# XieResearchGroup/Physics-aware-Multiplex-GNN

Hardware: AMD Instinct MI355X
Metric: molecules/sec (QM9 dim=128 n_layer=6) at 1/2/4/8 GPU; scatter-add HBM GB/s vs peak (higher is better)
Workload: dtype f32; 1 GPU; QM9-schema synthetic radius-graph batches, PAMNet dim=128 n_layer=6, 128 molecules/GPU (BASELINE configs[1]), full training step fwd+bwd+allreduce+clip+Adam+EMA; global_batch=128, parallelism=dp1 (molecule-sharded, RCCL all-reduce of flat grad), nodes_per_batch=2286, global_edges=32888, local_edges=4316, triplets=6662, pairs=10978

## Files before the change

include/pamnet_hip.h:

```cpp
#ifndef PAMNET_HIP_H
#define PAMNET_HIP_H

#include <stdint.h>

#ifdef __cplusplus
extern "C" {
#endif

#define PAMNET_OK 0
#define PAMNET_EINVAL (-1)
#define PAMNET_ENULL (-2)
#define PAMNET_WEIGHT_IMAGES 2
#define PAMNET_CHAIN_PIECES 16

typedef void* pamnet_stream_t;

#define PAMNET_ABI_VERSION 18
int pamnet_abi_version(void);

int pamnet_segment_sum_f32(float* out, const float* init, const float* A, const int32_t* ia, const float* B,
                           const int32_t* ib, const int32_t* perm, const int32_t* ptr, int64_t rows, int64_t d,
                           pamnet_stream_t stream);

int pamnet_gather_mul_f32(float* out, const float* A, const int32_t* ia, const float* B, const int32_t* ib,
                          int64_t m, int64_t d, pamnet_stream_t stream);

int pamnet_segment_sum_multi_f32(int64_t njobs, float* const* out, const float* const* A, const int32_t* const* perm,
                                 const int32_t* const* ptr, int64_t rows, int64_t d, pamnet_stream_t stream);
int pamnet_gather_mul2_f32(float* out1, float* out2, const float* A, const int32_t* ia, const float* B1,
                           const float* B2, int64_t m, int64_t d, pamnet_stream_t stream);

int pamnet_exclusive_scan_i32(const int32_t* in, int32_t* out, int64_t n, int32_t* tmp, pamnet_stream_t stream);
int pamnet_exclusive_scan_pair_i32(const int32_t* in_a, int32_t* out_a, const int32_t* in_b, int32_t* out_b, int64_t n,
                                   int32_t* tmp, pamnet_stream_t stream);

int pamnet_validate_inputs_i32(const int32_t* node_graph, int64_t n, int64_t n_graphs, const float* types,
                               int64_t type_stride, int64_t n_types, const int32_t* src, const int32_t* dst,
                               int64_t n_edges, int32_t* flag, pamnet_stream_t stream);
int pamnet_csr_from_keys_i32(const int32_t* keys, int64_t m, int64_t rows, int32_t* ptr, int32_t* perm,
                             int32_t* cursor, int32_t* perm_tmp, int32_t* tmp, pamnet_stream_t stream);
int pamnet_csr_from_keys_z_i32(const int32_t* keys, int64_t m, int64_t rows, int32_t* ptr, int32_t* perm,
                               int32_t* cursor, int32_t* perm_tmp, int32_t* tmp, pamnet_stream_t stream);

int pamnet_expand_rows_i32(const int32_t* ptr, int64_t rows, int32_t* row_of, int64_t cap, pamnet_stream_t stream);

int pamnet_csr_filter_count_i32(const int32_t* ptr_in, const int32_t* nbr, const float* dist, int64_t rows, float cut,
                                int32_t* count, pamnet_stream_t stream);
int pamnet_csr_filter_fill_i32(const int32_t* ptr_in, const int32_t* nbr, const float* dist, int64_t rows, float cut,
                               const int32_t* ptr_out, int32_t* nbr_out, float* dist_out, int64_t cap,
                               pamnet_stream_t stream);

int pamnet_radius_count_i32(const float* pos, const int32_t* node_graph, const int32_t* gptr, int64_t n,
                            int64_t n_graphs, float r, int64_t max_neighbors, int32_t* count, int32_t* cap_flag,
                            pamnet_stream_t stream);
int pamnet_radius_fill_i32(const float* pos, const int32_t* node_graph, const int32_t* gptr, int64_t n,
                           int64_t n_graphs, float r, int64_t max_neighbors, const int32_t* ptr, int32_t* nbr, float* dist,
                           int32_t* row_of , int64_t cap,
                           pamnet_stream_t stream);

int pamnet_knn_i32(const float* pos, const int32_t* node_graph, const int32_t* gptr, int64_t n, int32_t k,
                   float cutoff, int32_t* nbr, float* dist, pamnet_stream_t stream);
int pamnet_knn_cut_i32(const float* pos, const int32_t* node_graph, const int32_t* gptr, int64_t n, int32_t k, float cut_a,
                       float cut_b, int32_t* nbr, float* dist, int32_t* cnt_a, int32_t* cnt_b, pamnet_stream_t stream);
int pamnet_knn_tp_total_i64(const int32_t* nbr, const float* dist, int64_t n, int32_t k, float cut, int32_t with_triplets,
                            int32_t* indeg, int64_t* total, pamnet_stream_t stream);
int pamnet_knn_cut_fill_i32(const int32_t* nbr, const float* dist, int64_t n, int32_t k, float cut_a, const int32_t* raw_a,
                            int64_t cap_a, int32_t* nbr_a, float* dist_a, int32_t* row_a, int32_t* ptr_a, float cut_b,
                            const int32_t* raw_b, int64_t cap_b, int32_t* nbr_b, float* dist_b, int32_t* row_b, int32_t* ptr_b,
                            pamnet_stream_t stream);

int pamnet_edge_dist_f32(const float* pos, const int32_t* a, const int32_t* b, int64_t m, float* dist,
                         pamnet_stream_t stream);

int pamnet_triplet_count_i32(const int32_t* lptr, const int32_t* src, const int32_t* dst, int64_t n_edges,
                             int32_t with_triplets, int32_t* tcount, int32_t* tpcount, pamnet_stream_t stream);
int pamnet_triplet_fill_f32(const float* pos, const int32_t* lptr, const int32_t* src, const int32_t* dst,
                            int64_t n_edges, int32_t with_triplets, const int32_t* tp_ptr, int32_t* tp_idx,
                            int32_t* tp_edge, float* tp_angle, int32_t* tp_kind, int64_t cap, pamnet_stream_t stream);
int pamnet_triplet_transpose_count_i32(const int32_t* lptr, const int32_t* src, const int32_t* dst, const int32_t* lt_ptr,
                                       const int32_t* lt_perm, int64_t n_edges, int32_t with_triplets, int32_t* count,
                                       pamnet_stream_t stream);
int pamnet_triplet_transpose_fill_i32(const int32_t* lptr, const int32_t* src, const int32_t* dst, const int32_t* lt_ptr,
                                      const int32_t* lt_perm, int64_t n_edges, int32_t with_triplets, const int32_t* tp_ptr,
                                      const int32_t* tcount, const int32_t* tt_ptr, int32_t* tt_perm, int64_t cap,
                                      pamnet_stream_t stream);

int pamnet_reverse_edges_i32(const int32_t* ptr, const int32_t* row_of, const int32_t* col, int64_t m, int32_t* rev,
                             int32_t* flag, pamnet_stream_t stream);
int pamnet_gather_scalars_i64(int64_t n, const void* const* src ,
                              const int32_t* kind , int64_t* out, pamnet_stream_t stream);
int pamnet_check_sizes_i32(int64_t n_checks, const int32_t* const* actual ,
                           const int64_t* expected , const void* all_kept, const int32_t* self_loops,
                           int32_t* flag, pamnet_stream_t stream);
int pamnet_ingest_indices_i32(const void* batch, int32_t batch_kind, int64_t n, int64_t n_graphs, const void* x,
                              int32_t x_kind, int64_t x_stride, int64_t n_types, const void* edge_src,
                              const void* edge_dst, int32_t edge_kind, int64_t n_edges, int32_t* node_graph,
                              int32_t* gptr_flag, int32_t* types, int32_t* src, int32_t* dst, pamnet_stream_t stream);
int pamnet_gather2_i32(const int32_t* perm, const int32_t* a, const int32_t* b, int64_t m, int32_t* out_a,
                       int32_t* out_b, const float* pos, float* dist, pamnet_stream_t stream);
int pamnet_transpose_gather_i32(const int32_t* perm, const int32_t* q, const float* dist, int64_t m, int32_t* out_q,
                                float* out_dist, int32_t* inv, pamnet_stream_t stream);
int pamnet_collate_f32(int64_t n_graphs, const int32_t* sel, const int32_t* out_nptr, const int32_t* out_eptr,
                       const int32_t* src_nptr, const int32_t* src_eptr, const float* x, int64_t x_width,
                       const float* pos, const int32_t* esrc, const int32_t* edst, int64_t n_out, int64_t e_out,
                       float* out_x, float* out_pos, int32_t* out_batch, int32_t* out_esrc, int32_t* out_edst,
                       const float* y , float* out_y ,
                       pamnet_stream_t stream);

#define PAMNET_SCHEMA_QM9 0
#define PAMNET_SCHEMA_PDBBIND 1
#define PAMNET_SCHEMA_RNA 2
typedef struct pamnet_graph_desc {
    int64_t n, n_graphs, n_bonds;
    int64_t eg, el, tp;
    const void* batch;
    const void* types;
    int64_t types_stride, n_types;
    const float* pos;
    const float* rows;
    int64_t rows_width;
    const void* edge_src;
    const void* edge_dst;
    int32_t schema, batch_kind, types_kind, edge_kind;
    int32_t with_triplets;
    int32_t need_grad;
    int32_t aggregate_at_query;
    int32_t knn_k;
    float cutoff_l, cutoff_g;
    int32_t max_neighbors;
    int32_t mol_local;
} pamnet_graph_desc;
enum {
    PAMNET_GF_NODE_GRAPH = 0,
    PAMNET_GF_GPTR,
    PAMNET_GF_FLAG,
    PAMNET_GF_LOOPS,
    PAMNET_GF_TYPES,
    PAMNET_GF_POS,
    PAMNET_GF_SIGN,
    PAMNET_GF_G_PTR, PAMNET_GF_G_ROW, PAMNET_GF_G_COL, PAMNET_GF_G_DIST,
    PAMNET_GF_GT_PTR, PAMNET_GF_GT_PERM,
    PAMNET_GF_L_PTR, PAMNET_GF_L_ROW, PAMNET_GF_L_COL, PAMNET_GF_L_DIST,
    PAMNET_GF_LT_PTR, PAMNET_GF_LT_PERM,
    PAMNET_GF_T_PTR, PAMNET_GF_T_ROW, PAMNET_GF_T_COL, PAMNET_GF_T_ANGLE, PAMNET_GF_T_KIND,
    PAMNET_GF_TT_PTR, PAMNET_GF_TT_PERM,
    PAMNET_GF_CUTS,
    PAMNET_GF_TT_EDGE, PAMNET_GF_TT_NODE,
    PAMNET_GRAPH_FIELDS
};
typedef struct pamnet_mol_graph_out {
    int32_t *g_ptr, *g_row, *g_col;
    float* g_dist;
    int32_t* gT_perm;
    int32_t *l_ptr, *l_row, *l_col;
    float* l_dist;
    int32_t *lT_ptr, *lT_perm;
    int32_t *t_ptr, *t_row, *t_col;
    float* t_angle;
    int32_t* t_kind;
    int32_t *tT_ptr, *tT_perm;
} pamnet_mol_graph_out;
int pamnet_mol_graph_count_i32(const float* pos, const int32_t* gptr, int64_t n, int64_t n_graphs, const int32_t* src,
                               const int32_t* dst, int64_t n_bonds, float cutoff_g, int32_t with_triplets, int32_t* mol_tot,
                               int32_t* totals, pamnet_stream_t stream);
int pamnet_mol_graph_fill_i32(const float* pos, const int32_t* gptr, int64_t n, int64_t n_graphs, const int32_t* src,
                              const int32_t* dst, int64_t n_bonds, float cutoff_g, int32_t with_triplets, int32_t need_grad,
                              const int32_t* mol_tot, int64_t eg_cap, int64_t tp_cap, const pamnet_mol_graph_out* out,
                              pamnet_stream_t stream);
int pamnet_mol_graph_free_count_i32(const float* pos, const int32_t* gptr, int64_t n, int64_t n_graphs, float cutoff_l,
                                    float cutoff_g, int32_t with_triplets, int32_t* mol_tot, int32_t* totals,
                                    pamnet_stream_t stream);
int pamnet_mol_graph_free_fill_i32(const float* pos, const int32_t* gptr, int64_t n, int64_t n_graphs, int64_t n_local,
                                   float cutoff_l, float cutoff_g, int32_t with_triplets, int32_t need_grad,
                                   const int32_t* mol_tot, int64_t eg_cap, int64_t tp_cap, const pamnet_mol_graph_out* out,
                                   pamnet_stream_t stream);

int pamnet_graph_plan(const pamnet_graph_desc* desc, int64_t* layout , int64_t* arena_ints);
int pamnet_graph_build_i32(const pamnet_graph_desc* desc, int32_t* arena, float* sbf ,
                           pamnet_stream_t stream);

int pamnet_rbf_fwd_f32(const float* dist, const float* freq, float cutoff, int64_t m, float* rbf,
                       pamnet_stream_t stream);
int pamnet_rbf_bwd_f32(const float* dist, const float* freq, float cutoff, int64_t m, const float* grad,
                       float* dfreq, float* partial, pamnet_stream_t stream);
int pamnet_sbf_radial_f32(const float* dist, float cutoff, int64_t m, float* rad, pamnet_stream_t stream);
int pamnet_sbf_combine_f32(const float* rad, const int32_t* idx, const float* angle, int64_t m, float* sbf,
                           pamnet_stream_t stream);
int pamnet_rbf_fwd_env_f32(const float* dist, const float* freq, float cutoff, int32_t envelope_exponent, int64_t m,
                           float* rbf, pamnet_stream_t stream);
int pamnet_rbf_bwd_env_f32(const float* dist, const float* freq, float cutoff, int32_t envelope_exponent, int64_t m,
                           const float* grad, float* dfreq, float* partial, pamnet_stream_t stream);
int pamnet_sbf_radial_tab_f32(const float* dist, float cutoff, int64_t m, int32_t num_spherical, int32_t num_radial,
                              int32_t envelope_exponent, const float* zeros, const double* norm, float* rad,
                              pamnet_stream_t stream);
int pamnet_sbf_combine_tab_f32(const float* rad, const int32_t* idx, const float* angle, int64_t m, int32_t num_spherical,
                               int32_t num_radial, float* sbf, pamnet_stream_t stream);

int pamnet_rbf_ddist_f32(const float* dist, const float* freq, float cutoff, int64_t m, const float* grad, float* ddist,
                         pamnet_stream_t stream);
int pamnet_sbf_bwd_f32(const float* gsbf, const float* dist, float cutoff, int64_t n_edges, const int32_t* idx,
                       const float* angle, int64_t n_rows, const int32_t* tt_ptr, const int32_t* tt_perm, float* rad,
                       float* dangle, float* ddist, pamnet_stream_t stream);
int pamnet_pos_bwd_f32(const float* pos, int64_t n, const int32_t* g_ptr, const int32_t* g_row, const int32_t* g_col,
                       const int32_t* gt_ptr, const int32_t* gt_perm, const float* ddist_g, int64_t eg, const int32_t* l_ptr,
                       const int32_t* l_row, const int32_t* l_col, const int32_t* lt_ptr, const int32_t* lt_perm,
                       const float* ddist_l, int64_t el, const int32_t* t_ptr, const int32_t* t_row, const int32_t* t_col,
                       const int32_t* t_kind, const int32_t* tt_ptr, const int32_t* tt_perm, const float* dangle, int64_t tp,
                       double* bond_work, float* dpos, pamnet_stream_t stream);

int pamnet_fuse_pool_fwd_f32(const float* outs, const float* atts, int64_t n_layer, int64_t n, const float* sign,
                             const int32_t* gptr, int64_t n_graphs, int32_t mean, float* node_out, float* graph_out,
                             pamnet_stream_t stream);
int pamnet_fuse_pool_bwd_f32(const float* outs, const float* atts, int64_t n_layer, int64_t n, const float* sign,
                             const int32_t* node_graph, const int32_t* gptr, int32_t mean, const float* grad_graph,
                             float* grad_outs, float* grad_atts, pamnet_stream_t stream);

int pamnet_node_tail_fwd_f32(const float* x2, const float* res_x, int64_t n, const float* const* weights,
                             const float* const* biases, const float* w_out, const float* b_out, const float* w_att,
                             float* Z, float* R, float* x_out, float* out, float* att, const float* next_Wx1,
                             const float* next_bx1, const float* const* next_wp, int64_t next_ldwp, int64_t next_nblk,
                             float* next_Zx1, float* next_x1, float* next_P, int32_t packed, pamnet_stream_t stream);
int pamnet_node_tail_fwd_rider_f32(const float* x2, const float* res_x, int64_t n, const float* const* weights,
                                   const float* const* biases, const float* w_out, const float* b_out,
                                   const float* w_att, float* Z, float* R, float* x_out, const float* next_Wx1,
                                   const float* next_bx1, const float* const* next_wp, int64_t next_ldwp,
                                   int64_t next_nblk, float* next_Zx1, float* next_x1, float* next_P, const float* mlp_x,
                                   int64_t mlp_rows, int64_t mlp_tile0, int64_t mlp_ntiles, const float* const* mlp,
                                   float* const* mlp_out, int64_t rider_wgs, int32_t packed ,
                                   pamnet_stream_t stream);
int pamnet_node_heads_fwd_f32(int64_t n_layers, const float* const* x_out, const float* const* weights,
                              const float* const* biases, const float* const* w_out, const float* const* b_out,
                              const float* const* w_att, float* const* Z, float* const* out, float* const* att, int64_t n,
                              int32_t packed, pamnet_stream_t stream);
int pamnet_node_tail_bwd_f32(const float* d_xout, const float* d_out, const float* d_att, int64_t n,
                             const float* const* weights, const float* w_out, const float* w_att, const float* Z,
                             float* dZ, float* d_x2, float* d_resx, float* head_partial, float* d_wout, float* d_watt,
                             float* d_bout, int32_t packed, pamnet_stream_t stream);
int pamnet_node_heads_bwd_f32(int64_t n_layers, const float* const* d_out, const float* const* d_att,
                              const float* const* weights, const float* const* w_out, const float* const* w_att,
                              const float* const* Z, float* const* dZ3, float* const* g_head, float* const* head_partial,
                              int64_t n, int32_t packed, pamnet_stream_t stream);
int pamnet_node_tail_main_bwd_f32(const float* d_xout, const float* g_head, int64_t n, const float* const* weights,
                                  const float* Z, float* dZ, float* d_x2, float* d_resx, int32_t packed,
                                  pamnet_stream_t stream);
int pamnet_node_pre_tail_bwd_f32(const float* dP, const float* dx1_direct, const float* d_add, int64_t n,
                                 const float* Wx1, const float* const* wp, int64_t nblk, const float* Zx1, float* dZx1,
                                 const float* g_head, const float* const* weights, const float* Z, float* dZ,
                                 float* d_x2, float* d_resx, const void* rider ,
                                 pamnet_stream_t stream);
typedef struct pamnet_local_agg {
    const float *m_ji, *m_nb, *s, *q3, *init;
    const int32_t *t_ptr, *t_col, *l_ptr;
    float* m_t;
} pamnet_local_agg;
int pamnet_node_tail_fwd_agg_f32(float* x2, const float* res_x, int64_t n, const float* const* weights,
                                 const float* const* biases, const float* w_out, const float* b_out, const float* w_att,
                                 float* Z, float* R, float* x_out, const float* next_Wx1, const float* next_bx1,
                                 const float* const* next_wp, int64_t next_ldwp, int64_t next_nblk, float* next_Zx1,
                                 float* next_x1, float* next_P, const float* mlp_x, int64_t mlp_rows, int64_t mlp_tile0,
                                 int64_t mlp_ntiles, const float* const* mlp, float* const* mlp_out, int64_t rider_wgs,
                                 int32_t packed, const pamnet_local_agg* agg, pamnet_stream_t stream);
int pamnet_node_pre_tail_bwd_gather_f32(float* dP, const float* const* gather_src, const int32_t* const* gather_ptr,
                                        const int32_t* const* gather_perm, const float* dx1_direct, const float* d_add,
                                        int64_t n, const float* Wx1, const float* const* wp, int64_t nblk, const float* Zx1,
                                        float* dZx1, const float* g_head, const float* const* weights, const float* Z,
                                        float* dZ, float* d_x2, float* d_resx, const void* rider ,
                                        pamnet_stream_t stream);
int pamnet_pack_weights_f32(int64_t n, const float* const* W, const int64_t* ld, int32_t transposed, float* images,
                            pamnet_stream_t stream);
int pamnet_pack_weights_bf16x3(int64_t n, const float* const* W, const int64_t* ld, int32_t transposed, float* images,
                               pamnet_stream_t stream);
int pamnet_pack_weights_mixed_f32(int64_t n, const float* const* W, const int64_t* ld, const int32_t* kind,
                                  const int64_t* offset, int32_t transposed, float* images, pamnet_stream_t stream);
int pamnet_node_pre_fwd_f32(const float* x, int64_t n, const float* Wx1, const float* bx1, const float* const* wp,
                            int64_t ldwp, int64_t nblk, float* Zx1, float* x1, float* P, pamnet_stream_t stream);
int pamnet_node_pre_bwd_f32(const float* dP, const float* dx1_direct, const float* d_add, int64_t n, const float* Wx1,
                            const float* const* wp, int64_t ldwp, int64_t nblk, const float* Zx1, float* dZx1,
                            float* dx, int32_t packed, pamnet_stream_t stream);
int pamnet_wgrad_scratch_floats(int64_t njobs, const int64_t* rows, int64_t* floats);
int pamnet_wgrad_batched_f32(int64_t njobs, const float* const* dZ, const int64_t* ld_dz, const float* const* A,
                             const int64_t* ld_a, const int32_t* a_mode, const int64_t* rows, float* const* dW,
                             const int64_t* ld_dw, float* const* db, float* partial, const float* head_partial,
                             int64_t head_blocks, float* d_wout, float* d_watt, float* d_bout, pamnet_stream_t stream);
int pamnet_wgrad_ctx_bytes(int64_t* bytes );
int pamnet_wgrad_deferred_f32(int64_t njobs, const float* const* dZ, const int64_t* ld_dz, const float* const* A,
                              const int64_t* ld_a, const int32_t* a_mode, const int64_t* rows, float* const* dW,
                              const int64_t* ld_dw, float* const* db, float* partial, const float* head_partial,
                              int64_t head_blocks, float* d_wout, float* d_watt, float* d_bout,
                              const float* head2_partial ,
                              float* d_wout2, float* d_watt2, float* d_bout2, void* ctx ,
                              pamnet_stream_t stream);
int pamnet_wgrad_flush_f32(void* ctx , pamnet_stream_t stream);
int pamnet_wgrad_rider_bytes(int64_t* bytes);
int pamnet_wgrad_rider_plan_f32(int64_t njobs, const float* const* dZ, const int64_t* ld_dz, const float* const* A,
                                const int64_t* ld_a, const int32_t* a_mode, const int64_t* rows, float* const* dW,
                                const int64_t* ld_dw, float* const* db, float* partial, int64_t max_slots,
                                void* rider , int64_t* slots_out);
int pamnet_wgrad_rider_enqueue_f32(void* ctx , const void* rider );

int pamnet_global_edge_fwd_f32(const float* e, int64_t n_edges, const float* We, int64_t ld_we, const float* bm,
                               const float* Wea, int64_t ld_wea, const float* Pi, const float* Pj,
                               const int32_t* row_of, const int32_t* col, float* z, float* ea, float* msg,
                               pamnet_stream_t stream);
int pamnet_global_edge_bwd_f32(const float* d_agg, const int32_t* row_of, int64_t n_edges, const float* z,
                               const float* ea, const float* We, int64_t ld_we, const float* Wea, int64_t ld_wea,
                               float* dz, float* dea, float* d_e, int32_t accumulate, pamnet_stream_t stream);
int pamnet_local_edge_fwd_f32(const float* rbf, int64_t n_edges, const float* const* Wq, const int64_t* ldq,
                              const float* b_ji, const float* b_kj, const float* const* P, const int32_t* row_of,
                              const int32_t* col, float* z_ji, float* z_kj, float* q2, float* q3, float* m_ji,
                              float* m_nb, pamnet_stream_t stream);
int pamnet_local_edge_bwd_f32(const float* d_mji, const float* d_mnb, const float* d_q3, int64_t n_edges,
                              const float* z_ji, const float* z_kj, const float* q2, const float* const* Wq,
                              const int64_t* ldq, float* dz_ji, float* dz_kj, float* dq2, float* d_rbf,
                              int32_t accumulate, pamnet_stream_t stream);
int pamnet_global_edge_agg_fwd_f32(const float* e, int64_t n_edges, int64_t n_nodes, const float* We, int64_t ld_we,
                                   const float* bm, const float* Wea, int64_t ld_wea, const float* Pi, const float* Pj,
                                   const int32_t* ptr, const int32_t* row_of, const int32_t* col,
                                   const int32_t* cuts , const float* init, float* z,
                                   float* ea, float* out, pamnet_stream_t stream);
int pamnet_global_edge_agg_fwd_pp_f32(const float* e, int64_t n_edges, int64_t n_nodes, const float* We, int64_t ld_we,
                                      const float* bm, const float* Wea, int64_t ld_wea, const float* Pi, const float* Pj,
                                      const int32_t* ptr, const int32_t* row_of, const int32_t* col,
                                      const int32_t* cuts , const float* init, float* z, float* ea, float* out,
                                      pamnet_stream_t stream);
int pamnet_seg_cuts_i32(const int32_t* ptr, const int32_t* row_of, int64_t n_nodes, int64_t n_edges, int32_t* cuts,
                        int64_t* grid_out, pamnet_stream_t stream);
int pamnet_global_edge_agg_bwd_f32(const float* d_agg, int64_t n_edges, int64_t n_nodes, const int32_t* ptr,
                                   const int32_t* row_of, const int32_t* cuts , const float* z,
                                   const float* ea, const float* We,
                                   int64_t ld_we, const float* Wea, int64_t ld_wea, float* dz, float* dea, float* d_e,
                                   int32_t accumulate, float* dPi, pamnet_stream_t stream);
int pamnet_global_edge_agg_wg_floats(int64_t n_edges, int64_t* floats , int64_t* slots );
int pamnet_global_edge_agg_bwd_wg_f32(const float* d_agg, int64_t n_edges, int64_t n_nodes, const int32_t* ptr,
                                      const int32_t* row_of, const int32_t* cuts , const float* z,
                                      const float* ea, const float* e, const float* We, int64_t ld_we, const float* Wea,
                                      int64_t ld_wea, float* dz, float* d_e, int32_t accumulate, float* dPi, float* partial,
                                      pamnet_stream_t stream);
int pamnet_wgrad_edge_enqueue_f32(void* ctx , int64_t slots, float* dW_e, int64_t ld_e, float* db ,
                                  float* dW_ea, int64_t ld_ea, const float* partial);
int pamnet_local_agg_fwd_f32(const float* m_ji, const float* m_nb, const float* s, const float* q3,
                             const int32_t* t_ptr, const int32_t* t_col, const int32_t* l_ptr, const float* init,
                             int64_t n_nodes, float* m_t, float* out, pamnet_stream_t stream);
int pamnet_local_agg_bwd_f32(const float* d_x2, const int32_t* l_row, const float* q3, const float* m_t,
                             const float* m_nb, const float* s, const int32_t* t_ptr, const int32_t* t_col,
                             const int32_t* t_row, const int32_t* tT_ptr, const int32_t* tT_perm,
                             const int32_t* tT_edge , const int32_t* tT_node , int64_t n_edges,
                             float* d_mt, float* d_q3, float* d_s, float* d_mnb, pamnet_stream_t stream);
int pamnet_triplet_transpose_aux_i32(const int32_t* tT_perm, const int32_t* t_row, const int32_t* l_row, int64_t n_rows,
                                     int32_t* out_edge, int32_t* out_node, pamnet_stream_t stream);
int pamnet_mlp2_fwd_f32(const float* x, int64_t rows, const float* W1, const float* b1, const float* W2,
                        const float* b2, float* z1, float* z2, float* y, pamnet_stream_t stream);
int pamnet_mlp2_fwd_multi_f32(const float* x, int64_t rows, int64_t nsets, const float* const* params,
                              float* const* outs, pamnet_stream_t stream);
int pamnet_mlp2_bwd_f32(const float* dy, int64_t rows, const float* z1, const float* z2, const float* W1,
                        const float* W2, float* dz1, float* dz2, float* dx, int32_t accumulate,
                        pamnet_stream_t stream);
int pamnet_local_bwd_pair_f32(const float* dy, int64_t rows, const float* z1, const float* z2, const float* W1,
                              const float* W2, float* dz1, float* dz2, float* dx, int32_t accumulate_dx,
                              const float* d_mji, const float* d_mnb, const float* d_q3, int64_t n_edges,
                              const float* z_ji, const float* z_kj, const float* q2, const float* const* Wq,
                              const int64_t* ldq, float* dz_ji, float* dz_kj, float* dq2, float* d_rbf,
                              int32_t accumulate_rbf, pamnet_stream_t stream);

int pamnet_embed_scratch_floats(int64_t rows, int64_t K, int64_t* floats);
int pamnet_embed_fwd_f32(const float* x, int64_t rows, int64_t K, const int32_t* kind, const float* W0,
                         const float* b0, const float* W1, const float* b1, int32_t act, float* out,
                         pamnet_stream_t stream);
int pamnet_embed_bwd_f32(const float* x, int64_t rows, int64_t K, const int32_t* kind, const float* W0,
                         const float* b0, const float* W1, const float* b1, int32_t act, const float* gout,
                         float* dW0, float* db0, float* dW1, float* db1, float* dx, float* partial,
                         pamnet_stream_t stream);

typedef struct pamnet_embed_job {
    const float* x;
    const float* dist;
    const float* freq;
    float cutoff;
    int32_t K;
    int32_t act;
    int64_t rows;
    const int32_t* kind;
    const float *W0, *b0, *W1, *b1;
    float* out;
    const float* gout;
    float *dW0, *db0, *dW1, *db1, *dfreq, *dx;
    float* partial;
} pamnet_embed_job;
typedef struct pamnet_type_rows_job {
    const float* table;
    const int32_t* idx;
    int64_t n;
    int64_t n_types;
    float* out;
    const float* g;
    void* scratch;
    float* dtable;
} pamnet_type_rows_job;
int pamnet_embed_multi_fwd_f32(const pamnet_embed_job* jobs, int32_t n_jobs, const pamnet_type_rows_job* types,
                               pamnet_stream_t stream);
int pamnet_embed_multi_bwd_f32(const pamnet_embed_job* jobs, int32_t n_jobs, const pamnet_type_rows_job* types,
                               pamnet_stream_t stream);

int pamnet_stack_workspace(int64_t n, int64_t eg, int64_t el, int64_t tp, int64_t n_layer, int64_t d,
                           int64_t* saved_floats, int64_t* temp_floats);
int pamnet_stack_pack_floats(int64_t n_layer, int64_t d, int64_t* floats);
int pamnet_stack_layout(int64_t n, int64_t eg, int64_t el, int64_t tp, int64_t d, int64_t* layout);
int pamnet_stack_fwd_f32(const int64_t* sizes, const int32_t* const* graph_idx, int64_t n_layer, int64_t d,
                         const float* x0, const float* e_g, const float* rbf_e, const float* e_sbf,
                         const float* const* gparams, const float* const* lparams, float* saved, float* temp, float* outs,
                         float* atts, int32_t save_for_backward, float* wpack, pamnet_stream_t aux_stream,
                         void* const* aux_events, pamnet_stream_t stream);
int pamnet_stack_bwd_f32(const int64_t* sizes, const int32_t* const* graph_idx, int64_t n_layer, int64_t d,
                         const float* x0, const float* e_g, const float* rbf_e, const float* e_sbf,
                         const float* const* gparams, const float* const* lparams, const float* saved, float* temp,
                         const float* d_outs, const float* d_atts, float* const* ggrads, float* const* lgrads,
                         float* d_x0, float* d_eg, float* d_rbf, float* d_sbf, float* wpack, void* const* layer_done,
                         pamnet_stream_t stream);

int pamnet_reduce_scratch_bytes(int64_t* bytes);
int pamnet_stream_copy_f32(const float* src, float* dst, int64_t n, pamnet_stream_t stream);
int pamnet_sumsq_partials_f32(const float* g, int64_t n, double* partials, pamnet_stream_t stream);
int pamnet_l1_loss_f32(const float* out, const float* y, int64_t n, float grad_scale, float* loss, float* d_out,
                       pamnet_stream_t stream);
int pamnet_mse_loss_f32(const float* out, const float* y, int64_t n, float grad_scale, float* loss, float* d_out,
                        pamnet_stream_t stream);
int pamnet_smooth_l1_loss_f32(const float* out, const float* y, int64_t n, float grad_scale, float* loss, float* d_out,
                              pamnet_stream_t stream);
int pamnet_type_rows_grad_f32(const float* g, const int32_t* idx, int64_t n, int64_t n_types, int64_t d, void* scratch,
                              float* out, pamnet_stream_t stream);
#define PAMNET_MAX_PARAM_GROUPS 16
int pamnet_chunk_groups_check(const uint8_t* chunk_group_host, int64_t n_chunks, int64_t n_groups);
int pamnet_sumsq_partials_masked_f32(const float* g, int64_t n, const uint8_t* chunk_group, int64_t n_groups,
                                     const int32_t* frozen, double* partials, pamnet_stream_t stream);
int pamnet_grad_accumulate_f32(float* acc, float* g, int64_t n, pamnet_stream_t stream);

int pamnet_adam_ema_f32(float* p, float* g, float* m, float* v, float* shadow, int64_t n, float lr, float beta1,
                        float beta2, float eps, float weight_decay, int64_t step_count, float ema_decay,
                        const float* grad_norm, float max_norm, int32_t zero_grad, pamnet_stream_t stream);
int pamnet_adam_ema_norm_f32(float* p, float* g, float* m, float* v, float* shadow, int64_t n, float lr, float beta1,
                             float beta2, float eps, float weight_decay, int64_t step_count, float ema_decay,
                             const double* sumsq_partials, float* norm_out, float max_norm, int32_t zero_grad,
                             pamnet_stream_t stream);
int pamnet_adam_ema_groups_f32(float* p, float* g, float* m, float* v, float* shadow, int64_t n, const uint8_t* chunk_group,
                               int64_t n_groups, const float* lr_scale, const float* weight_decay, const int32_t* frozen,
                               float lr, float beta1, float beta2, float eps, int32_t decoupled, int64_t step_count,
                               float ema_decay, const double* sumsq_partials, float* norm_out, float max_norm,
                               int32_t zero_grad, pamnet_stream_t stream);

int pamnet_narrow_blocks(int64_t rows, int64_t* blocks );

int pamnet_narrow_global_fwd_f32(const float* e, int64_t m, int64_t d, const int32_t* tgt, const int32_t* src,
                                 const float* P, const float* We, int64_t ldwe, const float* bias, const float* Wea,
                                 int64_t ldwea, float* msg, pamnet_stream_t stream);
int pamnet_narrow_global_bwd_f32(const float* e, int64_t m, int64_t d, const int32_t* tgt, const int32_t* src,
                                 const float* P, const float* We, int64_t ldwe, const float* bias, const float* Wea,
                                 int64_t ldwea, const float* dagg, float* dz, float* de, float* partial, float* dWe,
                                 float* dWea, float* db, pamnet_stream_t stream);

int pamnet_narrow_mlp2_fwd_f32(const float* x, int64_t m, int64_t d, const float* W1, const float* b1, const float* W2,
                               const float* b2, int32_t res_x, const float* res, float* y, pamnet_stream_t stream);
int pamnet_narrow_mlp2_bwd_f32(const float* x, int64_t m, int64_t d, const float* W1, const float* b1, const float* W2,
                               const float* b2, const float* dy, int32_t res_x, float* dx, float* partial, float* dW,
                               float* db, pamnet_stream_t stream);
// ... 43 lines not shown
```

physics-aware-multiplex-gnn_amd/csrc/basis.hip:

```cpp
#include "common.h"
#include "basis_constants.h"

namespace {

__device__ __forceinline__ float envelope_f(float x) {
    if (!(x < 1.0f)) return 0.0f;
    const float x2 = x * x, x5 = x2 * x2 * x;
    return 1.0f / x + x5 * (-21.0f + x * (35.0f - 15.0f * x));
}

__device__ __forceinline__ double envelope_d(double x) {
    if (!(x < 1.0)) return 0.0;
    const double x2 = x * x, x5 = x2 * x2 * x;
    return 1.0 / x + x5 * (-21.0 + x * (35.0 - 15.0 * x));
}

constexpr int SERIES_TERMS = 28;
struct SeriesTab {
    double c[7][SERIES_TERMS + 1];
    double inv_dfact[7];
};
constexpr SeriesTab make_series() {
    SeriesTab t{};
    for (int l = 0; l < 7; ++l) {
        t.c[l][0] = 1.0;
        for (int k = 1; k <= SERIES_TERMS; ++k) t.c[l][k] = t.c[l][k - 1] * -0.5 / ((double)k * (double)(2 * l + 2 * k + 1));
        double d = 1.0;
        for (int m = 1; m <= l; ++m) d *= (double)(2 * m + 1);
        t.inv_dfact[l] = 1.0 / d;
    }
    return t;
}
__device__ __constant__ SeriesTab SBF_SERIES = make_series();

__device__ __forceinline__ double sph_jl(int l, double z) {
    if (z < (double)l + 1.0) {
        const double h = z * z;
        double sum = SBF_SERIES.c[l][SERIES_TERMS];
#pragma unroll
        for (int k = SERIES_TERMS - 1; k >= 0; --k) sum = fma(sum, h, SBF_SERIES.c[l][k]);
        double pref = SBF_SERIES.inv_dfact[l];
        for (int m = 0; m < l; ++m) pref *= z;
        return pref * sum;
    }
    double s, c;
    sincos(z, &s, &c);
    const double iz = 1.0 / z;
    double jm = s * iz;
    if (l == 0) return jm;
    double j = (jm - c) * iz;
    for (int m = 1; m < l; ++m) {
        const double jn = (double)(2 * m + 1) * iz * j - jm;
        jm = j;
        j = jn;
    }
    return j;
}

__global__ __launch_bounds__(256) void rbf_fwd_kernel(const float* __restrict__ dist, const float* __restrict__ freq,
                                                      float inv_cutoff, int64_t m, float* __restrict__ rbf) {
    const int64_t t = (int64_t)blockIdx.x * blockDim.x + threadIdx.x;
    if (t >= m * 16) return;
    const int64_t e = t >> 4;
    const int n = (int)(t & 15);
    const float x = dist[e] * inv_cutoff;
    rbf[t] = envelope_f(x) * sinf(freq[n] * x);
}

__global__ __launch_bounds__(256) void rbf_bwd_partial_kernel(const float* __restrict__ dist,
                                                              const float* __restrict__ freq, float inv_cutoff,
                                                              int64_t m, const float* __restrict__ grad,
                                                              float* __restrict__ partial) {
    __shared__ float red[256];
    const int n = threadIdx.x & 15, slot = threadIdx.x >> 4;
    const float f = freq[n];
    float acc = 0.f;
    for (int64_t e = (int64_t)blockIdx.x * 16 + slot; e < m; e += (int64_t)gridDim.x * 16) {
        const float x = dist[e] * inv_cutoff;
        acc += grad[e * 16 + n] * envelope_f(x) * x * cosf(f * x);
    }
    red[threadIdx.x] = acc;
    __syncthreads();
    for (int s = 128; s >= 16; s >>= 1) {
        if (threadIdx.x < s) red[threadIdx.x] += red[threadIdx.x + s];
        __syncthreads();
    }
    if (threadIdx.x < 16) partial[blockIdx.x * 16 + threadIdx.x] = red[threadIdx.x];
}

__global__ __launch_bounds__(1024) void rbf_bwd_final_kernel(const float* __restrict__ partial, int nblocks,
                                                             float* __restrict__ dfreq) {
    __shared__ float red[64][17];
    const int n = threadIdx.x & 15, sl = threadIdx.x >> 4;
    float s = 0.f;
    for (int b = sl; b < nblocks; b += 64) s += partial[b * 16 + n];
    red[sl][n] = s;
    __syncthreads();
    if (sl == 0) {
        float t = 0.f;
        for (int q = 0; q < 64; ++q) t += red[q][n];
        dfreq[n] = t;
    }
}

__global__ __launch_bounds__(256) void sbf_radial_rows_kernel(const float* __restrict__ dist, float inv_cutoff, int64_t m,
                                                              float* __restrict__ rad) {
    const int64_t t = (int64_t)blockIdx.x * blockDim.x + threadIdx.x;
    if (t >= m * 6) return;
    const int64_t e = t / 6;
    const int n = (int)(t - e * 6);
    const double x = (double)(dist[e] * inv_cutoff);
    const double env = envelope_d(x);
#pragma unroll 1
    for (int l = 0; l < 7; ++l) {
        const int c = l * 6 + n;
        rad[e * 42 + c] = (float)(env * PAMNET_SBF_NORM[c] * sph_jl(l, (double)PAMNET_SBF_ZEROS_F32[c] * x));
    }
}

__global__ __launch_bounds__(256) void sbf_radial_kernel(const float* __restrict__ dist, float inv_cutoff, int64_t m,
                                                         float* __restrict__ rad) {
    const int64_t t = (int64_t)blockIdx.x * blockDim.x + threadIdx.x;
    if (t >= m * 42) return;
    const int64_t e = t / 42;
    const int c = (int)(t - e * 42), l = c / 6;
    const double x = (double)(dist[e] * inv_cutoff);
    rad[t] = (float)(envelope_d(x) * PAMNET_SBF_NORM[c] * sph_jl(l, (double)PAMNET_SBF_ZEROS_F32[c] * x));
}

constexpr int SBF_ROWS = 64;
__global__ __launch_bounds__(256) void sbf_combine_kernel(const float* __restrict__ rad,
                                                          const int32_t* __restrict__ idx,
                                                          const float* __restrict__ angle, int64_t m,
                                                          float* __restrict__ sbf) {
    __shared__ double ylm[SBF_ROWS][7];
    __shared__ int src[SBF_ROWS];
    const int64_t row0 = (int64_t)blockIdx.x * SBF_ROWS;
    const int tid = threadIdx.x;
    if (tid < SBF_ROWS && row0 + tid < m) {
        const double ct = cos((double)angle[row0 + tid]);
        double p0 = 1.0, p1 = ct;
        ylm[tid][0] = PAMNET_YL0_PREF[0] * p0;
        ylm[tid][1] = PAMNET_YL0_PREF[1] * p1;
#pragma unroll
        for (int k = 2; k <= 6; ++k) {
            const double pl = ((double)(2 * k - 1) * ct * p1 - (double)(k - 1) * p0) / (double)k;
            p0 = p1;
            p1 = pl;
            ylm[tid][k] = PAMNET_YL0_PREF[k] * pl;
        }
        src[tid] = idx[row0 + tid];
    }
    __syncthreads();
    if (tid >= 252) return;
    const int rows = (int)((m - row0 < SBF_ROWS) ? (m - row0) : SBF_ROWS);
    const int r0 = tid / 42, c = tid - r0 * 42, l = c / 6;
    float* out = sbf + row0 * 42 + tid;
#pragma unroll 4
    for (int r = r0; r < rows; r += 6, out += 252)
        *out = (float)((double)rad[(int64_t)src[r] * 42 + c] * ylm[r][l]);
}

__device__ __forceinline__ double envelope_gen_d(double x, int p) {
    if (!(x < 1.0)) return 0.0;
    double xp = 1.0;
    for (int k = 0; k < p; ++k) xp *= x;
    const double a = -0.5 * (double)((p + 1) * (p + 2)), b = (double)(p * (p + 2)), c = -0.5 * (double)(p * (p + 1));
    return 1.0 / x + xp * (a + x * (b + c * x));
}
__device__ __forceinline__ float envelope_gen_f(float x, int p) {
    if (!(x < 1.0f)) return 0.0f;
    float xp = 1.0f;
    for (int k = 0; k < p; ++k) xp *= x;
    const float a = -0.5f * (float)((p + 1) * (p + 2)), b = (float)(p * (p + 2)), c = -0.5f * (float)(p * (p + 1));
    return 1.0f / x + xp * (a + x * (b + c * x));
}
__device__ __forceinline__ double sph_jl_gen(int l, double z) {
    if (z < (double)l + 1.0) {
        const double h = -0.5 * z * z;
        double term = 1.0, sum = 1.0;
        for (int k = 1; k <= 40; ++k) {
            term *= h / ((double)k * (double)(2 * l + 2 * k + 1));
            sum += term;
        }
        double pref = 1.0;
        for (int m = 1; m <= l; ++m) pref *= z / (double)(2 * m + 1);
        return pref * sum;
    }
    double s, c;
    sincos(z, &s, &c);
    const double iz = 1.0 / z;
    double jm = s * iz;
    if (l == 0) return jm;
    double j = (jm - c) * iz;
    for (int m = 1; m < l; ++m) {
        const double jn = (double)(2 * m + 1) * iz * j - jm;
        jm = j;
        j = jn;
    }
    return j;
}
constexpr int SBF_MAX_SPH = 16;
__global__ __launch_bounds__(256) void sbf_radial_tab_kernel(const float* __restrict__ dist, float inv_cutoff, int64_t m,
                                                             int ns, int nr, int p, const float* __restrict__ zeros,
                                                             const double* __restrict__ norm, float* __restrict__ rad) {
    const int64_t t = (int64_t)blockIdx.x * blockDim.x + threadIdx.x;
    if (t >= m * nr) return;
    const int64_t e = t / nr;
    const int n = (int)(t - e * nr);
    const double x = (double)(dist[e] * inv_cutoff);
    const double env = envelope_gen_d(x, p);
    for (int l = 0; l < ns; ++l) {
        const int c = l * nr + n;
        rad[e * (int64_t)(ns * nr) + c] = (float)(env * norm[c] * sph_jl_gen(l, (double)zeros[c] * x));
    }
}
__global__ __launch_bounds__(256) void sbf_combine_tab_kernel(const float* __restrict__ rad, const int32_t* __restrict__ idx,
                                                              const float* __restrict__ angle, int64_t m, int ns, int nr,
                                                              float* __restrict__ sbf) {
    __shared__ double ylm[SBF_ROWS][SBF_MAX_SPH];
    __shared__ int src[SBF_ROWS];
    const int64_t row0 = (int64_t)blockIdx.x * SBF_ROWS;
    const int tid = threadIdx.x;
    if (tid < SBF_ROWS && row0 + tid < m) {
        const double ct = cos((double)angle[row0 + tid]);
        double p0 = 1.0, p1 = ct;
        const double inv4pi = 0.25 / 3.14159265358979323846;
        ylm[tid][0] = sqrt(inv4pi);
        if (ns > 1) ylm[tid][1] = sqrt(3.0 * inv4pi) * p1;
        for (int k = 2; k < ns; ++k) {
            const double pl = ((double)(2 * k - 1) * ct * p1 - (double)(k - 1) * p0) / (double)k;
            p0 = p1;
            p1 = pl;
            ylm[tid][k] = sqrt((double)(2 * k + 1) * inv4pi) * pl;
        }
        src[tid] = idx[row0 + tid];
    }
    __syncthreads();
    const int w = ns * nr;
    const int64_t rows = (m - row0 < SBF_ROWS) ? (m - row0) : SBF_ROWS;
    const int total = (int)rows * w;
    for (int t = tid; t < total; t += 256) {
        const int r = t / w;
        const int c = t - r * w;
        sbf[row0 * w + t] = (float)((double)rad[(int64_t)src[r] * w + c] * ylm[r][c / nr]);
    }
}
__global__ __launch_bounds__(256) void rbf_fwd_env_kernel(const float* __restrict__ dist, const float* __restrict__ freq,
                                                          float inv_cutoff, int64_t m, int p, float* __restrict__ rbf) {
    const int64_t t = (int64_t)blockIdx.x * blockDim.x + threadIdx.x;
    if (t >= m * 16) return;
    const float x = dist[t >> 4] * inv_cutoff;
    rbf[t] = envelope_gen_f(x, p) * sinf(freq[t & 15] * x);
}
__global__ __launch_bounds__(256) void rbf_bwd_env_partial_kernel(const float* __restrict__ dist, const float* __restrict__ freq,
                                                                  float inv_cutoff, int64_t m, int p,
                                                                  const float* __restrict__ grad, float* __restrict__ partial) {
    __shared__ float red[256];
    const int n = threadIdx.x & 15, slot = threadIdx.x >> 4;
    const float f = freq[n];
    float acc = 0.f;
    for (int64_t e = (int64_t)blockIdx.x * 16 + slot; e < m; e += (int64_t)gridDim.x * 16) {
        const float x = dist[e] * inv_cutoff;
        acc += grad[e * 16 + n] * envelope_gen_f(x, p) * x * cosf(f * x);
    }
    red[threadIdx.x] = acc;
    __syncthreads();
    for (int s = 128; s >= 16; s >>= 1) {
        if (threadIdx.x < s) red[threadIdx.x] += red[threadIdx.x + s];
        __syncthreads();
    }
    if (threadIdx.x < 16) partial[blockIdx.x * 16 + threadIdx.x] = red[threadIdx.x];
}

__device__ __forceinline__ double envelope_dx_d(double x) {
    if (!(x < 1.0)) return 0.0;
    const double x2 = x * x, x4 = x2 * x2;
    return -1.0 / x2 + x4 * (-105.0 + x * (210.0 - 105.0 * x));
}

__global__ __launch_bounds__(256) void rbf_ddist_kernel(const float* __restrict__ dist, const float* __restrict__ freq,
                                                        float inv_cf, double inv_cutoff, int64_t m, const float* __restrict__ grad,
                                                        float* __restrict__ ddist) {
    const int64_t e = (int64_t)blockIdx.x * blockDim.x + threadIdx.x;
    if (e >= m) return;
    const double x = (double)(dist[e] * inv_cf);
    if (!(x < 1.0)) {
        ddist[e] = 0.0f;
        return;
    }
    const double env = envelope_d(x), denv = envelope_dx_d(x);
    const float* g = grad + e * 16;
    double acc = 0.0;
#pragma unroll
    for (int n = 0; n < 16; ++n) {
        const double f = (double)freq[n];
        double s, c;
        sincos(f * x, &s, &c);
        acc += (double)g[n] * (denv * s + env * f * c);
    }
    ddist[e] = (float)(acc * inv_cutoff);
}

__device__ __forceinline__ void yl0_and_derivative(double theta, double* y, double* dy) {
    double st, ct;
    sincos(theta, &st, &ct);
    double p[7], dp[7];
    p[0] = 1.0, p[1] = ct, dp[0] = 0.0, dp[1] = 1.0;
#pragma unroll
    for (int k = 2; k <= 6; ++k) {
        p[k] = ((double)(2 * k - 1) * ct * p[k - 1] - (double)(k - 1) * p[k - 2]) / (double)k;
        dp[k] = dp[k - 2] + (double)(2 * k - 1) * p[k - 1];
    }
#pragma unroll
    for (int k = 0; k <= 6; ++k) {
        y[k] = PAMNET_YL0_PREF[k] * p[k];
        dy[k] = -st * PAMNET_YL0_PREF[k] * dp[k];
    }
}

__global__ __launch_bounds__(256) void sbf_dangle_kernel(const float* __restrict__ gsbf, const float* __restrict__ rad,
                                                         const int32_t* __restrict__ idx, const float* __restrict__ angle,
                                                         int64_t m, float* __restrict__ dangle) {
    const int64_t t = (int64_t)blockIdx.x * blockDim.x + threadIdx.x;
    if (t >= m) return;
    double y[7], dy[7];
    yl0_and_derivative((double)angle[t], y, dy);
    const float* g = gsbf + t * 42;
    const float* r = rad + (int64_t)idx[t] * 42;
    double acc = 0.0;
#pragma unroll
    for (int l = 0; l < 7; ++l) {
        double s = 0.0;
#pragma unroll
        for (int n = 0; n < 6; ++n) s += (double)g[l * 6 + n] * (double)r[l * 6 + n];
        acc += s * dy[l];
    }
    dangle[t] = (float)acc;
}

__global__ __launch_bounds__(256) void sbf_ddist_kernel(const float* __restrict__ gsbf, const float* __restrict__ dist,
                                                        float inv_cf, double inv_cutoff, int64_t m, const float* __restrict__ angle,
                                                        const int32_t* __restrict__ tt_ptr, const int32_t* __restrict__ tt_perm,
                                                        float* __restrict__ ddist) {
    const int64_t q = ((int64_t)blockIdx.x * blockDim.x + threadIdx.x) >> 6;
    const int lane = threadIdx.x & 63;
    if (q >= m) return;
    const double x = (double)(dist[q] * inv_cf);
    if (!(x < 1.0)) {
        if (lane == 0) ddist[q] = 0.0f;
        return;
    }
    double v = 0.0;
    if (lane < 42) {
        const int l = lane / 6;
        double acc = 0.0;
        for (int k = tt_ptr[q]; k < tt_ptr[q + 1]; ++k) {
            const int64_t t = tt_perm[k];
            const double ct = cos((double)angle[t]);
            double p0 = 1.0, p1 = ct;
            for (int j = 2; j <= l; ++j) {
                const double pj = ((double)(2 * j - 1) * ct * p1 - (double)(j - 1) * p0) / (double)j;
                p0 = p1;
                p1 = pj;
            }
            acc += (double)gsbf[t * 42 + lane] * PAMNET_YL0_PREF[l] * (l == 0 ? 1.0 : p1);
        }
        const double env = envelope_d(x), denv = envelope_dx_d(x);
        const double z = (double)PAMNET_SBF_ZEROS_F32[lane], u = z * x;
        const double jl = sph_jl(l, u);
        const double djl = (l == 0) ? -sph_jl(1, u) : sph_jl(l - 1, u) - (double)(l + 1) / u * jl;
        v = acc * PAMNET_SBF_NORM[lane] * (denv * jl + env * z * djl);
    }
#pragma unroll
    for (int o = 32; o >= 1; o >>= 1) v += __shfl_xor(v, o, 64);
    if (lane == 0) ddist[q] = (float)(v * inv_cutoff);
}

__device__ __forceinline__ float leaky02(float a) { return a > 0.f ? a : 0.2f * a; }

__global__ __launch_bounds__(256) void fuse_node_kernel(const float* __restrict__ outs, const float* __restrict__ atts,
                                                        int n_layer, int64_t n, const float* __restrict__ sign,
                                                        float* __restrict__ node_out) {
    const int64_t v = (int64_t)blockIdx.x * blockDim.x + threadIdx.x;
    if (v >= n) return;
    float acc = 0.f;
    for (int l = 0; l < n_layer; ++l) {
        const float ag = leaky02(atts[(int64_t)(2 * l) * n + v]), al = leaky02(atts[(int64_t)(2 * l + 1) * n + v]);
        const float mx = fmaxf(ag, al);
        const float eg = expf(ag - mx), el = expf(al - mx);
        const float inv = 1.0f / (eg + el);
        acc += (outs[(int64_t)(2 * l) * n + v] * eg + outs[(int64_t)(2 * l + 1) * n + v] * el) * inv;
    }
    node_out[v] = sign ? acc * sign[v] : acc;
}

__global__ __launch_bounds__(256) void pool_kernel(const float* __restrict__ node_out, const int32_t* __restrict__ gptr,
                                                   int64_t n_graphs, int mean, float* __restrict__ graph_out) {
    const int lane = threadIdx.x & 63;
    const int64_t g = ((int64_t)blockIdx.x * blockDim.x + threadIdx.x) >> 6;
    if (g >= n_graphs) return;
    const int beg = gptr[g], end = gptr[g + 1];
    float s0 = 0.f, s1 = 0.f, s2 = 0.f, s3 = 0.f;
    int v = beg + lane;
    for (; v + 192 < end; v += 256) {
        s0 += node_out[v];
        s1 += node_out[v + 64];
        s2 += node_out[v + 128];
        s3 += node_out[v + 192];
    }
    for (; v < end; v += 64) s0 += node_out[v];
    float s = (s0 + s1) + (s2 + s3);
#pragma unroll
    for (int o = 32; o >= 1; o >>= 1) s += __shfl_xor(s, o, 64);
    if (lane == 0) graph_out[g] = mean ? s / (float)max(end - beg, 1) : s;
}

__global__ __launch_bounds__(256) void fuse_pool_bwd_kernel(const float* __restrict__ outs,
                                                            const float* __restrict__ atts, int n_layer, int64_t n,
                                                            const float* __restrict__ sign,
                                                            const int32_t* __restrict__ node_graph,
                                                            const int32_t* __restrict__ gptr, int mean,
                                                            const float* __restrict__ grad_graph,
                                                            float* __restrict__ grad_outs,
                                                            float* __restrict__ grad_atts) {
    const int64_t v = (int64_t)blockIdx.x * blockDim.x + threadIdx.x;
    if (v >= n) return;
    const int g = node_graph[v];
    float gn = grad_graph[g];
    if (mean) gn /= (float)max(gptr[g + 1] - gptr[g], 1);
    if (sign) gn *= sign[v];
    for (int l = 0; l < n_layer; ++l) {
        const int64_t ig = (int64_t)(2 * l) * n + v, il = (int64_t)(2 * l + 1) * n + v;
        const float rg = atts[ig], rl = atts[il];
        const float ag = leaky02(rg), al = leaky02(rl);
        const float mx = fmaxf(ag, al);
        const float eg = expf(ag - mx), el = expf(al - mx);
        const float inv = 1.0f / (eg + el);
        const float wg = eg * inv, wl = el * inv;
        grad_outs[ig] = gn * wg;
        grad_outs[il] = gn * wl;
        const float da = gn * (outs[ig] - outs[il]) * wg * wl;
        grad_atts[ig] = da * (rg > 0.f ? 1.0f : 0.2f);
        grad_atts[il] = -da * (rl > 0.f ? 1.0f : 0.2f);
    }
}

inline unsigned blocks_for(int64_t n, int per = 256) { return (unsigned)(n > 0 ? ceil_div(n, per) : 1); }

}

extern "C" int pamnet_abi_version(void) { return PAMNET_ABI_VERSION; }

extern "C" int pamnet_rbf_fwd_f32(const float* dist, const float* freq, float cutoff, int64_t m, float* rbf,
                                  pamnet_stream_t stream) {
    if (m < 0 || !(cutoff > 0.f)) return PAMNET_EINVAL;
    if (m == 0) return PAMNET_OK;
    if (!dist || !freq || !rbf) return PAMNET_ENULL;
    hipLaunchKernelGGL(rbf_fwd_kernel, dim3(blocks_for(m * 16)), dim3(256), 0, as_stream(stream), dist, freq,
                       1.0f / cutoff, m, rbf);
    PAMNET_LAUNCH_CHECK();
    return PAMNET_OK;
}
// ... 155 lines not shown
```

physics-aware-multiplex-gnn_amd/csrc/graph_engine.hip:

```cpp
#include "common.h"

namespace {

constexpr int64_t RAD_W = 42;

__global__ __launch_bounds__(256) void clamp_copy_kernel(const int32_t* __restrict__ in, int32_t* __restrict__ out, int64_t n,
                                                         int32_t cap) {
    const int64_t i = (int64_t)blockIdx.x * 256 + threadIdx.x;
    if (i < n) out[i] = in[i] < cap ? in[i] : cap;
}

__global__ __launch_bounds__(256) void split_rows_kernel(const float* __restrict__ x, int64_t width, int64_t n,
                                                         float* __restrict__ pos, float* __restrict__ sign) {
    const int64_t i = (int64_t)blockIdx.x * 256 + threadIdx.x;
    if (i >= n) return;
    const float px = x[i * width], py = x[i * width + 1], pz = x[i * width + 2];
    pos[3 * i] = px, pos[3 * i + 1] = py, pos[3 * i + 2] = pz;
    if (sign) sign[i] = px > 40.0f ? -1.0f : 1.0f;
}

inline unsigned blocks(int64_t n) { return (unsigned)((n + 255) / 256 > 0 ? (n + 255) / 256 : 1); }

struct Run {
    const pamnet_graph_desc& d;
    int32_t* base;
    float* sbf;
    pamnet_stream_t stream;
    bool dry;
    int64_t off = 0;
    int64_t* lay;

    int64_t take(int64_t n) {
        const int64_t o = off;
        off += (n + 3) / 4 * 4;
        return o;
    }
    int32_t* I(int64_t o) const { return base + o; }
    float* F(int64_t o) const { return reinterpret_cast<float*>(base + o); }
    void field(int f, int64_t o) { lay[f] = o; }
};

#define GO(call)                         \
    do {                                 \
        if (!r.dry) {                    \
            const int rc__ = (call);     \
            if (rc__) return rc__;       \
        }                                \
    } while (0)
#define GOK(...)                                               \
    do {                                                       \
        if (!r.dry) {                                          \
            hipLaunchKernelGGL(__VA_ARGS__);                   \
            const hipError_t e__ = hipGetLastError();          \
            if (e__ != hipSuccess) return (int)e__;            \
        }                                                      \
    } while (0)

int scan(Run& r, int64_t counts, int64_t n, int64_t& out) {
    out = r.take(n + 1);
    const int64_t tmp = r.take((n + 4095) / 4096 + 1);
    GO(pamnet_exclusive_scan_i32(r.I(counts), r.I(out), n, r.I(tmp), r.stream));
    return PAMNET_OK;
}

int csr(Run& r, int64_t keys, int64_t m, int64_t rows, int64_t cursor, int64_t& ptr, int64_t& perm) {
    if (ptr < 0) ptr = r.take(rows + 1);
    if (perm < 0) perm = r.take(m);
    const int64_t perm_tmp = r.take(m), tmp = r.take((rows + 4095) / 4096 + 1);
    GO(pamnet_csr_from_keys_z_i32(r.I(keys), m, rows, r.I(ptr), r.I(perm), r.I(cursor), r.I(perm_tmp), r.I(tmp), r.stream));
    return PAMNET_OK;
}

int clamp(Run& r, int64_t in, int64_t n, int64_t cap, int64_t& out) {
    out = r.take(n);
    GOK(clamp_copy_kernel, dim3(blocks(n)), dim3(256), 0, as_stream(r.stream), r.I(in), r.I(out), n, (int32_t)cap);
    return PAMNET_OK;
}

int run(Run& r) {
    const pamnet_graph_desc& d = r.d;
    const int64_t n = d.n, ng = d.n_graphs, eg = d.eg, el = d.el, tp = d.tp;
    const bool grad = d.need_grad != 0;
    const int wt = d.with_triplets ? 1 : 0;
    for (int f = 0; f < PAMNET_GRAPH_FIELDS; ++f) r.lay[f] = -1;

    const int64_t node_graph = r.take(n), types = r.take(n), gf = r.take(ng + 7);
    const int64_t src0 = r.take(d.n_bonds), dst0 = r.take(d.n_bonds);
    r.field(PAMNET_GF_NODE_GRAPH, node_graph);
    r.field(PAMNET_GF_GPTR, gf);
    r.field(PAMNET_GF_FLAG, gf + ng + 1);
    r.field(PAMNET_GF_LOOPS, gf + ng + 2);
    const bool has_types = d.schema != PAMNET_SCHEMA_PDBBIND;
    if (has_types) r.field(PAMNET_GF_TYPES, types);
    GO(pamnet_ingest_indices_i32(d.batch, d.batch_kind, n, ng, has_types ? d.types : nullptr, has_types ? d.types_kind : 0,
                                 d.types_stride > 0 ? d.types_stride : 1, d.n_types > 0 ? d.n_types : 1, d.edge_src, d.edge_dst,
                                 d.edge_kind, d.n_bonds, r.I(node_graph), r.I(gf), r.I(types), r.I(src0), r.I(dst0),
                                 r.stream));
    const int32_t* flag = r.dry ? nullptr : r.I(gf + ng + 1);
    const int32_t* loops = r.dry ? nullptr : r.I(gf + ng + 2);
    const int32_t* gptr = r.dry ? nullptr : r.I(gf);

    const float* pos = d.pos;
    if (d.schema != PAMNET_SCHEMA_QM9) {
        const int64_t p = r.take(3 * n);
        int64_t sg = -1;
        if (d.schema == PAMNET_SCHEMA_PDBBIND) sg = r.take(n);
        r.field(PAMNET_GF_POS, p);
        if (sg >= 0) r.field(PAMNET_GF_SIGN, sg);
        GOK(split_rows_kernel, dim3(blocks(n)), dim3(256), 0, as_stream(r.stream), d.rows, d.rows_width, n, r.F(p),
            sg >= 0 ? r.F(sg) : nullptr);
        pos = r.dry ? nullptr : r.F(p);
    }

    const int64_t z0 = r.off;
    const int64_t g_row = r.take(eg), g_col = r.take(eg), g_dist = r.take(eg);
    const int64_t t_row = r.take(tp), t_col = r.take(tp), t_angle = r.take(tp), t_kind = r.take(tp);
    int64_t l_row = -1, l_col = -1, l_dist = -1;
    int64_t kq_g = -1, kn_l = -1, kd_l = -1, kq_l = -1, gn2 = -1, gd2 = -1;
    if (d.schema != PAMNET_SCHEMA_QM9) l_row = r.take(el), l_col = r.take(el), l_dist = r.take(el);
    if (d.schema == PAMNET_SCHEMA_RNA) {
        kn_l = r.take(el), kd_l = r.take(el), kq_l = r.take(el);
        if (!d.aggregate_at_query) gn2 = r.take(eg), gd2 = r.take(eg), kq_g = r.take(eg);
    }
    const int64_t cur_a = r.take(n + 2), cur_b = r.take(n + 2), cur_c = r.take(n + 2);
    const int64_t tT_perm_z = grad ? r.take(tp) : -1;
    const int64_t z1 = r.off;
    if (!r.dry) {
        const hipError_t e = hipMemsetAsync(r.I(z0), 0, sizeof(int32_t) * (size_t)(z1 - z0), as_stream(r.stream));
        if (e != hipSuccess) return (int)e;
    }

    int64_t g_ptr = -1, l_ptr = -1, t_ptr_raw = -1, t_ptr = -1;
    int64_t gT_ptr = -1, gT_perm = -1, lT_ptr = -1, lT_perm = -1;
    const int32_t* chk_ptr[3] = {nullptr, nullptr, nullptr};
    int64_t chk_val[3] = {0, 0, 0};
    auto check = [&](int slot, int64_t raw_ptr, int64_t rows, int64_t expected) {
        chk_ptr[slot] = r.dry ? nullptr : r.I(raw_ptr + rows);
        chk_val[slot] = expected;
    };
    int64_t t_cnt = -1;
    auto triplet_ptr = [&](int64_t lp, int64_t lsrc, int64_t ldst) -> int {
        const int64_t tc = r.take(el), tpc = r.take(el);
        t_cnt = tc;
        GO(pamnet_triplet_count_i32(r.I(lp), r.I(lsrc), r.I(ldst), el, wt, r.I(tc), r.I(tpc), r.stream));
        int rc = scan(r, tpc, el, t_ptr_raw);
        if (rc) return rc;
        check(2, t_ptr_raw, el, tp);
        return clamp(r, t_ptr_raw, el + 1, tp, t_ptr);
    };

    int64_t tT_ptr = -1, tT_perm = -1;
    const int64_t mol_totals = gf + ng + 3;
    const bool mol = d.schema == PAMNET_SCHEMA_QM9 && d.mol_local != 0;
    if (mol) {
        l_row = r.take(el), l_col = r.take(el), l_dist = r.take(el);
        l_ptr = r.take(n + 1), g_ptr = r.take(n + 1), t_ptr = r.take(el + 1);
        if (grad) {
            gT_ptr = g_ptr, gT_perm = r.take(eg);
            lT_ptr = r.take(n + 1), lT_perm = r.take(el);
            tT_ptr = r.take(el + 1), tT_perm = tT_perm_z;
        }
        const int64_t mol_tot = r.take(4 * ng);
        GO(pamnet_mol_graph_count_i32(pos, gptr, n, ng, r.I(src0), r.I(dst0), d.n_bonds, d.cutoff_g, wt, r.I(mol_tot),
                                      r.I(mol_totals), r.stream));
        pamnet_mol_graph_out o{};
        if (!r.dry) {
            o.g_ptr = r.I(g_ptr), o.g_row = r.I(g_row), o.g_col = r.I(g_col), o.g_dist = r.F(g_dist);
            o.l_ptr = r.I(l_ptr), o.l_row = r.I(l_row), o.l_col = r.I(l_col), o.l_dist = r.F(l_dist);
            o.t_ptr = r.I(t_ptr), o.t_row = r.I(t_row), o.t_col = r.I(t_col), o.t_angle = r.F(t_angle), o.t_kind = r.I(t_kind);
            if (grad) {
                o.gT_perm = r.I(gT_perm), o.lT_ptr = r.I(lT_ptr), o.lT_perm = r.I(lT_perm);
                o.tT_ptr = r.I(tT_ptr), o.tT_perm = r.I(tT_perm);
            }
        }
        GO(pamnet_mol_graph_fill_i32(pos, gptr, n, ng, r.I(src0), r.I(dst0), d.n_bonds, d.cutoff_g, wt, grad ? 1 : 0,
                                     r.I(mol_tot), eg, tp, &o, r.stream));
        chk_ptr[0] = r.dry ? nullptr : r.I(mol_totals), chk_val[0] = eg;
        chk_ptr[1] = r.dry ? nullptr : r.I(mol_totals + 3), chk_val[1] = el;
        chk_ptr[2] = r.dry ? nullptr : r.I(mol_totals + 1), chk_val[2] = tp;
    } else if (d.schema == PAMNET_SCHEMA_QM9) {
        l_row = r.take(el), l_col = r.take(el), l_dist = r.take(el);
        int64_t perm = -1;
        int rc = csr(r, dst0, d.n_bonds, n, cur_a, l_ptr, perm);
        if (rc) return rc;
        GO(pamnet_gather2_i32(r.I(perm), r.I(src0), r.I(dst0), d.n_bonds, r.I(l_col), r.I(l_row), pos, r.F(l_dist), r.stream));
        if ((rc = triplet_ptr(l_ptr, l_col, l_row))) return rc;
        const int64_t cnt = r.take(n);
        int64_t raw = -1;
        GO(pamnet_radius_count_i32(pos, r.I(node_graph), gptr, n, ng, d.cutoff_g, d.max_neighbors, r.I(cnt), const_cast<int32_t*>(flag), r.stream));
        if ((rc = scan(r, cnt, n, raw))) return rc;
        check(0, raw, n, eg);
        check(1, l_ptr, n, el);
        if ((rc = clamp(r, raw, n + 1, eg, g_ptr))) return rc;
        GO(pamnet_radius_fill_i32(pos, r.I(node_graph), gptr, n, ng, d.cutoff_g, d.max_neighbors, r.I(g_ptr), r.I(g_col), r.F(g_dist),
                                  r.I(g_row), eg, r.stream));
    } else if (d.schema == PAMNET_SCHEMA_PDBBIND) {
        const int64_t cg = r.take(n), cl = r.take(n);
        int64_t raw_g = -1, raw_l = -1;
        GO(pamnet_radius_count_i32(pos, r.I(node_graph), gptr, n, ng, d.cutoff_g, d.max_neighbors, r.I(cg), const_cast<int32_t*>(flag), r.stream));
        int rc = scan(r, cg, n, raw_g);
        if (rc) return rc;
        GO(pamnet_radius_count_i32(pos, r.I(node_graph), gptr, n, ng, d.cutoff_l, 0, r.I(cl), nullptr, r.stream));
        if ((rc = scan(r, cl, n, raw_l))) return rc;
        check(0, raw_g, n, eg);
        check(1, raw_l, n, el);
        if ((rc = clamp(r, raw_g, n + 1, eg, g_ptr))) return rc;
        if ((rc = clamp(r, raw_l, n + 1, el, l_ptr))) return rc;
        GO(pamnet_radius_fill_i32(pos, r.I(node_graph), gptr, n, ng, d.cutoff_g, d.max_neighbors, r.I(g_ptr), r.I(g_col), r.F(g_dist),
                                  r.I(g_row), eg, r.stream));
        GO(pamnet_csr_filter_fill_i32(r.I(g_ptr), r.I(g_col), r.F(g_dist), n, d.cutoff_l, r.I(l_ptr), r.I(l_col), r.F(l_dist),
                                      el, r.stream));
        GO(pamnet_expand_rows_i32(r.I(l_ptr), n, r.I(l_row), el, r.stream));
        if ((rc = triplet_ptr(l_ptr, l_col, l_row))) return rc;
    } else {
        const int64_t k = d.knn_k;
        const int64_t kn = r.take(n * k), kd = r.take(n * k);
        const int64_t ca = r.take(n), cb = r.take(n);
        GO(pamnet_knn_cut_i32(pos, r.I(node_graph), gptr, n, (int32_t)k, d.cutoff_g, d.cutoff_l, r.I(kn), r.F(kd), r.I(ca), r.I(cb),
                              r.stream));
        const int64_t raw_a = r.take(n + 1), raw_b = r.take(n + 1), pa = r.take(n + 1), pb = r.take(n + 1);
        const int64_t stmp = r.take((n + 4095) / 4096 + 1);
        GO(pamnet_exclusive_scan_pair_i32(r.I(ca), r.I(raw_a), r.I(cb), r.I(raw_b), n, r.I(stmp), r.stream));
        check(0, raw_a, n, eg);
        check(1, raw_b, n, el);
        const int64_t gq_n = d.aggregate_at_query ? g_col : gn2, gq_d = d.aggregate_at_query ? g_dist : gd2;
        const int64_t gq_q = d.aggregate_at_query ? g_row : kq_g;
        GO(pamnet_knn_cut_fill_i32(r.I(kn), r.F(kd), n, (int32_t)k, d.cutoff_g, r.I(raw_a), eg, r.I(gq_n), r.F(gq_d), r.I(gq_q),
                                   r.I(pa), d.cutoff_l, r.I(raw_b), el, r.I(kn_l), r.F(kd_l), r.I(kq_l), r.I(pb), r.stream));
        int rc = PAMNET_OK;
        if (d.aggregate_at_query) {
            g_ptr = pa;
        } else {
            int64_t perm = -1;
            if ((rc = csr(r, gq_n, eg, n, cur_b, g_ptr, perm))) return rc;
            int64_t inv = -1;
            if (grad) inv = r.take(eg);
            GO(pamnet_transpose_gather_i32(r.I(perm), r.I(kq_g), r.F(gq_d), eg, r.I(g_col), r.F(g_dist),
                                           grad ? r.I(inv) : nullptr, r.stream));
            if (grad) gT_ptr = pa, gT_perm = inv;
        }
        if (!d.aggregate_at_query) {
            GO(pamnet_expand_rows_i32(r.I(g_ptr), n, r.I(g_row), eg, r.stream));
        }
        int64_t perm = -1;
        if ((rc = csr(r, kn_l, el, n, cur_a, l_ptr, perm))) return rc;
        int64_t inv = -1;
        if (grad) inv = r.take(el);
        GO(pamnet_transpose_gather_i32(r.I(perm), r.I(kq_l), r.F(kd_l), el, r.I(l_col), r.F(l_dist), grad ? r.I(inv) : nullptr,
                                       r.stream));
        if (grad) lT_ptr = pb, lT_perm = inv;
        GO(pamnet_expand_rows_i32(r.I(l_ptr), n, r.I(l_row), el, r.stream));
        if ((rc = triplet_ptr(l_ptr, l_col, l_row))) return rc;
    }

    if (!mol) {
        GO(pamnet_triplet_fill_f32(pos, r.I(l_ptr), r.I(l_col), r.I(l_row), el, wt, r.I(t_ptr), r.I(t_col), r.I(t_row),
                                   r.F(t_angle), r.I(t_kind), tp, r.stream));
    }
    GO(pamnet_check_sizes_i32(3, chk_ptr, chk_val, nullptr, d.schema == PAMNET_SCHEMA_QM9 ? loops : nullptr,
                              const_cast<int32_t*>(flag), r.stream));

    if (grad && !mol) {
        if (d.schema != PAMNET_SCHEMA_RNA) {
            gT_ptr = g_ptr;
            gT_perm = r.take(eg);
            GO(pamnet_reverse_edges_i32(r.I(g_ptr), r.I(g_row), r.I(g_col), eg, r.I(gT_perm), nullptr, r.stream));
        } else if (d.aggregate_at_query) {
            int rc = csr(r, g_col, eg, n, cur_b, gT_ptr, gT_perm);
            if (rc) return rc;
        }
        if (d.schema == PAMNET_SCHEMA_PDBBIND) {
            lT_ptr = l_ptr;
            lT_perm = r.take(el);
            GO(pamnet_reverse_edges_i32(r.I(l_ptr), r.I(l_row), r.I(l_col), el, r.I(lT_perm), nullptr, r.stream));
        } else if (d.schema == PAMNET_SCHEMA_QM9) {
            int rc = csr(r, l_col, el, n, cur_c, lT_ptr, lT_perm);
            if (rc) return rc;
        }
        const int64_t cntT = r.take(el);
        GO(pamnet_triplet_transpose_count_i32(r.I(l_ptr), r.I(l_col), r.I(l_row), r.I(lT_ptr), r.I(lT_perm), el, wt, r.I(cntT),
                                              r.stream));
        int64_t rawT = -1;
        int rc = scan(r, cntT, el, rawT);
        if (rc) return rc;
        if ((rc = clamp(r, rawT, el + 1, tp, tT_ptr))) return rc;
        tT_perm = tT_perm_z;
        GO(pamnet_triplet_transpose_fill_i32(r.I(l_ptr), r.I(l_col), r.I(l_row), r.I(lT_ptr), r.I(lT_perm), el, wt, r.I(t_ptr),
                                             r.I(t_cnt), r.I(tT_ptr), r.I(tT_perm), tp, r.stream));
    }

    int64_t tT_edge = -1, tT_node = -1;
    if (d.need_grad == 1 && tT_perm >= 0 && tp > 0) {
        tT_edge = r.take(tp), tT_node = r.take(tp);
        GO(pamnet_triplet_transpose_aux_i32(r.I(tT_perm), r.I(t_row), r.I(l_row), tp, r.I(tT_edge), r.I(tT_node), r.stream));
    }

    const int64_t rad = r.take(el * RAD_W);
    if (r.sbf) {
        GO(pamnet_sbf_radial_f32(r.F(l_dist), d.cutoff_l, el, r.F(rad), r.stream));
        GO(pamnet_sbf_combine_f32(r.F(rad), r.I(t_col), r.F(t_angle), tp, r.sbf, r.stream));
    }
    const int64_t cuts = r.take(260);
    GO(pamnet_seg_cuts_i32(r.I(g_ptr), r.I(g_row), n, eg, r.I(cuts), nullptr, r.stream));

    r.field(PAMNET_GF_G_PTR, g_ptr), r.field(PAMNET_GF_G_ROW, g_row), r.field(PAMNET_GF_G_COL, g_col);
    r.field(PAMNET_GF_G_DIST, g_dist), r.field(PAMNET_GF_GT_PTR, gT_ptr), r.field(PAMNET_GF_GT_PERM, gT_perm);
    r.field(PAMNET_GF_L_PTR, l_ptr), r.field(PAMNET_GF_L_ROW, l_row), r.field(PAMNET_GF_L_COL, l_col);
    r.field(PAMNET_GF_L_DIST, l_dist), r.field(PAMNET_GF_LT_PTR, lT_ptr), r.field(PAMNET_GF_LT_PERM, lT_perm);
    r.field(PAMNET_GF_T_PTR, t_ptr), r.field(PAMNET_GF_T_ROW, t_row), r.field(PAMNET_GF_T_COL, t_col);
    r.field(PAMNET_GF_T_ANGLE, t_angle), r.field(PAMNET_GF_T_KIND, t_kind);
    r.field(PAMNET_GF_TT_PTR, tT_ptr), r.field(PAMNET_GF_TT_PERM, tT_perm);
    r.field(PAMNET_GF_CUTS, cuts);
    r.field(PAMNET_GF_TT_EDGE, tT_edge), r.field(PAMNET_GF_TT_NODE, tT_node);
    return PAMNET_OK;
}

int validate(const pamnet_graph_desc* d) {
    if (!d) return PAMNET_ENULL;
    if (d->schema < PAMNET_SCHEMA_QM9 || d->schema > PAMNET_SCHEMA_RNA) return PAMNET_EINVAL;
    if (d->n < 1 || d->n_graphs < 1 || d->eg < 1 || d->el < 1 || d->tp < 1 || d->n_bonds < 0) return PAMNET_EINVAL;
    if (d->n >= ((int64_t)1 << 31) / 64 || d->eg >= (int64_t)1 << 31 || d->tp >= (int64_t)1 << 31) return PAMNET_EINVAL;
    if (d->schema == PAMNET_SCHEMA_QM9 && (d->n_bonds != d->el || d->n_types < 1)) return PAMNET_EINVAL;
    if (d->schema != PAMNET_SCHEMA_QM9 && (d->n_bonds != 0 || d->rows_width < 3)) return PAMNET_EINVAL;
    if (d->schema == PAMNET_SCHEMA_PDBBIND && !(d->cutoff_l <= d->cutoff_g)) return PAMNET_EINVAL;
    if (d->schema == PAMNET_SCHEMA_RNA && (d->knn_k < 1 || d->knn_k > 64 || d->n_types < 1)) return PAMNET_EINVAL;
    return PAMNET_OK;
}

}

extern "C" int pamnet_graph_plan(const pamnet_graph_desc* desc, int64_t* layout, int64_t* arena_ints) {
    const int rc = validate(desc);
    if (rc) return rc;
    if (!layout || !arena_ints) return PAMNET_ENULL;
    Run r{*desc, nullptr, nullptr, nullptr, true, 0, layout};
    const int rr = run(r);
    *arena_ints = r.off + 64;
    return rr;
}

extern "C" int pamnet_graph_build_i32(const pamnet_graph_desc* desc, int32_t* arena, float* sbf, pamnet_stream_t stream) {
    const int rc = validate(desc);
    if (rc) return rc;
    if (!arena || !desc->batch) return PAMNET_ENULL;
    if (desc->schema == PAMNET_SCHEMA_QM9 && (!desc->pos || !desc->types || !desc->edge_src || !desc->edge_dst)) return PAMNET_ENULL;
    if (desc->schema != PAMNET_SCHEMA_QM9 && !desc->rows) return PAMNET_ENULL;
    if (desc->schema == PAMNET_SCHEMA_RNA && !desc->types) return PAMNET_ENULL;
    int64_t layout[PAMNET_GRAPH_FIELDS];
    Run r{*desc, arena, sbf, stream, false, 0, layout};
    return run(r);
}
```

physics-aware-multiplex-gnn_amd/csrc/graph_mol.hip:

```cpp
#include "common.h"
#include "geom_core.h"

namespace {

constexpr int MOL_ATOMS = 64, MOL_BONDS = 256, MOL_CHUNKS = MOL_BONDS / 64;

struct MolIn {
    const float* pos;
    const int32_t *gptr, *src, *dst;
    int64_t n, n_graphs, n_bonds;
    float cutoff_g;
    int with_triplets, need_grad;
    float cutoff_l;
};

__device__ __forceinline__ int wave_sum(int v) {
#pragma unroll
    for (int o = 32; o > 0; o >>= 1) v += __shfl_xor(v, o, 64);
    return v;
}

__device__ __forceinline__ int wave_incl(int v, int lane) {
#pragma unroll
    for (int o = 1; o < 64; o <<= 1) {
        const int u = __shfl_up(v, o, 64);
        if (lane >= o) v += u;
    }
    return v;
}

__device__ __forceinline__ float lane_value(float v, int l) {
    return __int_as_float(__builtin_amdgcn_readlane(__float_as_int(v), l));
}

__device__ __forceinline__ void bond_range(const int32_t* __restrict__ dst, int m, int a0, int a1, int lane, int& b0, int& b1) {
    const int a = lane < 32 ? a0 : a1, t = lane & 31;
    int lo = 0, hi = m;
    for (int round = 0; round < 8; ++round) {
        const bool open = lo < hi;
        if (!__ballot(open)) break;
        const int step = open ? (hi - lo + 31) / 32 : 1;
        const int p = lo + (t + 1) * step - 1;
        const bool probe = open && p < hi;
        const bool less = probe && dst[p] < a;
        const unsigned long long v = __ballot(less);
        const int c = __popc((unsigned)(lane < 32 ? v : (v >> 32)));
        if (open) {
            const int nlo = lo + c * step, nhi = lo + (c + 1) * step - 1;
            lo = nlo;
            hi = nhi < hi ? nhi : hi;
        }
    }
    b0 = __builtin_amdgcn_readlane(lo, 0);
    b1 = __builtin_amdgcn_readlane(lo, 32);
}

template <bool FREE>
__device__ __forceinline__ void radius_masks(float xi, float yi, float zi, int lane, int na, float cutoff_g, float cutoff_l,
                                             unsigned long long& mask, unsigned long long& lmask) {
    mask = lmask = 0ull;
    for (int j = 0; j < na; ++j) {
        const float d = dist3_xyz(xi, yi, zi, lane_value(xi, j), lane_value(yi, j), lane_value(zi, j));
        if (j != lane && lane < na && d <= cutoff_g) mask |= 1ull << j;
        if (FREE && j != lane && lane < na && d <= cutoff_l) lmask |= 1ull << j;
    }
}

template <bool FILL, bool FREE>
__global__ __launch_bounds__(64) void mol_graph_kernel(MolIn in, int32_t* __restrict__ mol_tot,
                                                       int32_t* __restrict__ totals, pamnet_mol_graph_out out,
                                                       int64_t eg_cap, int64_t tp_cap) {
    __shared__ float px[MOL_ATOMS], py[MOL_ATOMS], pz[MOL_ATOMS];
    __shared__ int l_src[MOL_BONDS], l_dst[MOL_BONDS];
    __shared__ int lt[MOL_BONDS];
    __shared__ int lptr[MOL_ATOMS + 1], ltptr[MOL_ATOMS + 1];
    __shared__ int tptr[MOL_BONDS + 1], tcnt[MOL_BONDS];
    __shared__ int gex[MOL_ATOMS];
    __shared__ unsigned long long adj[MOL_ATOMS];
    const int g = blockIdx.x, lane = threadIdx.x;
    const int a0 = in.gptr[g], a1 = in.gptr[g + 1], na = a1 - a0;
    const bool last = g == (int)in.n_graphs - 1;
    int b0 = 0, b1 = 0;
    int se = 0, st = 0;
    if constexpr (FILL && FREE) {
        int sl = 0;
        for (int q = lane; q < g; q += 64) se += mol_tot[4 * q], st += mol_tot[4 * q + 1], sl += mol_tot[4 * q + 2];
        b0 = b1 = wave_sum(sl);
    } else if constexpr (FREE) {
    } else if constexpr (FILL) {
        b0 = mol_tot[4 * g + 2];
        b1 = last ? (int)in.n_bonds : mol_tot[4 * g + 6];
        for (int q = lane; q < g; q += 64) se += mol_tot[4 * q], st += mol_tot[4 * q + 1];
    } else {
        bond_range(in.dst, (int)in.n_bonds, a0, a1, lane, b0, b1);
    }
    int nb = b1 - b0;
    int flags = 0;
    if (na < 0 || na > MOL_ATOMS) flags |= 1;
    if (nb < 0 || nb > MOL_BONDS) flags |= 2;
    if (flags) {
        if (!FILL && lane == 0) {
            mol_tot[4 * g] = mol_tot[4 * g + 1] = 0;
            mol_tot[4 * g + 2] = FREE ? 0 : b0;
            mol_tot[4 * g + 3] = flags;
            atomicOr(&totals[2], flags);
        }
        return;
    }
    float xi = 0.f, yi = 0.f, zi = 0.f;
    if (lane < na) {
        const int64_t a = a0 + lane;
        xi = in.pos[3 * a], yi = in.pos[3 * a + 1], zi = in.pos[3 * a + 2];
        px[lane] = xi, py[lane] = yi, pz[lane] = zi;
    }
    unsigned long long mask = 0ull, lmask = 0ull;
    if constexpr (FREE) {
        radius_masks<true>(xi, yi, zi, lane, na, in.cutoff_g, in.cutoff_l, mask, lmask);
        const int ldeg = __popcll(lmask);
        const int linc = wave_incl(ldeg, lane);
        nb = __shfl(linc, 63, 64);
        if (nb > MOL_BONDS || (FILL && (int64_t)b0 + nb > in.n_bonds)) {
            if (!FILL && lane == 0) {
                mol_tot[4 * g] = mol_tot[4 * g + 1] = mol_tot[4 * g + 2] = 0;
                mol_tot[4 * g + 3] = 2;
                atomicOr(&totals[2], 2);
            }
            return;
        }
        int w = linc - ldeg;
        if (lane < na) lptr[lane] = w;
        if (lane == 0) lptr[na] = nb;
        for (unsigned long long m = lmask; m; m &= m - 1) {
            l_src[w] = __ffsll((long long)m) - 1, l_dst[w] = lane;
            ++w;
        }
    }
    const int nchunk = (nb + 63) >> 6;
    int bs[MOL_CHUNKS], bd[MOL_CHUNKS];
    bool stray = false;
#pragma unroll
    for (int c = 0; c < (FREE ? 0 : MOL_CHUNKS); ++c) {
        const int k = c * 64 + lane;
        bs[c] = bd[c] = -1;
        if (k < nb) {
            int s = in.src[b0 + k] - a0, d = in.dst[b0 + k] - a0;
            if (s < 0 || s >= na || d < 0 || d >= na) stray = true, s = d = 0;
            bs[c] = s, bd[c] = d;
        }
    }
    if (__ballot(stray)) flags |= 4;

    if constexpr (!FREE) {
        int run = 0, mine = 0;
        for (int i = 0; i < na; ++i) {
            if (lane == i) mine = run;
#pragma unroll
            for (int c = 0; c < MOL_CHUNKS; ++c) {
                if (c < nchunk) {
                    const bool hit = bd[c] == i;
                    const unsigned long long m = __ballot(hit);
                    if (hit) {
                        const int w = run + __popcll(m & ((1ull << lane) - 1ull));
                        l_src[w] = bs[c], l_dst[w] = i;
                    }
                    run += __popcll(m);
                }
            }
        }
        if (lane < na) lptr[lane] = mine;
        if (lane == 0) lptr[na] = nb;
    }
    __syncthreads();
    int ss[MOL_CHUNKS], sd[MOL_CHUNKS];
#pragma unroll
    for (int c = 0; c < MOL_CHUNKS; ++c) {
        const int k = c * 64 + lane;
        ss[c] = k < nb ? l_src[k] : -1;
        sd[c] = k < nb ? l_dst[k] : -1;
    }
    {
        int run = 0, mine = 0;
        for (int j = 0; j < na; ++j) {
            if (lane == j) mine = run;
#pragma unroll
            for (int c = 0; c < MOL_CHUNKS; ++c) {
                if (c < nchunk) {
                    const bool hit = ss[c] == j;
                    const unsigned long long m = __ballot(hit);
                    if (hit) lt[run + __popcll(m & ((1ull << lane) - 1ull))] = c * 64 + lane;
                    run += __popcll(m);
                }
            }
        }
        if (lane < na) ltptr[lane] = mine;
        if (lane == 0) ltptr[na] = nb;
    }

    int carry = 0;
#pragma unroll
    for (int c = 0; c < MOL_CHUNKS; ++c) {
        if (c < nchunk) {
            const int k = c * 64 + lane;
            int t = 0, cnt = 0;
            if (k < nb) {
                const int j = ss[c], i = sd[c];
                if (in.with_triplets)
                    for (int q = lptr[j]; q < lptr[j + 1]; ++q) t += (l_src[q] != i) ? 1 : 0;
                cnt = t + lptr[i + 1] - lptr[i];
                tcnt[k] = t;
            }
            const int inc = wave_incl(cnt, lane);
            if (k < nb) tptr[k] = carry + inc - cnt;
            carry += __shfl(inc, 63, 64);
        }
    }
    const int tp_m = carry;

    if constexpr (!FREE) radius_masks<false>(xi, yi, zi, lane, na, in.cutoff_g, 0.f, mask, lmask);
    const int deg = __popcll(mask);
    const int ginc = wave_incl(deg, lane);
    const int eg_m = __shfl(ginc, 63, 64);

    if (!FILL) {
        if (lane == 0) {
            mol_tot[4 * g] = flags ? 0 : eg_m;
            mol_tot[4 * g + 1] = flags ? 0 : tp_m;
            mol_tot[4 * g + 2] = FREE ? nb : b0;
            mol_tot[4 * g + 3] = flags;
            if (flags) {
                atomicOr(&totals[2], flags);
            } else {
                atomicAdd(&totals[0], eg_m);
                atomicAdd(&totals[1], tp_m);
                atomicAdd(&totals[3], nb);
            }
        }
        return;
    }
    if (flags) return;
    adj[lane] = mask;
    gex[lane] = ginc - deg;

    const int64_t eoff = wave_sum(se), toff = wave_sum(st);
    __syncthreads();

    if (lane < na) out.l_ptr[a0 + lane] = b0 + lptr[lane];
    if (last && lane == 0) {
        out.l_ptr[in.n] = (int32_t)in.n_bonds;
        out.g_ptr[in.n] = (int32_t)(eoff + eg_m < eg_cap ? eoff + eg_m : eg_cap);
        out.t_ptr[in.n_bonds] = (int32_t)(toff + tp_m < tp_cap ? toff + tp_m : tp_cap);
    }
#pragma unroll
    for (int c = 0; c < MOL_CHUNKS; ++c) {
        const int k = c * 64 + lane;
        if (k >= nb) continue;
        const int j = ss[c], i = sd[c];
        const float pix = px[i], piy = py[i], piz = pz[i], pjx = px[j], pjy = py[j], pjz = pz[j];
        out.l_row[b0 + k] = a0 + i;
        out.l_col[b0 + k] = a0 + j;
        out.l_dist[b0 + k] = dist3_xyz(pix, piy, piz, pjx, pjy, pjz);
        int64_t w = toff + tptr[k];
        out.t_ptr[b0 + k] = (int32_t)(w < tp_cap ? w : tp_cap);
        if (in.with_triplets) {
            for (int q = lptr[j]; q < lptr[j + 1]; ++q) {
                const int kk = l_src[q];
                if (kk == i) continue;
                if (w < tp_cap) {
                    out.t_col[w] = b0 + q;
                    out.t_row[w] = b0 + k;
                    out.t_kind[w] = 0;
                    out.t_angle[w] = angle3(pjx - pix, pjy - piy, pjz - piz, px[kk] - pjx, py[kk] - pjy, pz[kk] - pjz);
                }
                ++w;
            }
        }
        for (int q = lptr[i]; q < lptr[i + 1]; ++q) {
            const int j2 = l_src[q];
            if (w < tp_cap) {
                out.t_col[w] = b0 + q;
                out.t_row[w] = b0 + k;
                out.t_kind[w] = 1;
                out.t_angle[w] = angle3(pix - pjx, piy - pjy, piz - pjz, px[j2] - pix, py[j2] - piy, pz[j2] - piz);
            }
            ++w;
        }
    }

    if (lane < na) {
        const int64_t w0 = eoff + gex[lane];
        out.g_ptr[a0 + lane] = (int32_t)(w0 < eg_cap ? w0 : eg_cap);
        unsigned long long m = mask;
        int64_t w = w0;
        while (m) {
            const int j = __ffsll((long long)m) - 1;
            m &= m - 1;
            if (w < eg_cap) {
                out.g_row[w] = a0 + lane;
                out.g_col[w] = a0 + j;
                out.g_dist[w] = dist3_xyz(xi, yi, zi, px[j], py[j], pz[j]);
                if (in.need_grad) {
                    const int64_t rv = eoff + gex[j] + __popcll(adj[j] & ((1ull << lane) - 1ull));
                    out.gT_perm[w] = (int32_t)(rv < eg_cap ? rv : eg_cap - 1);
                }
            }
            ++w;
        }
    }
    if (!in.need_grad) return;

    if (lane < na) out.lT_ptr[a0 + lane] = b0 + ltptr[lane];
    if (last && lane == 0) {
        out.lT_ptr[in.n] = (int32_t)in.n_bonds;
        out.tT_ptr[in.n_bonds] = (int32_t)(toff + tp_m < tp_cap ? toff + tp_m : tp_cap);
    }
    for (int k = lane; k < nb; k += 64) out.lT_perm[b0 + k] = b0 + lt[k];

    carry = 0;
#pragma unroll
    for (int c = 0; c < MOL_CHUNKS; ++c) {
        if (c >= nchunk) continue;
        const int q = c * 64 + lane;
        const bool on = q < nb;
        const int kq = on ? ss[c] : 0, jq = on ? sd[c] : 0;
        const int ab = ltptr[jq], ae = in.with_triplets ? ltptr[jq + 1] : ab, bb = lptr[jq], be = lptr[jq + 1];
        int cnt = 0;
        if (on) {
            for (int a = ab; a < ae; ++a) cnt += (l_dst[lt[a]] != kq) ? 1 : 0;
            cnt += be - bb;
        }
        const int inc = wave_incl(cnt, lane);
        if (on) {
            int64_t w2 = toff + carry + inc - cnt;
            out.tT_ptr[b0 + q] = (int32_t)(w2 < tp_cap ? w2 : tp_cap);
            int a = ab, b = bb;
            while (true) {
                while (a < ae && l_dst[lt[a]] == kq) ++a;
                const int ea = a < ae ? lt[a] : 0x7fffffff, eb = b < be ? b : 0x7fffffff;
                if (ea == 0x7fffffff && eb == 0x7fffffff) break;
                int row;
                if (ea < eb) {
                    const int ie = l_dst[ea];
                    int rank = 0;
                    for (int q2 = bb; q2 < q; ++q2) rank += (l_src[q2] != ie) ? 1 : 0;
                    row = tptr[ea] + rank;
                    ++a;
                } else {
                    row = tptr[eb] + tcnt[eb] + (q - bb);
                    ++b;
                }
                if (w2 < tp_cap) out.tT_perm[w2] = (int32_t)(toff + row < tp_cap ? toff + row : tp_cap - 1);
                ++w2;
            }
        }
        carry += __shfl(inc, 63, 64);
    }
}

int check_in(const float* pos, const int32_t* gptr, int64_t n, int64_t n_graphs, const int32_t* src, const int32_t* dst,
             int64_t n_bonds, float cutoff_g) {
    if (n < 0 || n_graphs < 1 || n_bonds < 0 || n >= ((int64_t)1 << 31) || n_bonds >= ((int64_t)1 << 30) || !(cutoff_g >= 0.f))
        return PAMNET_EINVAL;
    if (!pos || !gptr || (n_bonds > 0 && (!src || !dst))) return PAMNET_ENULL;
    return PAMNET_OK;
}

int check_free(const float* pos, const int32_t* gptr, int64_t n, int64_t n_graphs, int64_t n_local, float cutoff_l,
               float cutoff_g) {
    if (n < 0 || n_graphs < 1 || n_local < 0 || n >= ((int64_t)1 << 31) || n_local >= ((int64_t)1 << 30) || !(cutoff_l > 0.f) ||
        !(cutoff_g > 0.f))
        return PAMNET_EINVAL;
    if (!pos || !gptr) return PAMNET_ENULL;
    return PAMNET_OK;
}

}

extern "C" int pamnet_mol_graph_count_i32(const float* pos, const int32_t* gptr, int64_t n, int64_t n_graphs,
                                          const int32_t* src, const int32_t* dst, int64_t n_bonds, float cutoff_g,
                                          int32_t with_triplets, int32_t* mol_tot, int32_t* totals,
                                          pamnet_stream_t stream) {
    const int rc = check_in(pos, gptr, n, n_graphs, src, dst, n_bonds, cutoff_g);
    if (rc) return rc;
    if (!mol_tot || !totals) return PAMNET_ENULL;
    const MolIn in{pos, gptr, src, dst, n, n_graphs, n_bonds, cutoff_g, with_triplets ? 1 : 0, 0, 0.f};
    const pamnet_mol_graph_out none{};
    hipLaunchKernelGGL((mol_graph_kernel<false, false>), dim3((unsigned)n_graphs), dim3(64), 0, as_stream(stream), in, mol_tot, totals,
                       none, (int64_t)0, (int64_t)0);
    PAMNET_LAUNCH_CHECK();
    return PAMNET_OK;
}

extern "C" int pamnet_mol_graph_fill_i32(const float* pos, const int32_t* gptr, int64_t n, int64_t n_graphs,
                                         const int32_t* src, const int32_t* dst, int64_t n_bonds, float cutoff_g,
                                         int32_t with_triplets, int32_t need_grad, const int32_t* mol_tot, int64_t eg_cap,
                                         int64_t tp_cap, const pamnet_mol_graph_out* out, pamnet_stream_t stream) {
    const int rc = check_in(pos, gptr, n, n_graphs, src, dst, n_bonds, cutoff_g);
    if (rc) return rc;
    if (!mol_tot || !out) return PAMNET_ENULL;
    if (eg_cap < 0 || tp_cap < 0) return PAMNET_EINVAL;
    const pamnet_mol_graph_out& o = *out;
    if (!o.g_ptr || !o.l_ptr || !o.t_ptr) return PAMNET_ENULL;
    if (eg_cap > 0 && (!o.g_row || !o.g_col || !o.g_dist || (need_grad && !o.gT_perm))) return PAMNET_ENULL;
    if (n_bonds > 0 && (!o.l_row || !o.l_col || !o.l_dist || (need_grad && !o.lT_perm))) return PAMNET_ENULL;
    if (tp_cap > 0 && (!o.t_row || !o.t_col || !o.t_angle || !o.t_kind || (need_grad && !o.tT_perm))) return PAMNET_ENULL;
    if (need_grad && (!o.lT_ptr || !o.tT_ptr)) return PAMNET_ENULL;
    const MolIn in{pos, gptr, src, dst, n, n_graphs, n_bonds, cutoff_g, with_triplets ? 1 : 0, need_grad ? 1 : 0, 0.f};
    hipLaunchKernelGGL((mol_graph_kernel<true, false>), dim3((unsigned)n_graphs), dim3(64), 0, as_stream(stream), in,
                       const_cast<int32_t*>(mol_tot), (int32_t*)nullptr, o, eg_cap, tp_cap);
    PAMNET_LAUNCH_CHECK();
    return PAMNET_OK;
}

extern "C" int pamnet_mol_graph_free_count_i32(const float* pos, const int32_t* gptr, int64_t n, int64_t n_graphs,
                                               float cutoff_l, float cutoff_g, int32_t with_triplets, int32_t* mol_tot,
                                               int32_t* totals, pamnet_stream_t stream) {
    const int rc = check_free(pos, gptr, n, n_graphs, 0, cutoff_l, cutoff_g);
    if (rc) return rc;
    if (!mol_tot || !totals) return PAMNET_ENULL;
    const MolIn in{pos, gptr, nullptr, nullptr, n, n_graphs, 0, cutoff_g, with_triplets ? 1 : 0, 0, cutoff_l};
    const pamnet_mol_graph_out none{};
    hipLaunchKernelGGL((mol_graph_kernel<false, true>), dim3((unsigned)n_graphs), dim3(64), 0, as_stream(stream), in, mol_tot,
                       totals, none, (int64_t)0, (int64_t)0);
    PAMNET_LAUNCH_CHECK();
    return PAMNET_OK;
}

extern "C" int pamnet_mol_graph_free_fill_i32(const float* pos, const int32_t* gptr, int64_t n, int64_t n_graphs,
                                              int64_t n_local, float cutoff_l, float cutoff_g, int32_t with_triplets,
                                              int32_t need_grad, const int32_t* mol_tot, int64_t eg_cap, int64_t tp_cap,
                                              const pamnet_mol_graph_out* out, pamnet_stream_t stream) {
    const int rc = check_free(pos, gptr, n, n_graphs, n_local, cutoff_l, cutoff_g);
    if (rc) return rc;
    if (!mol_tot || !out) return PAMNET_ENULL;
    if (eg_cap < 0 || tp_cap < 0) return PAMNET_EINVAL;
    const pamnet_mol_graph_out& o = *out;
    if (!o.g_ptr || !o.l_ptr || !o.t_ptr) return PAMNET_ENULL;
    if (eg_cap > 0 && (!o.g_row || !o.g_col || !o.g_dist || (need_grad && !o.gT_perm))) return PAMNET_ENULL;
    if (n_local > 0 && (!o.l_row || !o.l_col || !o.l_dist || (need_grad && !o.lT_perm))) return PAMNET_ENULL;
    if (tp_cap > 0 && (!o.t_row || !o.t_col || !o.t_angle || !o.t_kind || (need_grad && !o.tT_perm))) return PAMNET_ENULL;
    if (need_grad && (!o.lT_ptr || !o.tT_ptr)) return PAMNET_ENULL;
    const MolIn in{pos, gptr, nullptr, nullptr, n, n_graphs, n_local, cutoff_g, with_triplets ? 1 : 0, need_grad ? 1 : 0,
                   cutoff_l};
    hipLaunchKernelGGL((mol_graph_kernel<true, true>), dim3((unsigned)n_graphs), dim3(64), 0, as_stream(stream), in,
                       const_cast<int32_t*>(mol_tot), (int32_t*)nullptr, o, eg_cap, tp_cap);
    PAMNET_LAUNCH_CHECK();
    return PAMNET_OK;
}
```

physics-aware-multiplex-gnn_amd/pamnet_amd/graph.py:

```python
import os

import torch

from . import lib

I32 = torch.int32


def _i32(n, dev):
    return torch.empty(int(n), dtype=I32, device=dev)


def _f32(n, dev):
    return torch.empty(int(n), dtype=torch.float32, device=dev)


class _ZeroArena(object):

    def __init__(self, ints, dev):
        self.buf = torch.zeros(int(ints) + 64, dtype=I32, device=dev)
        self.off = 0

    def take(self, n, dtype=I32):
        n = int(n)
        v = self.buf[self.off:self.off + n]
        self.off += (n + 3) // 4 * 4
        return v if dtype == I32 else v.view(dtype)


def _alloc_i32(n, dev, zeroed):
    return zeroed.take(n) if zeroed else _i32(n, dev)


def _alloc_f32(n, dev, zeroed):
    return zeroed.take(n, torch.float32) if zeroed else _f32(n, dev)


def exclusive_scan(counts):
    n = counts.numel()
    out = _i32(n + 1, counts.device)
    tmp = _i32((n + 4095) // 4096 + 1, counts.device)
    lib.call('pamnet_exclusive_scan_i32', lib.ptr(counts), lib.ptr(out), n, lib.ptr(tmp), lib.stream_of(counts))
    return out


def csr_from_keys(keys, rows):
    m = keys.numel()
    dev = keys.device
    ptr, perm = _i32(rows + 1, dev), _i32(m, dev)
    cursor, perm_tmp, tmp = _i32(rows + 1, dev), _i32(m, dev), _i32((rows + 4095) // 4096 + 1, dev)
    lib.call('pamnet_csr_from_keys_i32', lib.ptr(keys), m, rows, lib.ptr(ptr), lib.ptr(perm), lib.ptr(cursor),
             lib.ptr(perm_tmp), lib.ptr(tmp), lib.stream_of(keys))
    return ptr, perm


def expand_rows(ptr, total, zeroed=False):
    rows = ptr.numel() - 1
    out = _alloc_i32(total, ptr.device, zeroed)
    lib.call('pamnet_expand_rows_i32', lib.ptr(ptr), rows, lib.ptr(out), int(total), lib.stream_of(ptr))
    return out


def host_ints(*scalars):
    import ctypes
    n = len(scalars)
    ts = [s.reshape(-1)[:1] for s in scalars]
    kinds = []
    for t in ts:
        if t.dtype == torch.int32:
            kinds.append(0)
        elif t.dtype in (torch.bool, torch.uint8):
            kinds.append(1)
        elif t.dtype == torch.int64:
            kinds.append(2)
        else:
            raise TypeError('host_ints: unsupported dtype %s' % t.dtype)
    out = torch.empty(n, dtype=torch.int64, device=ts[0].device)
    lib.call('pamnet_gather_scalars_i64', n, (ctypes.c_void_p * n)(*[t.data_ptr() for t in ts]),
             (ctypes.c_int32 * n)(*kinds), lib.ptr(out), lib.stream_of(out))
    return [int(v) for v in out.tolist()]


def _filter_count(ptr_in, nbr, dist, cut):
    rows = ptr_in.numel() - 1
    count = _i32(rows, nbr.device)
    lib.call('pamnet_csr_filter_count_i32', lib.ptr(ptr_in), lib.ptr(nbr), lib.ptr(dist), rows, float(cut),
             lib.ptr(count), lib.stream_of(nbr))
    return exclusive_scan(count)


def _filter_fill(ptr_in, nbr, dist, cut, ptr, total, zeroed=False):
    rows = ptr_in.numel() - 1
    nbr_out, dist_out = _alloc_i32(total, nbr.device, zeroed), _alloc_f32(total, nbr.device, zeroed)
    lib.call('pamnet_csr_filter_fill_i32', lib.ptr(ptr_in), lib.ptr(nbr), lib.ptr(dist), rows, float(cut),
             lib.ptr(ptr), lib.ptr(nbr_out), lib.ptr(dist_out), int(total), lib.stream_of(nbr))
    return ptr, nbr_out, dist_out


def csr_filter(ptr_in, nbr, dist, cut, flag=None):
    ptr = _filter_count(ptr_in, nbr, dist, cut)
    if flag is None:
        return _filter_fill(ptr_in, nbr, dist, cut, ptr, int(ptr[-1]))
    total, bad = host_ints(ptr[-1], flag)
    if bad:
        _raise_bad_inputs()
    return _filter_fill(ptr_in, nbr, dist, cut, ptr, total)


def csr_filter2(ptr_in, nbr, dist, cut_a, cut_b, flag=None):
    pa, pb = _filter_count(ptr_in, nbr, dist, cut_a), _filter_count(ptr_in, nbr, dist, cut_b)
    if flag is None:
        ta, tb = host_ints(pa[-1], pb[-1])
    else:
        ta, tb, bad = host_ints(pa[-1], pb[-1], flag)
        if bad:
            _raise_bad_inputs()
    return _filter_fill(ptr_in, nbr, dist, cut_a, pa, ta), _filter_fill(ptr_in, nbr, dist, cut_b, pb, tb)


def edge_dist(pos, a, b):
    out = _f32(a.numel(), pos.device)
    lib.call('pamnet_edge_dist_f32', lib.ptr(pos), lib.ptr(a), lib.ptr(b), a.numel(), lib.ptr(out), lib.stream_of(pos))
    return out


class CSR(object):
    __slots__ = ('ptr', 'row_of', 'col', 'm', 'rows')

    def __init__(self, ptr, row_of, col):
        self.ptr, self.row_of, self.col = ptr, row_of, col
        self.m, self.rows = int(row_of.numel()), int(ptr.numel() - 1)


class Transpose(object):
    __slots__ = ('ptr', 'perm', 'rows')

    def __init__(self, idx, rows):
        self.ptr, self.perm = csr_from_keys(idx, rows)
        self.rows = rows


class _Given(object):
    __slots__ = ('ptr', 'perm', 'rows')

    def __init__(self, ptr, perm, rows):
        self.ptr, self.perm, self.rows = ptr, perm, rows


class SymmetricTranspose(object):
    __slots__ = ('ptr', 'perm', 'rows')

    def __init__(self, csr):
        self.ptr, self.rows = csr.ptr, csr.rows
        self.perm = _i32(csr.m, csr.ptr.device)
        lib.call('pamnet_reverse_edges_i32', lib.ptr(csr.ptr), lib.ptr(csr.row_of), lib.ptr(csr.col), csr.m,
                 lib.ptr(self.perm), None, lib.stream_of(csr.ptr))


class _NoTransposeT(object):
    ptr = perm = None


_NoTranspose = _NoTransposeT()


class Graph(object):

    capped = False
    pos_grad = False

    @property
    def trip_rows(self):
        if '_trip_rows' not in self.__dict__:
            self._trip_rows = (self.tp_kind == 0).nonzero().view(-1)
        return self._trip_rows

    @property
    def pair_rows(self):
        if '_pair_rows' not in self.__dict__:
            self._pair_rows = (self.tp_kind == 1).nonzero().view(-1)
        return self._pair_rows

    @property
    def n_trip(self):
        return int(self.trip_rows.numel())

    @property
    def n_pair(self):
        return int(self.pair_rows.numel())


def radius_count(pos, node_graph, gptr, r, max_neighbors=0, cap_flag=None):
    n = pos.size(0)
    count = _i32(n, pos.device)
    lib.call('pamnet_radius_count_i32', lib.ptr(pos), lib.ptr(node_graph), lib.ptr(gptr), n, int(gptr.numel()) - 1,
             float(r), int(max_neighbors or 0), lib.ptr(count), lib.ptr(cap_flag), lib.stream_of(pos))
    return exclusive_scan(count)


def radius_fill(pos, node_graph, gptr, r, ptr, total, zeroed=False, rows_out=None, max_neighbors=0):
    nbr = _alloc_i32(total, pos.device, zeroed)
    dist = _alloc_f32(total, pos.device, zeroed)
    row_of = _alloc_i32(total, pos.device, zeroed) if rows_out is not None else None
    lib.call('pamnet_radius_fill_i32', lib.ptr(pos), lib.ptr(node_graph), lib.ptr(gptr), pos.size(0), int(gptr.numel()) - 1,
             float(r), int(max_neighbors or 0), lib.ptr(ptr), lib.ptr(nbr), lib.ptr(dist), lib.ptr(row_of), int(total),
             lib.stream_of(pos))
    if rows_out is not None:
        rows_out.append(row_of)
    return ptr, nbr, dist


def radius_graph(pos, node_graph, gptr, r):
    ptr = radius_count(pos, node_graph, gptr, r)
    return radius_fill(pos, node_graph, gptr, r, ptr, int(ptr[-1]))


def knn_table(pos, node_graph, gptr, k, cutoff):
    n = pos.size(0)
    nbr, dist = _i32(n * k, pos.device), _f32(n * k, pos.device)
    lib.call('pamnet_knn_i32', lib.ptr(pos), lib.ptr(node_graph), lib.ptr(gptr), n, k, float(cutoff), lib.ptr(nbr),
             lib.ptr(dist), lib.stream_of(pos))
    ptr = (torch.arange(n + 1, device=pos.device, dtype=torch.int64) * k).to(I32)
    return ptr, nbr, dist


KNN_TP_TOTAL = os.environ.get('PAMNET_KNN_TP_TOTAL', '0') != '0'


def knn_cuts(pos, node_graph, gptr, k, cut_a, cut_b, flag=None, tp_of_b=None):
    n, dev = int(pos.size(0)), pos.device
    st = lib.stream_of(pos)
    kn, kd = _i32(n * k, dev), _f32(n * k, dev)
    cnt = _i32(2 * n + 2 * (n + 1) + (n + 4095) // 4096 + 1, dev)
    ca, cb, ra, rb, tmp = cnt[:n], cnt[n:2 * n], cnt[2 * n:3 * n + 1], cnt[3 * n + 1:4 * n + 2], cnt[4 * n + 2:]
    lib.call('pamnet_knn_cut_i32', lib.ptr(pos), lib.ptr(node_graph), lib.ptr(gptr), n, int(k), float(cut_a), float(cut_b),
             lib.ptr(kn), lib.ptr(kd), lib.ptr(ca), lib.ptr(cb), st)
    lib.call('pamnet_exclusive_scan_pair_i32', lib.ptr(ca), lib.ptr(ra), lib.ptr(cb), lib.ptr(rb), n, lib.ptr(tmp), st)
    want = [ra[-1], rb[-1]]
    if tp_of_b is not None:
        buf = torch.zeros((n + 1) // 2 + 1, dtype=torch.int64, device=dev)
        tot = buf[-1:]
        lib.call('pamnet_knn_tp_total_i64', lib.ptr(kn), lib.ptr(kd), n, int(k), float(cut_b), 1 if tp_of_b else 0,
                 lib.ptr(buf), lib.ptr(tot), st)
        want.append(tot)
    if flag is not None:
        want.append(flag)
    got = host_ints(*want)
    ta, tb = got[0], got[1]
    tp_total = got[2] if tp_of_b is not None else None
    if flag is not None and got[-1]:
        _raise_bad_inputs()
    outs = [(_i32(t, dev), _f32(t, dev), _i32(t, dev), _i32(n + 1, dev)) for t in (ta, tb)]
    lib.call('pamnet_knn_cut_fill_i32', lib.ptr(kn), lib.ptr(kd), n, int(k), float(cut_a), lib.ptr(ra), ta, lib.ptr(outs[0][0]),
             lib.ptr(outs[0][1]), lib.ptr(outs[0][2]), lib.ptr(outs[0][3]), float(cut_b), lib.ptr(rb), tb, lib.ptr(outs[1][0]),
             lib.ptr(outs[1][1]), lib.ptr(outs[1][2]), lib.ptr(outs[1][3]), st)
    res = tuple((o[3], o[0], o[1], o[2]) for o in outs)
    return res if tp_of_b is None else res + (tp_total,)


class InverseTranspose(object):
    __slots__ = ('ptr', 'perm', 'rows')

    def __init__(self, ptr, inv):
        self.ptr, self.perm, self.rows = ptr, inv, int(ptr.numel() - 1)


def _transpose_edges(ptr, nbr, dist, n, zeroed=False, want_inverse=False, q=None):
    total = int(nbr.numel())
    if q is None:
        q = expand_rows(ptr, total, zeroed=zeroed)
    tptr, perm = csr_from_keys(nbr, n)
    out_q, out_d = _i32(total, nbr.device), _f32(total, nbr.device)
    inv = _i32(total, nbr.device) if want_inverse else None
    lib.call('pamnet_transpose_gather_i32', lib.ptr(perm), lib.ptr(q), lib.ptr(dist), total, lib.ptr(out_q), lib.ptr(out_d),
             lib.ptr(inv), lib.stream_of(nbr))
    return tptr, out_q, out_d, (InverseTranspose(ptr, inv) if want_inverse else None)


def _triplet_ptr(lp, l_src, l_dst, with_triplets):
    e_l = l_src.numel()
    tcount, tpcount = _i32(e_l, l_src.device), _i32(e_l, l_src.device)
    lib.call('pamnet_triplet_count_i32', lib.ptr(lp), lib.ptr(l_src), lib.ptr(l_dst), e_l, 1 if with_triplets else 0,
             lib.ptr(tcount), lib.ptr(tpcount), lib.stream_of(l_src))
    return exclusive_scan(tpcount), tcount


class TripletTranspose(object):
    __slots__ = ('ptr', 'perm', 'rows')

    def __init__(self, loc, loc_T, tp_ptr, tcount, total, with_triplets, zeroed=False):
        e_l, dev = loc.m, loc.ptr.device
        st = lib.stream_of(loc.ptr)
        wt = 1 if with_triplets else 0
        cnt = _i32(e_l, dev)
        lib.call('pamnet_triplet_transpose_count_i32', lib.ptr(loc.ptr), lib.ptr(loc.col), lib.ptr(loc.row_of), lib.ptr(loc_T.ptr),
                 lib.ptr(loc_T.perm), e_l, wt, lib.ptr(cnt), st)
        self.ptr = exclusive_scan(cnt)
        if zeroed:
            self.ptr = torch.clamp(self.ptr, max=total)
        self.perm = _alloc_i32(total, dev, zeroed)
        lib.call('pamnet_triplet_transpose_fill_i32', lib.ptr(loc.ptr), lib.ptr(loc.col), lib.ptr(loc.row_of), lib.ptr(loc_T.ptr),
                 lib.ptr(loc_T.perm), e_l, wt, lib.ptr(tp_ptr), lib.ptr(tcount), lib.ptr(self.ptr), lib.ptr(self.perm), total, st)
        self.rows = max(e_l, 1)


def _input_flag(node_graph, n_graphs, types=None, n_types=None, src=None, dst=None):
    flag = _i32(1, node_graph.device)
    ne = 0 if src is None else int(src.numel())
    stride = 0
    if types is not None and n_types is not None:
        assert types.dtype == torch.float32 and types.dim() == 1
        stride = types.stride(0) if types.numel() > 1 else 1
    else:
        types = None
    lib.call('pamnet_validate_inputs_i32', lib.ptr(node_graph), node_graph.numel(), int(n_graphs),
             None if types is None else types.data_ptr(), stride, int(n_types or 0), lib.ptr(src) if ne else None,
             lib.ptr(dst) if ne else None, ne, lib.ptr(flag), lib.stream_of(node_graph))
    return flag


_KINDS = {torch.int64: 1, torch.int32: 2, torch.float32: 3}


def ingest(batch, n_graphs, x=None, n_types=None, edge_index=None):
    n = int(batch.numel())
    if batch.dtype not in _KINDS or not batch.is_contiguous() or batch.dim() != 1:
        return None
    xk, xs, xcol = 0, 1, None
    if x is not None and n_types is not None:
        xcol = x.reshape(-1) if (x.dim() == 1 or (x.dim() == 2 and x.size(1) == 1)) else None
        if xcol is None or xcol.dtype not in _KINDS or xcol.numel() != n:
            return None
        xk, xs = _KINDS[xcol.dtype], (xcol.stride(0) if n > 1 else 1)
        if xs < 1:
            return None
    ne, ek, es, ed = 0, 0, None, None
    if edge_index is not None:
        if edge_index.dim() != 2 or edge_index.size(0) != 2 or edge_index.dtype not in _KINDS:
            return None
        es, ed = edge_index[0], edge_index[1]
        if not (es.is_contiguous() and ed.is_contiguous()):
            return None
        ne, ek = int(es.numel()), _KINDS[edge_index.dtype]
    dev = batch.device
    na, ea = (n + 3) // 4 * 4, (ne + 3) // 4 * 4
    buf = _i32(2 * na + 2 * ea + n_graphs + 7, dev)
    node_graph, types = buf[:n], buf[na:na + n]
    src, dst = buf[2 * na:2 * na + ne], buf[2 * na + ea:2 * na + ea + ne]
    gf = buf[2 * na + 2 * ea:]
    lib.call('pamnet_ingest_indices_i32', batch.data_ptr() if n else None, _KINDS[batch.dtype], n, int(n_graphs),
             xcol.data_ptr() if (xk and n) else None, xk, xs, int(n_types or 1), es.data_ptr() if ne else None,
             ed.data_ptr() if ne else None, ek, ne, node_graph.data_ptr() if n else None, gf.data_ptr(),
             types.data_ptr() if n else None, src.data_ptr() if ne else None, dst.data_ptr() if ne else None,
             lib.stream_of(batch))
    return node_graph, gf[:n_graphs + 1], (types if xk else None), src, dst, gf[n_graphs + 1:n_graphs + 2], \
        gf[n_graphs + 2:n_graphs + 3], gf[n_graphs + 3:n_graphs + 7]


def _check_sizes(flag, checks, all_kept=None, loops=None):
    import ctypes
    n = len(checks)
    actual = (ctypes.c_void_p * n)(*[lib.ptr(t) for t, _ in checks])
    expected = (ctypes.c_int64 * n)(*[int(v) for _, v in checks])
    lib.call('pamnet_check_sizes_i32', n, actual, expected, None if all_kept is None else lib.ptr(all_kept),
             None if loops is None else lib.ptr(loops), lib.ptr(flag), lib.stream_of(flag))


CAP_BIT = 64


def _raise_bad_inputs():
    raise IndexError('index out of range in the batch handed to PAMNet.forward: `batch` must be sorted with ids in '
                     '[0, num_graphs), atom types in [0, embeddings.size(0)), edge_index in [0, num_nodes)')


class GraphCheckError(IndexError):
    pass


_CHECK_STREAMS = {}


def read_flags(flags, completed=False):
    if not flags:
        return 0
    if completed and flags[0].is_cuda:
        dev = flags[0].device
        st = _CHECK_STREAMS.get(dev)
        if st is None:
            st = _CHECK_STREAMS[dev] = torch.cuda.Stream(device=dev)
        with torch.cuda.stream(st):
            vals = torch.stack(flags).reshape(-1).tolist()
    else:
        vals = torch.stack(flags).reshape(-1).tolist()
    bits = 0
    for v in vals:
        bits |= int(v)
    return bits


def raise_for_flag(bits):
    if bits & 1:
        _raise_bad_inputs()
    if bits:
        what = [n for k, n in ((1, 'global edges'), (2, 'local edges'), (3, 'triplet / pair rows'), (4, 'size 4')) if bits & (2 << k - 1)]
        if bits & 32:
            what.append('self loops in edge_index')
        if bits & CAP_BIT:
            raise GraphCheckError('max_num_neighbors binds in this batch (a node has more points within cutoff_g than the '
                                  'radius search keeps, models.py:110,128,301): the one-call graph assumes symmetric radius '
                                  'graphs -- hand the batch over without `sizes` (the plain path builds the capped graph)')
        raise GraphCheckError('the data-dependent sizes handed to PAMNet.forward (`data.sizes`) do not match the batch: '
                              + ', '.join(what) + ' -- results of this batch are invalid')


ENGINE = __import__('os').environ.get('PAMNET_GRAPH_ENGINE', '1') != '0'
MOL_LOCAL = True
KNN_K = 50
MOL_ATOMS, MOL_BONDS = 64, 256


class _Facade(object):

    def __init__(self, g, fields, m, rows):
        self.__dict__['_g'], self.__dict__['_fields'] = g, fields
        self.m, self.rows = int(m), int(rows)

    def __getattr__(self, name):
        spec = self.__dict__['_fields'].get(name)
        if spec is None:
            raise AttributeError(name)
        v = self.__dict__['_g']._view(*spec)
        self.__dict__[name] = v
        return v


class EngineGraph(Graph):

    def _view(self, field, count, is_float=False):
        off = self._layout[field]
        if off < 0:
            return None
        v = self._arena[off:off + int(count)]
        return v.view(torch.float32) if is_float else v

    def _addr(self, field):
        off = self._layout[field]
        return None if off < 0 else self._base + 4 * off

    def __getattr__(self, name):
        mk = self.__dict__.get('_lazy', {}).get(name)
        if mk is None:
            raise AttributeError(name)
        v = mk()
        self.__dict__[name] = v
        return v


_SCHEMA = {'QM9': 0, 'PDBbind': 1, 'rna': 2}


def _engine_graph(dataset, cutoff_l, cutoff_g, flow, x_raw, batch, pos, edge_index, n_graphs, need_grad, knn_k,
                  with_triplets, n_types, sizes, default_basis=True, mol_local=False, max_nb=0, aux_tables=True):
    import ctypes
    rna = dataset[:3].lower() == 'rna'
    n = int(batch.numel())
    eg, el, tp = (int(v) for v in sizes)
    if not (ENGINE and batch.is_cuda and n > 0 and min(eg, el, tp) > 0 and batch.dim() == 1 and batch.is_contiguous()
            and batch.dtype in _KINDS):
        return None
    d = lib.GraphDesc()
    d.n, d.n_graphs, d.eg, d.el, d.tp = n, int(n_graphs), eg, el, tp
    d.batch, d.batch_kind = batch.data_ptr(), _KINDS[batch.dtype]
    d.with_triplets, d.knn_k = (1 if with_triplets else 0), int(knn_k)
    d.need_grad = (1 if aux_tables else 2) if need_grad else 0
    d.cutoff_l, d.cutoff_g = float(cutoff_l), float(cutoff_g)
    d.max_neighbors = int(max_nb)
    d.n_types = int(n_types or 0)
    keep = [batch]
    if dataset == 'QM9':
        if pos is None or edge_index is None or n_types is None:
            return None
        xcol = x_raw.reshape(-1) if (x_raw.dim() == 1 or (x_raw.dim() == 2 and x_raw.size(1) == 1)) else None
        if xcol is None or xcol.dtype not in _KINDS or xcol.numel() != n:
            return None
        if edge_index.dim() != 2 or edge_index.size(0) != 2 or edge_index.dtype not in _KINDS:
            return None
        es, ed = edge_index[0], edge_index[1]
        if not (es.is_contiguous() and ed.is_contiguous()) or int(es.numel()) != el:
            return None
        pos = pos if (pos.dtype == torch.float32 and pos.is_contiguous()) else pos.to(torch.float32).contiguous()
        d.schema, d.n_bonds = 0, el
        d.mol_local = 1 if (mol_local and MOL_LOCAL and not 0 < max_nb <= MOL_ATOMS) else 0
        d.types, d.types_kind, d.types_stride = xcol.data_ptr(), _KINDS[xcol.dtype], (xcol.stride(0) if n > 1 else 1)
        d.pos, d.edge_src, d.edge_dst, d.edge_kind = pos.data_ptr(), es.data_ptr(), ed.data_ptr(), _KINDS[edge_index.dtype]
        keep += [xcol, pos, edge_index]
    else:
        if x_raw.dim() != 2 or x_raw.dtype != torch.float32 or not x_raw.is_contiguous() or x_raw.size(1) < 4:
            return None
        w = int(x_raw.size(1))
        d.rows, d.rows_width, d.n_bonds = x_raw.data_ptr(), w, 0
        if rna:
            if n_types is None or not 1 <= int(knn_k) <= 64:
                return None
            d.schema, d.types, d.types_kind, d.types_stride = 2, x_raw.data_ptr() + 4 * (w - 1), 3, w
            d.aggregate_at_query = 1 if flow == 'target_to_source' else 0
        elif dataset == 'PDBbind':
            if not cutoff_l <= cutoff_g:
                return None
            d.schema = 1
        else:
            return None
        keep.append(x_raw)
    layout = (ctypes.c_int64 * lib.GRAPH_FIELDS)()
    need = ctypes.c_int64(0)
    lib.call('pamnet_graph_plan', ctypes.addressof(d), ctypes.addressof(layout), ctypes.addressof(need))
    dev = batch.device
    arena = torch.empty(int(need.value), dtype=I32, device=dev)
    sbf = torch.empty((tp, 42), dtype=torch.float32, device=dev) if default_basis else None
    lib.call('pamnet_graph_build_i32', ctypes.addressof(d), arena.data_ptr(), lib.ptr(sbf), lib.stream_of(batch))
    F = lib.GF
    g = EngineGraph()
    g._arena, g._layout, g._base, g._inputs = arena, list(layout), arena.data_ptr(), keep
    g.n, g.n_graphs, g.need_grad_built = n, int(n_graphs), bool(need_grad)
    g.sbf, g._sbf_cutoff = sbf, float(cutoff_l)
    g.check = g._view(F['FLAG'], 1)
    g.pos = pos if dataset == 'QM9' else None
    ng = int(n_graphs)
    lazy = {
        'node_graph': lambda: g._view(F['NODE_GRAPH'], n), 'gptr': lambda: g._view(F['GPTR'], ng + 1),
        'types': lambda: g._view(F['TYPES'], n), 'sign': lambda: g._view(F['SIGN'], n, True),
        'loops': lambda: g._view(F['LOOPS'], 1),
        'dist_g': lambda: g._view(F['G_DIST'], eg, True), 'dist_l': lambda: g._view(F['L_DIST'], el, True),
        'tp_angle': lambda: g._view(F['T_ANGLE'], tp, True), 'tp_kind': lambda: g._view(F['T_KIND'], tp),
        'cuts': lambda: g._view(F['CUTS'], 257),
        'glob': lambda: _Facade(g, {'ptr': (F['G_PTR'], n + 1), 'row_of': (F['G_ROW'], eg), 'col': (F['G_COL'], eg)}, eg, n),
        'loc': lambda: _Facade(g, {'ptr': (F['L_PTR'], n + 1), 'row_of': (F['L_ROW'], el), 'col': (F['L_COL'], el)}, el, n),
        'tp': lambda: _Facade(g, {'ptr': (F['T_PTR'], el + 1), 'row_of': (F['T_ROW'], tp), 'col': (F['T_COL'], tp)}, tp, el),
    }
    if dataset != 'QM9':
        lazy['pos'] = lambda: g._view(F['POS'], 3 * n, True).view(n, 3)
        del g.__dict__['pos']
    if need_grad:
        lazy['glob_T'] = lambda: _Facade(g, {'ptr': (F['GT_PTR'], n + 1), 'perm': (F['GT_PERM'], eg)}, eg, n)
        lazy['loc_T'] = lambda: _Facade(g, {'ptr': (F['LT_PTR'], n + 1), 'perm': (F['LT_PERM'], el)}, el, n)
        lazy['tp_T'] = lambda: _Facade(g, {'ptr': (F['TT_PTR'], el + 1), 'perm': (F['TT_PERM'], tp)}, tp, el)
    else:
        g.glob_T = g.loc_T = g.tp_T = _NoTranspose
    g.__dict__['_lazy'] = lazy
    order = ('G_PTR', 'G_ROW', 'G_COL', 'GT_PTR', 'GT_PERM', 'L_PTR', 'L_ROW', 'L_COL', 'LT_PTR', 'LT_PERM',
             'T_PTR', 'T_ROW', 'T_COL', 'TT_PTR', 'TT_PERM', 'CUTS', 'TT_EDGE', 'TT_NODE')
    idx = (ctypes.c_void_p * 18)()
    for k, name in enumerate(order):
        idx[k] = g._addr(F[name])
    g._tables = ((ctypes.c_int64 * 4)(n, eg, el, tp), idx)
    g._sizes = (n, eg, el, tp)
    return g


def _mol_local_graph(g, pos, ing, cutoff_g, with_triplets, need_grad, cutoff_l=None):
    import ctypes
    node_graph, gptr, _, src0, dst0, flag, loops, totals = ing
    dev = pos.device
    free = cutoff_l is not None
    n, ng, m = g.n, g.n_graphs, int(src0.numel())
    st = lib.stream_of(pos)
    mol_tot = _i32(4 * ng, dev)
    wt = 1 if with_triplets else 0
    if free:
        lib.call('pamnet_mol_graph_free_count_i32', lib.ptr(pos), lib.ptr(gptr), n, ng, float(cutoff_l), float(cutoff_g), wt,
                 lib.ptr(mol_tot), lib.ptr(totals), st)
    else:
        lib.call('pamnet_mol_graph_count_i32', lib.ptr(pos), lib.ptr(gptr), n, ng, lib.ptr(src0), lib.ptr(dst0), m,
                 float(cutoff_g), wt, lib.ptr(mol_tot), lib.ptr(totals), st)
    eg, tp, viol, counted, bad, lp_ = host_ints(totals[0], totals[1], totals[2], totals[3], flag, loops)
    if bad:
        _raise_bad_inputs()
    if free:
        m = counted
    if viol or lp_ or counted != m or eg <= 0 or tp <= 0:
        return False
    def carve(sizes):
        offs, tot = [], 0
        for k in sizes:
            offs.append(tot)
            tot += (k + 3) // 4 * 4
        buf = _i32(tot, dev)
        return [buf[o:o + k] for o, k in zip(offs, sizes)]

    (g_ptr, l_ptr, lT_ptr, l_row, l_col, lT_perm, t_ptr, tT_ptr, g_row, g_col, gT_perm, t_row, t_col, t_kind,
     tT_perm) = carve([n + 1] * 3 + [m] * 3 + [m + 1] * 2 + [eg] * 3 + [tp] * 4)
    l_dist, g_dist, t_angle = _f32(m, dev), _f32(eg, dev), _f32(tp, dev)
    o = lib.MolGraphOut()
    o.g_ptr, o.g_row, o.g_col, o.g_dist = g_ptr.data_ptr(), g_row.data_ptr(), g_col.data_ptr(), g_dist.data_ptr()
    o.l_ptr, o.l_row, o.l_col, o.l_dist = l_ptr.data_ptr(), l_row.data_ptr(), l_col.data_ptr(), l_dist.data_ptr()
    o.t_ptr, o.t_row, o.t_col = t_ptr.data_ptr(), t_row.data_ptr(), t_col.data_ptr()
    o.t_angle, o.t_kind = t_angle.data_ptr(), t_kind.data_ptr()
    if need_grad:
        o.gT_perm, o.lT_ptr, o.lT_perm = gT_perm.data_ptr(), lT_ptr.data_ptr(), lT_perm.data_ptr()
        o.tT_ptr, o.tT_perm = tT_ptr.data_ptr(), tT_perm.data_ptr()
    if free:
        lib.call('pamnet_mol_graph_free_fill_i32', lib.ptr(pos), lib.ptr(gptr), n, ng, m, float(cutoff_l), float(cutoff_g), wt,
                 1 if need_grad else 0, lib.ptr(mol_tot), eg, tp, ctypes.addressof(o), st)
    else:
        lib.call('pamnet_mol_graph_fill_i32', lib.ptr(pos), lib.ptr(gptr), n, ng, lib.ptr(src0), lib.ptr(dst0), m,
                 float(cutoff_g), wt, 1 if need_grad else 0, lib.ptr(mol_tot), eg, tp, ctypes.addressof(o), st)
    g.loops = loops
    g.pos = pos
    g.glob, g.dist_g = CSR(g_ptr, g_row, g_col), g_dist
    g.loc, g.dist_l = CSR(l_ptr, l_row, l_col), l_dist
    g.tp = CSR(t_ptr, t_row, t_col)
    g.tp_angle, g.tp_kind = t_angle, t_kind
    g.glob_T = g.loc_T = g.tp_T = _NoTranspose
    if need_grad:
        g.glob_T = _Given(g_ptr, gT_perm, n)
        g.loc_T = _Given(lT_ptr, lT_perm, n)
        g.tp_T = _Given(tT_ptr, tT_perm, max(m, 1))
    return True


def build_graph(dataset, cutoff_l, cutoff_g, flow, x_raw, batch, pos=None, edge_index=None, num_graphs=None,
                need_grad=True, knn_k=None, with_triplets=True, n_types=None, sizes=None, default_basis=True, mol_local=None,
                max_num_neighbors=None, aux_tables=True):
    dev = batch.device
    max_nb = int(max_num_neighbors or 0)
    capped = False
    knn_k = KNN_K if knn_k is None else int(knn_k)
    if sizes is not None and knn_k != KNN_K:
        raise ValueError('host-side sizes (store.MoleculeStore) are counted for k = %d neighbours; got knn_k = %d' % (KNN_K, knn_k))
    if sizes is not None and num_graphs is not None:
        eng = _engine_graph(dataset, cutoff_l, cutoff_g, flow, x_raw, batch, pos, edge_index, num_graphs, need_grad, knn_k,
                            with_triplets, n_types, sizes, default_basis, mol_local=bool(mol_local), max_nb=max_nb,
                            aux_tables=aux_tables)
        if eng is not None:
            return eng
    g = Graph()
    n = int(batch.numel())
    g.n = n
    g.n_graphs = int(num_graphs) if num_graphs is not None else int(batch[-1]) + 1
    g.types = None
    rna = dataset[:3].lower() == 'rna'
    ing = None
    if batch.is_cuda and n > 0:
        if dataset == 'QM9':
            if n_types is not None:
                ing = ingest(batch, g.n_graphs, x_raw, n_types, edge_index)
        elif rna and n_types is not None and x_raw.dim() == 2:
            ing = ingest(batch, g.n_graphs, x_raw[:, -1], n_types)
        elif rna or dataset == 'PDBbind':
            ing = ingest(batch, g.n_graphs)
    if ing is not None:
        node_graph, g.gptr, g.types = ing[0], ing[1], ing[2]
    else:
        node_graph = batch.to(I32).contiguous()
        g.gptr, _ = csr_from_keys(node_graph, g.n_graphs)
    g.node_graph = node_graph
    g.sign = None
    g.check = None
    tp_pre = None
    tp_hint = None
    hinted = False
    checks = []
    glob_rows = []
    glob_inv = loc_inv = None
    loc_radius = False

    if dataset == 'QM9' and edge_index is None:
        pos = pos.to(torch.float32).contiguous()
        if ing is not None:
            flag = ing[5]
        else:
            flag = _input_flag(node_graph, g.n_graphs, x_raw.to(torch.float32).reshape(-1), n_types)
        if (sizes is None and ing is not None and MOL_LOCAL and mol_local is not False
                and not 0 < max_nb <= MOL_ATOMS
                and (mol_local is True or n <= MOL_ATOMS * g.n_graphs // 2)):
            if _mol_local_graph(g, pos, ing, cutoff_g, with_triplets, need_grad, cutoff_l=cutoff_l):
                return _with_seg_cuts(g, dataset) if aux_tables else g
        gptr_g = radius_count(pos, node_graph, g.gptr, cutoff_g, max_nb, flag)
        lp = radius_count(pos, node_graph, g.gptr, cutoff_l)
        if sizes is not None:
            total_g, total_l, tp_hint = (int(v) for v in sizes)
            g.check = flag
            checks += [(gptr_g[-1:], total_g), (lp[-1:], total_l)]
            hinted = _ZeroArena(3 * total_g + 3 * total_l + 5 * tp_hint + 64, dev)
            gptr_g, lp = torch.clamp(gptr_g, max=total_g), torch.clamp(lp, max=total_l)
        else:
            deg = (lp[1:] - lp[:-1]).long()
            tp_dev = (deg * deg + (deg * (deg - 1) if with_triplets else 0)).sum()
            total_g, total_l, tp_hint, bad = host_ints(gptr_g[-1], lp[-1], tp_dev, flag)
            if bad & ~CAP_BIT:
                _raise_bad_inputs()
            capped = bool(bad & CAP_BIT)
        gp, gn, gd = radius_fill(pos, node_graph, g.gptr, cutoff_g, gptr_g, total_g, zeroed=hinted, rows_out=glob_rows,
                                 max_neighbors=max_nb)
        if capped and flow != 'target_to_source':
            gp, gn, gd, glob_inv = _transpose_edges(gp, gn, gd, n, want_inverse=need_grad, q=glob_rows.pop())
        loc_rows = []
        lp, l_src, l_dist = radius_fill(pos, node_graph, g.gptr, cutoff_l, lp, total_l, zeroed=hinted, rows_out=loc_rows)
        l_dst = loc_rows[0]
        loc_radius = True
    elif dataset == 'QM9':
        pos = pos.to(torch.float32).contiguous()
        def bonds(ei, raw=None):
            src0, dst0 = raw if raw is not None else (ei[0].to(I32).contiguous(), ei[1].to(I32).contiguous())
            bonds.raw = (src0, dst0)
            lp_, perm = csr_from_keys(dst0, n)
            m = int(src0.numel())
            src_, dst_, bonds.dist = _i32(m, dev), _i32(m, dev), _f32(m, dev)
            lib.call('pamnet_gather2_i32', lib.ptr(perm), lib.ptr(src0), lib.ptr(dst0), m, lib.ptr(src_), lib.ptr(dst_),
                     lib.ptr(pos), lib.ptr(bonds.dist), lib.stream_of(src0))
            tp_, bonds.tcount = _triplet_ptr(lp_, src_, dst_, with_triplets)
            return lp_, src_, dst_, tp_

        ei = edge_index
        if (sizes is None and ing is not None and MOL_LOCAL and mol_local is not False and ei.size(1) > 0
                and not 0 < max_nb <= MOL_ATOMS
                and (mol_local is True or n <= MOL_ATOMS * g.n_graphs // 2)):
            done = _mol_local_graph(g, pos, ing, cutoff_g, with_triplets, need_grad)
            if done:
                return _with_seg_cuts(g, dataset) if aux_tables else g
        lp, l_src, l_dst, tp_ptr = bonds(ei, None if ing is None else (ing[3], ing[4]))
        if ing is not None:
            flag, kept = ing[5], ing[6]
            g.loops = kept
        else:
            types = x_raw.to(torch.float32).reshape(-1)
            flag = _input_flag(node_graph, g.n_graphs, types, n_types, *bonds.raw)
            kept = (ei[0] != ei[1]).all()
        gptr_g = radius_count(pos, node_graph, g.gptr, cutoff_g, max_nb, flag)
        if sizes is not None:
            total_g, tp_total = int(sizes[0]), int(sizes[2])
            checks += [(gptr_g[-1:], total_g), (lp[-1:], int(sizes[1])), (tp_ptr[-1:], tp_total)]
            g.check = flag
            if ing is None:
                g.all_kept = kept
            hinted = _ZeroArena(3 * total_g + 5 * tp_total + 64, dev)
            gptr_g = torch.clamp(gptr_g, max=total_g)
            tp_ptr = torch.clamp(tp_ptr, max=tp_total)
        else:
            total_g, k, tp_total, bad = host_ints(gptr_g[-1], kept, tp_ptr[-1], flag)
            if bad & ~CAP_BIT:
                _raise_bad_inputs()
            capped = bool(bad & CAP_BIT)
            if (k != 0) if ing is not None else (not k):
                lp, l_src, l_dst, tp_ptr = bonds(ei[:, ei[0] != ei[1]])
                tp_total = int(tp_ptr[-1])
        gp, gn, gd = radius_fill(pos, node_graph, g.gptr, cutoff_g, gptr_g, total_g, zeroed=hinted, rows_out=glob_rows,
                                 max_neighbors=max_nb)
        if capped and flow != 'target_to_source':
            gp, gn, gd, glob_inv = _transpose_edges(gp, gn, gd, n, want_inverse=need_grad, q=glob_rows.pop())
        l_dist = bonds.dist
        tp_pre = (tp_ptr, tp_total)
    elif dataset == 'PDBbind':
        xr = x_raw.unsqueeze(-1) if x_raw.dim() == 1 else x_raw
        pos = xr[:, :3].to(torch.float32).contiguous()
        g.sign = torch.where(pos[:, 0] > 40.0, -torch.ones_like(pos[:, 0]), torch.ones_like(pos[:, 0])).contiguous()
        pflag = ing[5] if ing is not None else _input_flag(node_graph, g.n_graphs)
        gptr_g = radius_count(pos, node_graph, g.gptr, cutoff_g, max_nb, pflag)
        local = cutoff_l <= cutoff_g
        if local and sizes is not None:
            lp = radius_count(pos, node_graph, g.gptr, cutoff_l)
            total_g, total_l, tp_hint = (int(v) for v in sizes)
            g.check = pflag
            checks += [(gptr_g[-1:], total_g), (lp[-1:], total_l)]
            hinted = _ZeroArena(3 * total_g + 3 * total_l + 5 * tp_hint + 64, dev)
            gptr_g, lp = torch.clamp(gptr_g, max=total_g), torch.clamp(lp, max=total_l)
            gp, gn, gd = radius_fill(pos, node_graph, g.gptr, cutoff_g, gptr_g, total_g, zeroed=hinted, rows_out=glob_rows)
            lp, l_src, l_dist = _filter_fill(gp, gn, gd, cutoff_l, lp, total_l, zeroed=hinted)
        elif local:
            lp = radius_count(pos, node_graph, g.gptr, cutoff_l)
            deg = (lp[1:] - lp[:-1]).long()
            tp_dev = (deg * deg + (deg * (deg - 1) if with_triplets else 0)).sum()
            total_g, total_l, tp_total, bad = host_ints(gptr_g[-1], lp[-1], tp_dev, pflag)
            if bad & ~CAP_BIT:
                _raise_bad_inputs()
            capped = bool(bad & CAP_BIT)
            gp, gn, gd = radius_fill(pos, node_graph, g.gptr, cutoff_g, gptr_g, total_g, rows_out=glob_rows,
                                     max_neighbors=max_nb)
            if capped:
                lp, l_src, l_dist = csr_filter(gp, gn, gd, cutoff_l)
                tp_hint = None
                cap_rows = glob_rows.pop()
            else:
                lp, l_src, l_dist = _filter_fill(gp, gn, gd, cutoff_l, lp, total_l)
                tp_hint = tp_total
        else:
            total_g, bad = host_ints(gptr_g[-1], pflag)
            if bad & ~CAP_BIT:
                _raise_bad_inputs()
            capped = bool(bad & CAP_BIT)
            gp, gn, gd = radius_fill(pos, node_graph, g.gptr, cutoff_g, gptr_g, total_g, max_neighbors=max_nb)
            lp, l_src, l_dist = csr_filter(gp, gn, gd, cutoff_l)
            tp_hint = None
            cap_rows = None
        if capped:
            lp, l_src, l_dist, loc_inv = _transpose_edges(lp, l_src, l_dist, n, want_inverse=need_grad)
            if flow != 'target_to_source':
                gp, gn, gd, glob_inv = _transpose_edges(gp, gn, gd, n, want_inverse=need_grad, q=cap_rows)
        l_dst = expand_rows(lp, l_src.numel(), zeroed=hinted)
    elif rna:
        xr = x_raw.unsqueeze(-1) if x_raw.dim() == 1 else x_raw
        pos = xr[:, :3].to(torch.float32).contiguous()
        flag = ing[5] if ing is not None else _input_flag(node_graph, g.n_graphs, xr[:, -1].to(torch.float32), n_types)
        gq = qq = None
        if sizes is not None:
            kp, kn, kd = knn_table(pos, node_graph, g.gptr, knn_k, float('inf'))
            total_g, total_l, tp_hint = (int(v) for v in sizes)
            pa, pb = _filter_count(kp, kn, kd, cutoff_g), _filter_count(kp, kn, kd, cutoff_l)
            g.check = flag
            checks += [(pa[-1:], total_g), (pb[-1:], total_l)]
            hinted = _ZeroArena(4 * total_g + 4 * total_l + 5 * tp_hint + 64, dev)
            pa, pb = torch.clamp(pa, max=total_g), torch.clamp(pb, max=total_l)
            gp, gn, gd = _filter_fill(kp, kn, kd, cutoff_g, pa, total_g, zeroed=hinted)
            qp, qn, qd = _filter_fill(kp, kn, kd, cutoff_l, pb, total_l, zeroed=hinted)
        elif n > 0 and knn_k <= 64:
            if KNN_TP_TOTAL:
                (gp, gn, gd, gq), (qp, qn, qd, qq), tp_hint = knn_cuts(pos, node_graph, g.gptr, knn_k, cutoff_g, cutoff_l, flag,
                                                                        tp_of_b=bool(with_triplets))
            else:
                (gp, gn, gd, gq), (qp, qn, qd, qq) = knn_cuts(pos, node_graph, g.gptr, knn_k, cutoff_g, cutoff_l, flag)
        else:
            kp, kn, kd = knn_table(pos, node_graph, g.gptr, knn_k, float('inf'))
            (gp, gn, gd), (qp, qn, qd) = csr_filter2(kp, kn, kd, cutoff_g, cutoff_l, flag)
        if flow != 'target_to_source':
            gp, gn, gd, glob_inv = _transpose_edges(gp, gn, gd, n, zeroed=hinted, want_inverse=need_grad, q=gq)
            gq = None
        elif gq is not None:
            glob_rows.append(gq)
        lp, l_src, l_dist, loc_inv = _transpose_edges(qp, qn, qd, n, zeroed=hinted, want_inverse=need_grad, q=qq)
        l_dst = expand_rows(lp, l_src.numel(), zeroed=hinted)
    else:
        raise ValueError("Invalid dataset. If you are using any dataset related to RNA 3D structure prediction, "
                         "be sure to use 'rna' as the first 3 characters of the dataset name.")

    g.pos = pos
    g.glob = CSR(gp, glob_rows[0] if glob_rows else expand_rows(gp, gn.numel(), zeroed=hinted), gn)
    g.dist_g = gd
    g.loc = CSR(lp, l_dst, l_src)
    g.dist_l = l_dist

    e_l = g.loc.m
    st = lib.stream_of(pos)
    wt = 1 if with_triplets else 0
    if tp_pre is None:
        tp_ptr, tcount = _triplet_ptr(lp, l_src, l_dst, with_triplets)
        tot = tp_hint if tp_hint is not None else int(tp_ptr[-1])
        if hinted:
            checks.append((tp_ptr[-1:], tot))
            tp_ptr = torch.clamp(tp_ptr, max=tot)
    else:
        tp_ptr, tot = tp_pre
        tcount = bonds.tcount
    tp_idx, tp_edge, tp_kind = (_alloc_i32(tot, dev, hinted) for _ in range(3))
    tp_angle = _alloc_f32(tot, dev, hinted)
    lib.call('pamnet_triplet_fill_f32', lib.ptr(pos), lib.ptr(lp), lib.ptr(l_src), lib.ptr(l_dst), e_l, wt,
             lib.ptr(tp_ptr), lib.ptr(tp_idx), lib.ptr(tp_edge), lib.ptr(tp_angle), lib.ptr(tp_kind), tot, st)
    if checks:
        _check_sizes(g.check, checks, getattr(g, 'all_kept', None), getattr(g, 'loops', None))
    g.tp = CSR(tp_ptr, tp_edge, tp_idx)
    g.tp_angle, g.tp_kind = tp_angle, tp_kind

    g.capped = capped
    g.glob_T = g.loc_T = g.tp_T = _NoTranspose
    if need_grad:
        radius_g = dataset in ('QM9', 'PDBbind') and not capped
        g.glob_T = SymmetricTranspose(g.glob) if radius_g else (glob_inv if glob_inv is not None
                                                               else Transpose(g.glob.col, n))
        g.loc_T = SymmetricTranspose(g.loc) if ((dataset == 'PDBbind' and not capped) or loc_radius) else (
            loc_inv if loc_inv is not None else Transpose(g.loc.col, n))
        g.tp_T = (TripletTranspose(g.loc, g.loc_T, tp_ptr, tcount, tot, with_triplets, zeroed=hinted) if (e_l > 0 and tot > 0)
                  else Transpose(tp_idx, max(e_l, 1)))
    return _with_seg_cuts(g, dataset) if aux_tables else g


def _with_seg_cuts(g, dataset):
    if dataset in ('QM9', 'PDBbind') and g.n > 0:
        g.seg_cuts = _i32(260, g.glob.ptr.device)
        lib.call('pamnet_seg_cuts_i32', lib.ptr(g.glob.ptr), lib.ptr(g.glob.row_of), g.n, g.glob.m, lib.ptr(g.seg_cuts), None,
                 lib.stream_of(g.glob.ptr))
        if g.tp_T is not _NoTranspose and g.tp.m > 0 and g.loc.m > 0:
            dev = g.glob.ptr.device
            g.tT_edge, g.tT_node = _i32(g.tp.m, dev), _i32(g.tp.m, dev)
            lib.call('pamnet_triplet_transpose_aux_i32', lib.ptr(g.tp_T.perm), lib.ptr(g.tp.row_of), lib.ptr(g.loc.row_of), g.tp.m,
                     lib.ptr(g.tT_edge), lib.ptr(g.tT_node), lib.stream_of(g.glob.ptr))
    return g


def spherical_basis_tab(g, cutoff_l, num_spherical, num_radial, envelope_exponent, zeros, norm):
    dev = g.pos.device
    st = lib.stream_of(g.pos)
    e_l, tot, w = g.loc.m, g.tp.m, int(num_spherical) * int(num_radial)
    if not (zeros.dtype == torch.float32 and norm.dtype == torch.float64 and zeros.numel() == w and norm.numel() == w
            and zeros.device == dev and norm.device == dev):
        raise TypeError('spherical basis tables: zeros must be float32 [%d], norm float64 [%d], both on %s (got %s %s on %s, '
                        '%s %s on %s)' % (w, w, dev, zeros.dtype, tuple(zeros.shape), zeros.device, norm.dtype,
                                          tuple(norm.shape), norm.device))
    rad = _f32(e_l * w, dev)
    lib.call('pamnet_sbf_radial_tab_f32', lib.ptr(g.dist_l), float(cutoff_l), e_l, int(num_spherical), int(num_radial),
             int(envelope_exponent), lib.ptr(zeros), lib.ptr(norm), lib.ptr(rad), st)
    sbf = torch.empty((tot, w), dtype=torch.float32, device=dev)
    lib.call('pamnet_sbf_combine_tab_f32', lib.ptr(rad), lib.ptr(g.tp.col), lib.ptr(g.tp_angle), tot, int(num_spherical),
             int(num_radial), lib.ptr(sbf), st)
    return sbf


def spherical_basis(g, cutoff_l):
    if getattr(g, '_sbf_cutoff', None) == float(cutoff_l) and g.__dict__.get('sbf') is not None:
        return g.sbf
    dev = g.pos.device
    st = lib.stream_of(g.pos)
    e_l = g.loc.m
    rad = _f32(e_l * 42, dev)
    lib.call('pamnet_sbf_radial_f32', lib.ptr(g.dist_l), float(cutoff_l), e_l, lib.ptr(rad), st)
    tot = g.tp.m
    sbf = torch.empty((tot, 42), dtype=torch.float32, device=dev)
    lib.call('pamnet_sbf_combine_f32', lib.ptr(rad), lib.ptr(g.tp.col), lib.ptr(g.tp_angle), tot, lib.ptr(sbf), st)
    return sbf


_SECOND_ORDER = ('PAMNet: second derivatives through the positions are not supported (the kernels\' backward passes are not '
                 'themselves differentiable): torch.autograd.grad(..., create_graph=True) cannot give forces with a grad_fn')


def _index_lists(g):
    glob, loc, tp = g.glob, g.loc, g.tp
    return (g.n, glob.ptr, glob.row_of, glob.col, g.glob_T.ptr, g.glob_T.perm, glob.m, loc.ptr, loc.row_of, loc.col,
            g.loc_T.ptr, g.loc_T.perm, loc.m, tp.ptr, tp.row_of, tp.col, g.tp_kind, g.tp_T.ptr, g.tp_T.perm, tp.m)


class _Geometry(torch.autograd.Function):

    @staticmethod
    def forward(ctx, pos, g):
        ctx.save_for_backward(pos)
        ctx.idx = _index_lists(g)
        return g.dist_g.clone(), g.dist_l.clone(), g.tp_angle.clone()

    @staticmethod
    def backward(ctx, d_dg, d_dl, d_ang):
        if torch.is_grad_enabled():
            raise RuntimeError(_SECOND_ORDER)
        pos, = ctx.saved_tensors
        (n, g_ptr, g_row, g_col, gt_ptr, gt_perm, eg, l_ptr, l_row, l_col, lt_ptr, lt_perm, el, t_ptr, t_row, t_col, t_kind,
         tt_ptr, tt_perm, tp) = ctx.idx
        pos = pos.contiguous()
        d_dg, d_dl, d_ang = d_dg.contiguous(), d_dl.contiguous(), d_ang.contiguous()
        work = torch.empty(3 * max(el, 1), dtype=torch.float64, device=pos.device)
        dpos = torch.empty((n, 3), dtype=torch.float32, device=pos.device)
        lib.call('pamnet_pos_bwd_f32', lib.ptr(pos), n, lib.ptr(g_ptr), lib.ptr(g_row), lib.ptr(g_col), lib.ptr(gt_ptr),
                 lib.ptr(gt_perm), lib.ptr(d_dg), eg, lib.ptr(l_ptr), lib.ptr(l_row), lib.ptr(l_col), lib.ptr(lt_ptr),
                 lib.ptr(lt_perm), lib.ptr(d_dl), el, lib.ptr(t_ptr), lib.ptr(t_row), lib.ptr(t_col), lib.ptr(t_kind),
                 lib.ptr(tt_ptr), lib.ptr(tt_perm), lib.ptr(d_ang), tp, lib.ptr(work), lib.ptr(dpos), lib.stream_of(pos))
        return dpos, None


class _SphericalBasis(torch.autograd.Function):

    @staticmethod
    def forward(ctx, dist_l, angle, g, cutoff_l, sbf):
        ctx.save_for_backward(dist_l, angle)
        ctx.idx = (g.tp.col, g.tp_T.ptr, g.tp_T.perm, g.loc.m, g.tp.m)
        ctx.cutoff = float(cutoff_l)
        return sbf.clone()

    @staticmethod
    def backward(ctx, gs):
        if torch.is_grad_enabled():
            raise RuntimeError(_SECOND_ORDER)
        dist_l, angle = ctx.saved_tensors
        t_col, tt_ptr, tt_perm, e_l, tot = ctx.idx
        gs = gs.contiguous()
        rad = torch.empty(max(e_l, 1) * 42, dtype=torch.float32, device=gs.device)
        dangle, ddist = torch.empty_like(angle), torch.empty_like(dist_l)
        lib.call('pamnet_sbf_bwd_f32', lib.ptr(gs), lib.ptr(dist_l), ctx.cutoff, e_l, lib.ptr(t_col), lib.ptr(angle), tot,
                 lib.ptr(tt_ptr), lib.ptr(tt_perm), lib.ptr(rad), lib.ptr(dangle), lib.ptr(ddist), lib.stream_of(gs))
        return ddist, dangle, None, None, None


class _DiffGraph(object):

    pos_grad = True

    def __init__(self, g, **geometry):
        self.__dict__.update(geometry)
        self.__dict__['_plain'] = g

    def __getattr__(self, name):
        return getattr(self.__dict__['_plain'], name)


def differentiable_geometry(g, pos, cutoff_l):
    if g.glob_T is _NoTranspose or g.loc_T is _NoTranspose or g.tp_T is _NoTranspose:
        raise RuntimeError('differentiable geometry needs a graph built with need_grad=True')
    dist_g, dist_l, angle = _Geometry.apply(pos, g)
    sbf = _SphericalBasis.apply(dist_l, angle, g, cutoff_l, g.sbf)
    return _DiffGraph(g, dist_g=dist_g, dist_l=dist_l, tp_angle=angle, sbf=sbf)
```

physics-aware-multiplex-gnn_amd/pamnet_amd/lib.py:

```python
import ctypes
import os
import re

HERE = os.path.dirname(os.path.abspath(__file__))
LIB_PATH = os.environ.get('PAMNET_HIP_LIB') or os.path.join(HERE, 'libpamnet_hip.so')
HEADER = os.path.join(os.path.dirname(os.path.dirname(HERE)), 'include', 'pamnet_hip.h')

_lib = None
_CT = {'float*': ctypes.c_void_p, 'int32_t*': ctypes.c_void_p, 'void*': ctypes.c_void_p,
       'int64_t': ctypes.c_int64, 'int32_t': ctypes.c_int32, 'float': ctypes.c_float, 'double': ctypes.c_double,
       'pamnet_stream_t': ctypes.c_void_p, 'int': ctypes.c_int}


def declared_functions(header=HEADER):
    text = open(header).read()
    text = re.sub(r'/\*.*?\*/', '', text, flags=re.S)
    out = {}
    for m in re.finditer(r'\bint\s+(pamnet_\w+)\s*\(([^)]*)\)\s*;', text):
        name, args = m.group(1), m.group(2).strip()
        types = []
        if args and args != 'void':
            for a in args.split(','):
                a = a.replace('const', ' ').strip()
                if '*' in a:
                    types.append(ctypes.c_void_p)
                else:
                    types.append(_CT[a.rsplit(None, 1)[0].strip()])
        out[name] = types
    return out


def load():
    global _lib
    if _lib is None:
        if not os.path.exists(LIB_PATH):
            raise RuntimeError('libpamnet_hip.so is not built (%s). Run `python __graft_entry__.py` or '
                               'pamnet_amd.build.build(); there is no CPU fallback.' % LIB_PATH)
        import torch
        lib = ctypes.CDLL(LIB_PATH)
        for name, types in declared_functions().items():
            fn = getattr(lib, name)
            fn.argtypes = types
            fn.restype = ctypes.c_int
        want = int(re.search(r'#define\s+PAMNET_ABI_VERSION\s+(\d+)', open(HEADER).read()).group(1))
        lib.pamnet_abi_version.argtypes = []
        got = int(lib.pamnet_abi_version())
        if got != want:
            raise RuntimeError('libpamnet_hip.so was built for ABI version %d, include/pamnet_hip.h declares %d: rebuild '
                               '(python __graft_entry__.py)' % (got, want))
        if os.environ.get('PAMNET_HIP_LIB'):
            import warnings
            warnings.warn('pamnet_amd: PAMNET_HIP_LIB is set -- kernels come from %s (ABI %d), not from the in-tree build %s'
                          % (LIB_PATH, got, os.path.join(HERE, 'libpamnet_hip.so')), RuntimeWarning, stacklevel=2)
        _lib = lib
    return _lib


def check(rc, name):
    if rc != 0:
        kind = {-1: 'PAMNET_EINVAL (bad size / unsupported width)', -2: 'PAMNET_ENULL (null pointer)'}.get(
            rc, 'hipError_t %d' % rc)
        raise RuntimeError('%s failed: %s' % (name, kind))


_EMPTY = {}


def ptr(t):
    if t is None:
        return None
    p = t.data_ptr()
    if not t.is_contiguous():
        raise AssertionError('pamnet_hip: tensor must be contiguous')
    if p == 0 and t.is_cuda:
        import torch
        if t.device not in _EMPTY:
            _EMPTY[t.device] = torch.zeros(64, dtype=torch.float32, device=t.device)
        return _EMPTY[t.device].data_ptr()
    return p


_raw_stream = None


def stream_of(t):
    global _raw_stream
    if not t.is_cuda:
        raise RuntimeError('pamnet_hip kernels run on an MI355X only: tensor is on %s (no CPU fallback)' % t.device)
    if _raw_stream is None:
        import torch
        _raw_stream = getattr(torch._C, '_cuda_getCurrentRawStream', None) or \
            (lambda idx: torch.cuda.current_stream(idx).cuda_stream)
    return _raw_stream(t.device.index)


_fns = {}


def call(name, *args):
    fn = _fns.get(name)
    if fn is None:
        fn = _fns[name] = getattr(load(), name)
    rc = fn(*args)
    if rc:
        check(rc, name)


_P = ctypes.c_void_p


class EmbedJob(ctypes.Structure):
    _fields_ = [('x', _P), ('dist', _P), ('freq', _P), ('cutoff', ctypes.c_float), ('K', ctypes.c_int32),
                ('act', ctypes.c_int32), ('rows', ctypes.c_int64), ('kind', _P), ('W0', _P), ('b0', _P), ('W1', _P),
                ('b1', _P), ('out', _P), ('gout', _P), ('dW0', _P), ('db0', _P), ('dW1', _P), ('db1', _P), ('dfreq', _P),
                ('dx', _P), ('partial', _P)]


class TypeRowsJob(ctypes.Structure):
    _fields_ = [('table', _P), ('idx', _P), ('n', ctypes.c_int64), ('n_types', ctypes.c_int64), ('out', _P), ('g', _P),
                ('scratch', _P), ('dtable', _P)]


class GraphDesc(ctypes.Structure):
    _fields_ = [('n', ctypes.c_int64), ('n_graphs', ctypes.c_int64), ('n_bonds', ctypes.c_int64),
                ('eg', ctypes.c_int64), ('el', ctypes.c_int64), ('tp', ctypes.c_int64),
                ('batch', _P), ('types', _P), ('types_stride', ctypes.c_int64), ('n_types', ctypes.c_int64),
                ('pos', _P), ('rows', _P), ('rows_width', ctypes.c_int64), ('edge_src', _P), ('edge_dst', _P),
                ('schema', ctypes.c_int32), ('batch_kind', ctypes.c_int32), ('types_kind', ctypes.c_int32),
                ('edge_kind', ctypes.c_int32), ('with_triplets', ctypes.c_int32), ('need_grad', ctypes.c_int32),
                ('aggregate_at_query', ctypes.c_int32), ('knn_k', ctypes.c_int32),
                ('cutoff_l', ctypes.c_float), ('cutoff_g', ctypes.c_float), ('max_neighbors', ctypes.c_int32),
                ('mol_local', ctypes.c_int32)]


class MolGraphOut(ctypes.Structure):
    _fields_ = [(k, _P) for k in ('g_ptr', 'g_row', 'g_col', 'g_dist', 'gT_perm', 'l_ptr', 'l_row', 'l_col', 'l_dist',
                                  'lT_ptr', 'lT_perm', 't_ptr', 't_row', 't_col', 't_angle', 't_kind', 'tT_ptr', 'tT_perm')]


GF = {name: i for i, name in enumerate(
    ['NODE_GRAPH', 'GPTR', 'FLAG', 'LOOPS', 'TYPES', 'POS', 'SIGN', 'G_PTR', 'G_ROW', 'G_COL', 'G_DIST', 'GT_PTR', 'GT_PERM',
     'L_PTR', 'L_ROW', 'L_COL', 'L_DIST', 'LT_PTR', 'LT_PERM', 'T_PTR', 'T_ROW', 'T_COL', 'T_ANGLE', 'T_KIND', 'TT_PTR',
     'TT_PERM', 'CUTS', 'TT_EDGE', 'TT_NODE'])}
GRAPH_FIELDS = len(GF)
```

Before: 70040 molecules/s.

## Fuse SBF basis, seg cuts and triplet aux tables into per-molecule graph fill kernel

The per-molecule graph builder is split into a single-wave count kernel and a 256-thread fill kernel that share a prepared LDS state. The fill kernel now also emits segment cuts, triplet-transpose aux tables and the spherical Bessel basis (radial values kept in shared memory), which removes the separate radial, combine, seg-cuts and aux-transpose launches and their global round-trips on the QM9 molecule path. The count path also skips prefix scans it does not need, and the host readback of totals now uses one pinned copy instead of gathering scalars. In exchange the fill kernel uses much more LDS per block, which may limit occupancy.

```diff
diff --git a/include/pamnet_hip.h b/include/pamnet_hip.h
--- a/include/pamnet_hip.h
+++ b/include/pamnet_hip.h
@@ -159,6 +159,10 @@
     float* t_angle;
     int32_t* t_kind;
     int32_t *tT_ptr, *tT_perm;
+    int32_t* cuts;
+    int32_t *tT_edge, *tT_node;
+    float* sbf;
+    float sbf_cutoff;
 } pamnet_mol_graph_out;
 int pamnet_mol_graph_count_i32(const float* pos, const int32_t* gptr, int64_t n, int64_t n_graphs, const int32_t* src,
                                const int32_t* dst, int64_t n_bonds, float cutoff_g, int32_t with_triplets, int32_t* mol_tot,
diff --git a/physics-aware-multiplex-gnn_amd/csrc/basis.hip b/physics-aware-multiplex-gnn_amd/csrc/basis.hip
--- a/physics-aware-multiplex-gnn_amd/csrc/basis.hip
+++ b/physics-aware-multiplex-gnn_amd/csrc/basis.hip
@@ -1,5 +1,6 @@
 #include "common.h"
 #include "basis_constants.h"
+#include "sbf_core.h"
 
 namespace {
 
@@ -7,54 +8,6 @@
     if (!(x < 1.0f)) return 0.0f;
     const float x2 = x * x, x5 = x2 * x2 * x;
     return 1.0f / x + x5 * (-21.0f + x * (35.0f - 15.0f * x));
-}
-
-__device__ __forceinline__ double envelope_d(double x) {
-    if (!(x < 1.0)) return 0.0;
-    const double x2 = x * x, x5 = x2 * x2 * x;
-    return 1.0 / x + x5 * (-21.0 + x * (35.0 - 15.0 * x));
-}
-
-constexpr int SERIES_TERMS = 28;
-struct SeriesTab {
-    double c[7][SERIES_TERMS + 1];
-    double inv_dfact[7];
-};
-constexpr SeriesTab make_series() {
-    SeriesTab t{};
-    for (int l = 0; l < 7; ++l) {
-        t.c[l][0] = 1.0;
-        for (int k = 1; k <= SERIES_TERMS; ++k) t.c[l][k] = t.c[l][k - 1] * -0.5 / ((double)k * (double)(2 * l + 2 * k + 1));
-        double d = 1.0;
-        for (int m = 1; m <= l; ++m) d *= (double)(2 * m + 1);
-        t.inv_dfact[l] = 1.0 / d;
-    }
-    return t;
-}
-__device__ __constant__ SeriesTab SBF_SERIES = make_series();
-
-__device__ __forceinline__ double sph_jl(int l, double z) {
-    if (z < (double)l + 1.0) {
-        const double h = z * z;
-        double sum = SBF_SERIES.c[l][SERIES_TERMS];
-#pragma unroll
-        for (int k = SERIES_TERMS - 1; k >= 0; --k) sum = fma(sum, h, SBF_SERIES.c[l][k]);
-        double pref = SBF_SERIES.inv_dfact[l];
-        for (int m = 0; m < l; ++m) pref *= z;
-        return pref * sum;
-    }
-    double s, c;
-    sincos(z, &s, &c);
-    const double iz = 1.0 / z;
-    double jm = s * iz;
-    if (l == 0) return jm;
-    double j = (jm - c) * iz;
-    for (int m = 1; m < l; ++m) {
-        const double jn = (double)(2 * m + 1) * iz * j - jm;
-        jm = j;
-        j = jn;
-    }
-    return j;
 }
 
 __global__ __launch_bounds__(256) void rbf_fwd_kernel(const float* __restrict__ dist, const float* __restrict__ freq,
@@ -123,9 +76,7 @@
     const int64_t t = (int64_t)blockIdx.x * blockDim.x + threadIdx.x;
     if (t >= m * 42) return;
     const int64_t e = t / 42;
-    const int c = (int)(t - e * 42), l = c / 6;
-    const double x = (double)(dist[e] * inv_cutoff);
-    rad[t] = (float)(envelope_d(x) * PAMNET_SBF_NORM[c] * sph_jl(l, (double)PAMNET_SBF_ZEROS_F32[c] * x));
+    rad[t] = sbf_radial_value(dist[e], inv_cutoff, (int)(t - e * 42));
 }
 
 constexpr int SBF_ROWS = 64;
@@ -138,17 +89,7 @@
     const int64_t row0 = (int64_t)blockIdx.x * SBF_ROWS;
     const int tid = threadIdx.x;
     if (tid < SBF_ROWS && row0 + tid < m) {
-        const double ct = cos((double)angle[row0 + tid]);
-        double p0 = 1.0, p1 = ct;
-        ylm[tid][0] = PAMNET_YL0_PREF[0] * p0;
-        ylm[tid][1] = PAMNET_YL0_PREF[1] * p1;
-#pragma unroll
-        for (int k = 2; k <= 6; ++k) {
-            const double pl = ((double)(2 * k - 1) * ct * p1 - (double)(k - 1) * p0) / (double)k;
-            p0 = p1;
-            p1 = pl;
-            ylm[tid][k] = PAMNET_YL0_PREF[k] * pl;
-        }
+        sbf_yl0(angle[row0 + tid], ylm[tid]);
         src[tid] = idx[row0 + tid];
     }
     __syncthreads();
@@ -158,7 +99,7 @@
     float* out = sbf + row0 * 42 + tid;
 #pragma unroll 4
     for (int r = r0; r < rows; r += 6, out += 252)
-        *out = (float)((double)rad[(int64_t)src[r] * 42 + c] * ylm[r][l]);
+        *out = sbf_product(rad[(int64_t)src[r] * 42 + c], ylm[r][l]);
 }
 
 __device__ __forceinline__ double envelope_gen_d(double x, int p) {
diff --git a/physics-aware-multiplex-gnn_amd/csrc/graph_engine.hip b/physics-aware-multiplex-gnn_amd/csrc/graph_engine.hip
--- a/physics-aware-multiplex-gnn_amd/csrc/graph_engine.hip
+++ b/physics-aware-multiplex-gnn_amd/csrc/graph_engine.hip
@@ -124,6 +124,10 @@
     }
     const int64_t cur_a = r.take(n + 2), cur_b = r.take(n + 2), cur_c = r.take(n + 2);
     const int64_t tT_perm_z = grad ? r.take(tp) : -1;
+    const bool mol = d.schema == PAMNET_SCHEMA_QM9 && d.mol_local != 0;
+    const bool aux = d.need_grad == 1 && grad && tp > 0;
+    const int64_t cuts = r.take(260);
+    const int64_t tT_edge_z = mol && aux ? r.take(tp) : -1, tT_node_z = mol && aux ? r.take(tp) : -1;
     const int64_t z1 = r.off;
     if (!r.dry) {
         const hipError_t e = hipMemsetAsync(r.I(z0), 0, sizeof(int32_t) * (size_t)(z1 - z0), as_stream(r.stream));
@@ -151,7 +155,6 @@
 
     int64_t tT_ptr = -1, tT_perm = -1;
     const int64_t mol_totals = gf + ng + 3;
-    const bool mol = d.schema == PAMNET_SCHEMA_QM9 && d.mol_local != 0;
     if (mol) {
         l_row = r.take(el), l_col = r.take(el), l_dist = r.take(el);
         l_ptr = r.take(n + 1), g_ptr = r.take(n + 1), t_ptr = r.take(el + 1);
@@ -172,6 +175,9 @@
                 o.gT_perm = r.I(gT_perm), o.lT_ptr = r.I(lT_ptr), o.lT_perm = r.I(lT_perm);
                 o.tT_ptr = r.I(tT_ptr), o.tT_perm = r.I(tT_perm);
             }
+            o.cuts = r.I(cuts);
+            if (aux) o.tT_edge = r.I(tT_edge_z), o.tT_node = r.I(tT_node_z);
+            if (r.sbf) o.sbf = r.sbf, o.sbf_cutoff = d.cutoff_l;
         }
         GO(pamnet_mol_graph_fill_i32(pos, gptr, n, ng, r.I(src0), r.I(dst0), d.n_bonds, d.cutoff_g, wt, grad ? 1 : 0,
                                      r.I(mol_tot), eg, tp, &o, r.stream));
@@ -289,19 +295,18 @@
                                              r.I(t_cnt), r.I(tT_ptr), r.I(tT_perm), tp, r.stream));
     }
 
-    int64_t tT_edge = -1, tT_node = -1;
-    if (d.need_grad == 1 && tT_perm >= 0 && tp > 0) {
+    int64_t tT_edge = tT_edge_z, tT_node = tT_node_z;
+    if (!mol && aux && tT_perm >= 0) {
         tT_edge = r.take(tp), tT_node = r.take(tp);
         GO(pamnet_triplet_transpose_aux_i32(r.I(tT_perm), r.I(t_row), r.I(l_row), tp, r.I(tT_edge), r.I(tT_node), r.stream));
     }
 
     const int64_t rad = r.take(el * RAD_W);
-    if (r.sbf) {
+    if (r.sbf && !mol) {
         GO(pamnet_sbf_radial_f32(r.F(l_dist), d.cutoff_l, el, r.F(rad), r.stream));
         GO(pamnet_sbf_combine_f32(r.F(rad), r.I(t_col), r.F(t_angle), tp, r.sbf, r.stream));
     }
-    const int64_t cuts = r.take(260);
-    GO(pamnet_seg_cuts_i32(r.I(g_ptr), r.I(g_row), n, eg, r.I(cuts), nullptr, r.stream));
+    if (!mol) GO(pamnet_seg_cuts_i32(r.I(g_ptr), r.I(g_row), n, eg, r.I(cuts), nullptr, r.stream));
 
     r.field(PAMNET_GF_G_PTR, g_ptr), r.field(PAMNET_GF_G_ROW, g_row), r.field(PAMNET_GF_G_COL, g_col);
     r.field(PAMNET_GF_G_DIST, g_dist), r.field(PAMNET_GF_GT_PTR, gT_ptr), r.field(PAMNET_GF_GT_PERM, gT_perm);
diff --git a/physics-aware-multiplex-gnn_amd/csrc/graph_mol.hip b/physics-aware-multiplex-gnn_amd/csrc/graph_mol.hip
--- a/physics-aware-multiplex-gnn_amd/csrc/graph_mol.hip
+++ b/physics-aware-multiplex-gnn_amd/csrc/graph_mol.hip
@@ -1,5 +1,6 @@
 #include "common.h"
 #include "geom_core.h"
+#include "sbf_core.h"
 
 namespace {
 
@@ -66,20 +67,27 @@
     }
 }
 
+__device__ __forceinline__ void wave_lds_sync() {
+    __builtin_amdgcn_fence(__ATOMIC_ACQ_REL, "wavefront");
+    __builtin_amdgcn_wave_barrier();
+}
+
+struct MolShared {
+    float px[MOL_ATOMS], py[MOL_ATOMS], pz[MOL_ATOMS];
+    int l_src[MOL_BONDS], l_dst[MOL_BONDS];
+    int lt[MOL_BONDS];
+    int lptr[MOL_ATOMS + 1], ltptr[MOL_ATOMS + 1];
+    int tptr[MOL_BONDS + 1], tcnt[MOL_BONDS];
+    int ttptr[MOL_BONDS];
+    int gex[MOL_ATOMS + 1];
+    unsigned long long adj[MOL_ATOMS];
+    long long eoff, toff;
+    int ok, nb, b0, eg_m, tp_m;
+};
+
 template <bool FILL, bool FREE>
-__global__ __launch_bounds__(64) void mol_graph_kernel(MolIn in, int32_t* __restrict__ mol_tot,
-                                                       int32_t* __restrict__ totals, pamnet_mol_graph_out out,
-                                                       int64_t eg_cap, int64_t tp_cap) {
-    __shared__ float px[MOL_ATOMS], py[MOL_ATOMS], pz[MOL_ATOMS];
-    __shared__ int l_src[MOL_BONDS], l_dst[MOL_BONDS];
-    __shared__ int lt[MOL_BONDS];
-    __shared__ int lptr[MOL_ATOMS + 1], ltptr[MOL_ATOMS + 1];
-    __shared__ int tptr[MOL_BONDS + 1], tcnt[MOL_BONDS];
-    __shared__ int gex[MOL_ATOMS];
-    __shared__ unsigned long long adj[MOL_ATOMS];
-    const int g = blockIdx.x, lane = threadIdx.x;
-    const int a0 = in.gptr[g], a1 = in.gptr[g + 1], na = a1 - a0;
-    const bool last = g == (int)in.n_graphs - 1;
+__device__ __forceinline__ bool mol_prepare(MolShared& S, const MolIn& in, int32_t* __restrict__ mol_tot,
+                                            int32_t* __restrict__ totals, int g, int lane, int a0, int na, bool last) {
     int b0 = 0, b1 = 0;
     int se = 0, st = 0;
     if constexpr (FILL && FREE) {
@@ -92,6 +100,7 @@
         b1 = last ? (int)in.n_bonds : mol_tot[4 * g + 6];
         for (int q = lane; q < g; q += 64) se += mol_tot[4 * q], st += mol_tot[4 * q + 1];
     } else {
+        const int a1 = a0 + na;
         bond_range(in.dst, (int)in.n_bonds, a0, a1, lane, b0, b1);
     }
     int nb = b1 - b0;
@@ -105,13 +114,13 @@
             mol_tot[4 * g + 3] = flags;
             atomicOr(&totals[2], flags);
         }
-        return;
+        return false;
     }
     float xi = 0.f, yi = 0.f, zi = 0.f;
     if (lane < na) {
         const int64_t a = a0 + lane;
         xi = in.pos[3 * a], yi = in.pos[3 * a + 1], zi = in.pos[3 * a + 2];
-        px[lane] = xi, py[lane] = yi, pz[lane] = zi;
+        S.px[lane] = xi, S.py[lane] = yi, S.pz[lane] = zi;
     }
     unsigned long long mask = 0ull, lmask = 0ull;
     if constexpr (FREE) {
@@ -125,13 +134,13 @@
                 mol_tot[4 * g + 3] = 2;
                 atomicOr(&totals[2], 2);
             }
-            return;
+            return false;
         }
         int w = linc - ldeg;
-        if (lane < na) lptr[lane] = w;
-        if (lane == 0) lptr[na] = nb;
+        if (lane < na) S.lptr[lane] = w;
+        if (lane == 0) S.lptr[na] = nb;
         for (unsigned long long m = lmask; m; m &= m - 1) {
-            l_src[w] = __ffsll((long long)m) - 1, l_dst[w] = lane;
+            S.l_src[w] = __ffsll((long long)m) - 1, S.l_dst[w] = lane;
             ++w;
         }
     }
@@ -161,24 +170,24 @@
                     const unsigned long long m = __ballot(hit);
                     if (hit) {
                         const int w = run + __popcll(m & ((1ull << lane) - 1ull));
-                        l_src[w] = bs[c], l_dst[w] = i;
+                        S.l_src[w] = bs[c], S.l_dst[w] = i;
                     }
                     run += __popcll(m);
                 }
             }
         }
-        if (lane < na) lptr[lane] = mine;
-        if (lane == 0) lptr[na] = nb;
-    }
-    __syncthreads();
+        if (lane < na) S.lptr[lane] = mine;
+        if (lane == 0) S.lptr[na] = nb;
+    }
+    wave_lds_sync();
     int ss[MOL_CHUNKS], sd[MOL_CHUNKS];
 #pragma unroll
     for (int c = 0; c < MOL_CHUNKS; ++c) {
         const int k = c * 64 + lane;
-        ss[c] = k < nb ? l_src[k] : -1;
-        sd[c] = k < nb ? l_dst[k] : -1;
-    }
-    {
+        ss[c] = k < nb ? S.l_src[k] : -1;
+        sd[c] = k < nb ? S.l_dst[k] : -1;
+    }
+    if constexpr (FILL) {
         int run = 0, mine = 0;
         for (int j = 0; j < na; ++j) {
             if (lane == j) mine = run;
@@ -187,13 +196,13 @@
                 if (c < nchunk) {
                     const bool hit = ss[c] == j;
                     const unsigned long long m = __ballot(hit);
-                    if (hit) lt[run + __popcll(m & ((1ull << lane) - 1ull))] = c * 64 + lane;
+                    if (hit) S.lt[run + __popcll(m & ((1ull << lane) - 1ull))] = c * 64 + lane;
                     run += __popcll(m);
                 }
             }
         }
-        if (lane < na) ltptr[lane] = mine;
-        if (lane == 0) ltptr[na] = nb;
+        if (lane < na) S.ltptr[lane] = mine;
+        if (lane == 0) S.ltptr[na] = nb;
     }
 
     int carry = 0;
@@ -205,23 +214,26 @@
             if (k < nb) {
                 const int j = ss[c], i = sd[c];
                 if (in.with_triplets)
-                    for (int q = lptr[j]; q < lptr[j + 1]; ++q) t += (l_src[q] != i) ? 1 : 0;
-                cnt = t + lptr[i + 1] - lptr[i];
-                tcnt[k] = t;
-            }
-            const int inc = wave_incl(cnt, lane);
-            if (k < nb) tptr[k] = carry + inc - cnt;
-            carry += __shfl(inc, 63, 64);
-        }
-    }
-    const int tp_m = carry;
+                    for (int q = S.lptr[j]; q < S.lptr[j + 1]; ++q) t += (S.l_src[q] != i) ? 1 : 0;
+                cnt = t + S.lptr[i + 1] - S.lptr[i];
+                if constexpr (FILL) S.tcnt[k] = t;
+            }
+            if constexpr (FILL) {
+                const int inc = wave_incl(cnt, lane);
+                if (k < nb) S.tptr[k] = carry + inc - cnt;
+                carry += __shfl(inc, 63, 64);
+            } else {
+                carry += cnt;
+            }
+        }
+    }
+    const int tp_m = FILL ? carry : wave_sum(carry);
 
     if constexpr (!FREE) radius_masks<false>(xi, yi, zi, lane, na, in.cutoff_g, 0.f, mask, lmask);
     const int deg = __popcll(mask);
-    const int ginc = wave_incl(deg, lane);
-    const int eg_m = __shfl(ginc, 63, 64);
-
-    if (!FILL) {
+
+    if constexpr (!FILL) {
+        const int eg_m = wave_sum(deg);
         if (lane == 0) {
             mol_tot[4 * g] = flags ? 0 : eg_m;
             mol_tot[4 * g + 1] = flags ? 0 : tp_m;
@@ -235,125 +247,240 @@
                 atomicAdd(&totals[3], nb);
             }
         }
-        return;
-    }
-    if (flags) return;
-    adj[lane] = mask;
-    gex[lane] = ginc - deg;
-
-    const int64_t eoff = wave_sum(se), toff = wave_sum(st);
+        return false;
+    } else {
+        if (flags) return false;
+        const int ginc = wave_incl(deg, lane);
+        const int eg_m = __shfl(ginc, 63, 64);
+        S.adj[lane] = mask;
+        S.gex[lane] = ginc - deg;
+        const long long eoff = wave_sum(se), toff = wave_sum(st);
+        if (lane == 0) {
+            S.gex[MOL_ATOMS] = eg_m;
+            S.tptr[nb] = tp_m;
+            S.eoff = eoff, S.toff = toff;
+            S.nb = nb, S.b0 = b0, S.eg_m = eg_m, S.tp_m = tp_m;
+        }
+        if (!in.need_grad) return true;
+        wave_lds_sync();
+        carry = 0;
+#pragma unroll
+        for (int c = 0; c < MOL_CHUNKS; ++c) {
+            if (c >= nchunk) continue;
+            const int q = c * 64 + lane;
+            const bool on = q < nb;
+            const int kq = on ? ss[c] : 0, jq = on ? sd[c] : 0;
+            const int ab = S.ltptr[jq], ae = in.with_triplets ? S.ltptr[jq + 1] : ab;
+            int cnt = 0;
+            if (on) {
+                for (int a = ab; a < ae; ++a) cnt += (S.l_dst[S.lt[a]] != kq) ? 1 : 0;
+                cnt += S.lptr[jq + 1] - S.lptr[jq];
+            }
+            const int inc = wave_incl(cnt, lane);
+            if (on) S.ttptr[q] = carry + inc - cnt;
+            carry += __shfl(inc, 63, 64);
+        }
+        return true;
+    }
+}
+
+template <bool FREE>
+__global__ __launch_bounds__(64) void mol_count_kernel(MolIn in, int32_t* __restrict__ mol_tot, int32_t* __restrict__ totals) {
+    __shared__ MolShared S;
+    const int g = blockIdx.x, lane = threadIdx.x;
+    const int a0 = in.gptr[g], na = in.gptr[g + 1] - a0;
+    mol_prepare<false, FREE>(S, in, mol_tot, totals, g, lane, a0, na, g == (int)in.n_graphs - 1);
+}
+
+__device__ __forceinline__ int edge_atom(const MolShared& S, int na, int e) {
+    int lo = 0, hi = na;
+    while (hi - lo > 1) {
+        const int mid = (lo + hi) >> 1;
+        if (S.gex[mid] <= e) lo = mid; else hi = mid;
+    }
+    return lo;
+}
+
+constexpr int SEG_GRID_MAX = 256;
+constexpr int FILL_THREADS = 256, FILL_ROWS = 128;
+
+template <bool FREE>
+__global__ __launch_bounds__(FILL_THREADS) void mol_fill_kernel(MolIn in, const int32_t* __restrict__ mol_tot,
+                                                                pamnet_mol_graph_out out, int64_t eg_cap, int64_t tp_cap,
+                                                                float inv_cutoff) {
+    __shared__ MolShared S;
+    __shared__ float rad[MOL_BONDS * 42];
+    __shared__ double ylm[FILL_ROWS][7];
+    __shared__ int rsrc[FILL_ROWS];
+    const int g = blockIdx.x, tid = threadIdx.x, lane = tid & 63, wave = tid >> 6;
+    const int a0 = in.gptr[g], na = in.gptr[g + 1] - a0;
+    const bool last = g == (int)in.n_graphs - 1;
+    if (wave == 0) {
+        const bool ok = mol_prepare<true, FREE>(S, in, const_cast<int32_t*>(mol_tot), nullptr, g, lane, a0, na, last);
+        if (lane == 0) S.ok = ok ? 1 : 0;
+    }
     __syncthreads();
-
-    if (lane < na) out.l_ptr[a0 + lane] = b0 + lptr[lane];
-    if (last && lane == 0) {
+    if (!S.ok) return;
+    const int nb = S.nb, b0 = S.b0, eg_m = S.eg_m, tp_m = S.tp_m;
+    const int64_t eoff = S.eoff, toff = S.toff;
+    const bool grad = in.need_grad != 0;
+    constexpr int TM = FILL_THREADS - 1;
+    const int r1 = (tid + FILL_THREADS - 64) & TM, r2 = (tid + FILL_THREADS - 128) & TM, r3 = (tid + FILL_THREADS - 192) & TM;
+
+    if (tid < nb) {
+        const int k = tid, j = S.l_src[k], i = S.l_dst[k];
+        out.l_row[b0 + k] = a0 + i;
+        out.l_col[b0 + k] = a0 + j;
+        out.l_dist[b0 + k] = dist3_xyz(S.px[i], S.py[i], S.pz[i], S.px[j], S.py[j], S.pz[j]);
+        const int64_t w = toff + S.tptr[k];
+        out.t_ptr[b0 + k] = (int32_t)(w < tp_cap ? w : tp_cap);
+    }
+    if (r1 < na) {
+        out.l_ptr[a0 + r1] = b0 + S.lptr[r1];
+        const int64_t w0 = eoff + S.gex[r1];
+        out.g_ptr[a0 + r1] = (int32_t)(w0 < eg_cap ? w0 : eg_cap);
+        if (grad) out.lT_ptr[a0 + r1] = b0 + S.ltptr[r1];
+    }
+    if (last && r1 == 64) {
         out.l_ptr[in.n] = (int32_t)in.n_bonds;
         out.g_ptr[in.n] = (int32_t)(eoff + eg_m < eg_cap ? eoff + eg_m : eg_cap);
         out.t_ptr[in.n_bonds] = (int32_t)(toff + tp_m < tp_cap ? toff + tp_m : tp_cap);
-    }
-#pragma unroll
-    for (int c = 0; c < MOL_CHUNKS; ++c) {
-        const int k = c * 64 + lane;
-        if (k >= nb) continue;
-        const int j = ss[c], i = sd[c];
-        const float pix = px[i], piy = py[i], piz = pz[i], pjx = px[j], pjy = py[j], pjz = pz[j];
-        out.l_row[b0 + k] = a0 + i;
-        out.l_col[b0 + k] = a0 + j;
-        out.l_dist[b0 + k] = dist3_xyz(pix, piy, piz, pjx, pjy, pjz);
-        int64_t w = toff + tptr[k];
-        out.t_ptr[b0 + k] = (int32_t)(w < tp_cap ? w : tp_cap);
-        if (in.with_triplets) {
-            for (int q = lptr[j]; q < lptr[j + 1]; ++q) {
-                const int kk = l_src[q];
-                if (kk == i) continue;
-                if (w < tp_cap) {
-                    out.t_col[w] = b0 + q;
-                    out.t_row[w] = b0 + k;
-                    out.t_kind[w] = 0;
-                    out.t_angle[w] = angle3(pjx - pix, pjy - piy, pjz - piz, px[kk] - pjx, py[kk] - pjy, pz[kk] - pjz);
+        if (grad) {
+            out.lT_ptr[in.n] = (int32_t)in.n_bonds;
+            out.tT_ptr[in.n_bonds] = (int32_t)(toff + tp_m < tp_cap ? toff + tp_m : tp_cap);
+        }
+    }
+    if (grad && r2 < nb) out.lT_perm[b0 + r2] = b0 + S.lt[r2];
+    if (out.cuts) {
+        const int64_t m = eg_cap;
+        const int64_t G = m > 16 * SEG_GRID_MAX ? SEG_GRID_MAX : (m > 16 ? (m + 15) / 16 : 1);
+        if (g == 0 && r2 == 64) out.cuts[0] = 0;
+        if (last && r2 == 65) out.cuts[G] = (int32_t)in.n;
+        if (m > 0) {
+            int64_t k0 = (eoff * G + m - 1) / m, k1 = ((eoff + eg_m) * G + m - 1) / m;
+            if (k0 < 1) k0 = 1;
+            if (k1 > G) k1 = G;
+            for (int64_t k = k0 + r2; k < k1; k += FILL_THREADS) {
+                const int64_t t = k * m / G;
+                const int i = edge_atom(S, na, (int)(t - eoff));
+                int64_t a = eoff + S.gex[i], b = eoff + S.gex[i + 1];
+                a = a < eg_cap ? a : eg_cap, b = b < eg_cap ? b : eg_cap;
+                out.cuts[k] = (t - a <= b - t) ? a0 + i : a0 + i + 1;
+            }
+            if (last)
+                for (int64_t k = k1 + r2; k < G; k += FILL_THREADS) out.cuts[k] = (int32_t)in.n;
+        }
+    }
+    if (grad && r3 < nb) {
+        const int q = r3, kq = S.l_src[q], jq = S.l_dst[q];
+        const int ab = S.ltptr[jq], ae = in.with_triplets ? S.ltptr[jq + 1] : ab, bb = S.lptr[jq], be = S.lptr[jq + 1];
+        int64_t w2 = toff + S.ttptr[q];
+        out.tT_ptr[b0 + q] = (int32_t)(w2 < tp_cap ? w2 : tp_cap);
+        int a = ab, b = bb;
+        while (true) {
+            while (a < ae && S.l_dst[S.lt[a]] == kq) ++a;
+            const int ea = a < ae ? S.lt[a] : 0x7fffffff, eb = b < be ? b : 0x7fffffff;
+            if (ea == 0x7fffffff && eb == 0x7fffffff) break;
+            int row, e;
+            if (ea < eb) {
+                const int ie = S.l_dst[ea];
+                int rank = 0;
+                for (int q2 = bb; q2 < q; ++q2) rank += (S.l_src[q2] != ie) ? 1 : 0;
+                row = S.tptr[ea] + rank;
+                e = ea;
+                ++a;
+            } else {
+                row = S.tptr[eb] + S.tcnt[eb] + (q - bb);
+                e = eb;
+                ++b;
+            }
+            if (w2 < tp_cap) {
+                out.tT_perm[w2] = (int32_t)(toff + row < tp_cap ? toff + row : tp_cap - 1);
+                if (out.tT_edge) out.tT_edge[w2] = b0 + e, out.tT_node[w2] = a0 + S.l_dst[e];
+            }
+            ++w2;
+        }
+    }
+    for (int e = tid; e < eg_m; e += FILL_THREADS) {
+        const int64_t w = eoff + e;
+        if (w >= eg_cap) break;
+        const int i = edge_atom(S, na, e);
+        unsigned long long mk = S.adj[i];
+        for (int r = e - S.gex[i]; r > 0; --r) mk &= mk - 1;
+        const int j = __ffsll((long long)mk) - 1;
+        out.g_row[w] = a0 + i;
+        out.g_col[w] = a0 + j;
+        out.g_dist[w] = dist3_xyz(S.px[i], S.py[i], S.pz[i], S.px[j], S.py[j], S.pz[j]);
+        if (grad) {
+            const int64_t rv = eoff + S.gex[j] + __popcll(S.adj[j] & ((1ull << i) - 1ull));
+            out.gT_perm[w] = (int32_t)(rv < eg_cap ? rv : eg_cap - 1);
+        }
+    }
+    const bool basis = out.sbf != nullptr;
+    if (basis) {
+        for (int v = tid; v < nb * 42; v += FILL_THREADS) {
+            const int k = v / 42, j = S.l_src[k], i = S.l_dst[k];
+            rad[v] = sbf_radial_value(dist3_xyz(S.px[i], S.py[i], S.pz[i], S.px[j], S.py[j], S.pz[j]), inv_cutoff, v - k * 42);
+        }
+        __syncthreads();
+    }
+    for (int rb = 0; rb < tp_m; rb += FILL_ROWS) {
+        const int r = rb + tid;
+        if (tid < FILL_ROWS && r < tp_m) {
+            int lo = 0, hi = nb;
+            while (hi - lo > 1) {
+                const int mid = (lo + hi) >> 1;
+                if (S.tptr[mid] <= r) lo = mid; else hi = mid;
+            }
+            const int k = lo, j = S.l_src[k], i = S.l_dst[k];
+            const float pix = S.px[i], piy = S.py[i], piz = S.pz[i], pjx = S.px[j], pjy = S.py[j], pjz = S.pz[j];
+            int idx = r - S.tptr[k], q, kind;
+            float ang;
+            if (idx < S.tcnt[k]) {
+                q = S.lptr[j];
+                while (true) {
+                    if (S.l_src[q] != i) {
+                        if (idx == 0) break;
+                        --idx;
+                    }
+                    ++q;
                 }
-                ++w;
-            }
-        }
-        for (int q = lptr[i]; q < lptr[i + 1]; ++q) {
-            const int j2 = l_src[q];
+                const int kk = S.l_src[q];
+                kind = 0;
+                ang = angle3(pjx - pix, pjy - piy, pjz - piz, S.px[kk] - pjx, S.py[kk] - pjy, S.pz[kk] - pjz);
+            } else {
+                q = S.lptr[i] + idx - S.tcnt[k];
+                const int j2 = S.l_src[q];
+                kind = 1;
+                ang = angle3(pix - pjx, piy - pjy, piz - pjz, S.px[j2] - pix, S.py[j2] - piy, S.pz[j2] - piz);
+            }
+            const int64_t w = toff + r;
             if (w < tp_cap) {
                 out.t_col[w] = b0 + q;
                 out.t_row[w] = b0 + k;
-                out.t_kind[w] = 1;
-                out.t_angle[w] = angle3(pix - pjx, piy - pjy, piz - pjz, px[j2] - pix, py[j2] - piy, pz[j2] - piz);
-            }
-            ++w;
-        }
-    }
-
-    if (lane < na) {
-        const int64_t w0 = eoff + gex[lane];
-        out.g_ptr[a0 + lane] = (int32_t)(w0 < eg_cap ? w0 : eg_cap);
-        unsigned long long m = mask;
-        int64_t w = w0;
-        while (m) {
-            const int j = __ffsll((long long)m) - 1;
-            m &= m - 1;
-            if (w < eg_cap) {
-                out.g_row[w] = a0 + lane;
-                out.g_col[w] = a0 + j;
-                out.g_dist[w] = dist3_xyz(xi, yi, zi, px[j], py[j], pz[j]);
-                if (in.need_grad) {
-                    const int64_t rv = eoff + gex[j] + __popcll(adj[j] & ((1ull << lane) - 1ull));
-                    out.gT_perm[w] = (int32_t)(rv < eg_cap ? rv : eg_cap - 1);
-                }
-            }
-            ++w;
-        }
-    }
-    if (!in.need_grad) return;
-
-    if (lane < na) out.lT_ptr[a0 + lane] = b0 + ltptr[lane];
-    if (last && lane == 0) {
-        out.lT_ptr[in.n] = (int32_t)in.n_bonds;
-        out.tT_ptr[in.n_bonds] = (int32_t)(toff + tp_m < tp_cap ? toff + tp_m : tp_cap);
-    }
-    for (int k = lane; k < nb; k += 64) out.lT_perm[b0 + k] = b0 + lt[k];
-
-    carry = 0;
-#pragma unroll
-    for (int c = 0; c < MOL_CHUNKS; ++c) {
-        if (c >= nchunk) continue;
-        const int q = c * 64 + lane;
-        const bool on = q < nb;
-        const int kq = on ? ss[c] : 0, jq = on ? sd[c] : 0;
-        const int ab = ltptr[jq], ae = in.with_triplets ? ltptr[jq + 1] : ab, bb = lptr[jq], be = lptr[jq + 1];
-        int cnt = 0;
-        if (on) {
-            for (int a = ab; a < ae; ++a) cnt += (l_dst[lt[a]] != kq) ? 1 : 0;
-            cnt += be - bb;
-        }
-        const int inc = wave_incl(cnt, lane);
-        if (on) {
-            int64_t w2 = toff + carry + inc - cnt;
-            out.tT_ptr[b0 + q] = (int32_t)(w2 < tp_cap ? w2 : tp_cap);
-            int a = ab, b = bb;
-            while (true) {
-                while (a < ae && l_dst[lt[a]] == kq) ++a;
-                const int ea = a < ae ? lt[a] : 0x7fffffff, eb = b < be ? b : 0x7fffffff;
-                if (ea == 0x7fffffff && eb == 0x7fffffff) break;
-                int row;
-                if (ea < eb) {
-                    const int ie = l_dst[ea];
-                    int rank = 0;
-                    for (int q2 = bb; q2 < q; ++q2) rank += (l_src[q2] != ie) ? 1 : 0;
-                    row = tptr[ea] + rank;
-                    ++a;
-                } else {
-                    row = tptr[eb] + tcnt[eb] + (q - bb);
-                    ++b;
-                }
-                if (w2 < tp_cap) out.tT_perm[w2] = (int32_t)(toff + row < tp_cap ? toff + row : tp_cap - 1);
-                ++w2;
-            }
-        }
-        carry += __shfl(inc, 63, 64);
-    }
+                out.t_kind[w] = kind;
+                out.t_angle[w] = ang;
+            }
+            if (basis) {
+                sbf_yl0(ang, ylm[tid]);
+                rsrc[tid] = q;
+            }
+        }
+        if (!basis) continue;
+        __syncthreads();
+        constexpr int PASS_ROWS = FILL_THREADS / 42;
+        if (tid < PASS_ROWS * 42) {
+            const int rows = tp_m - rb < FILL_ROWS ? tp_m - rb : FILL_ROWS;
+            const int r0 = tid / 42, c = tid - r0 * 42, l = c / 6;
+            for (int rr = r0; rr < rows; rr += PASS_ROWS) {
+                const int64_t w = toff + rb + rr;
+                if (w < tp_cap) out.sbf[w * 42 + c] = sbf_product(rad[rsrc[rr] * 42 + c], ylm[rr][l]);
+            }
+        }
+        __syncthreads();
+    }
+    if (basis && last)
+        for (int64_t v = (toff + tp_m) * 42 + tid; v < tp_cap * 42; v += FILL_THREADS) out.sbf[v] = 0.f;
 }
 
 int check_in(const float* pos, const int32_t* gptr, int64_t n, int64_t n_graphs, const int32_t* src, const int32_t* dst,
@@ -370,6 +497,13 @@
         !(cutoff_g > 0.f))
         return PAMNET_EINVAL;
     if (!pos || !gptr) return PAMNET_ENULL;
+    return PAMNET_OK;
+}
+
+int check_extras(const pamnet_mol_graph_out& o, int32_t need_grad) {
+    if ((o.tT_edge == nullptr) != (o.tT_node == nullptr)) return PAMNET_EINVAL;
+    if (o.tT_edge && !need_grad) return PAMNET_EINVAL;
+    if (o.sbf && !(o.sbf_cutoff > 0.f)) return PAMNET_EINVAL;
     return PAMNET_OK;
 }
 
@@ -383,9 +517,7 @@
     if (rc) return rc;
     if (!mol_tot || !totals) return PAMNET_ENULL;
     const MolIn in{pos, gptr, src, dst, n, n_graphs, n_bonds, cutoff_g, with_triplets ? 1 : 0, 0, 0.f};
-    const pamnet_mol_graph_out none{};
-    hipLaunchKernelGGL((mol_graph_kernel<false, false>), dim3((unsigned)n_graphs), dim3(64), 0, as_stream(stream), in, mol_tot, totals,
-                       none, (int64_t)0, (int64_t)0);
+    hipLaunchKernelGGL(mol_count_kernel<false>, dim3((unsigned)n_graphs), dim3(64), 0, as_stream(stream), in, mol_tot, totals);
     PAMNET_LAUNCH_CHECK();
     return PAMNET_OK;
 }
@@ -404,9 +536,10 @@
     if (n_bonds > 0 && (!o.l_row || !o.l_col || !o.l_dist || (need_grad && !o.lT_perm))) return PAMNET_ENULL;
     if (tp_cap > 0 && (!o.t_row || !o.t_col || !o.t_angle || !o.t_kind || (need_grad && !o.tT_perm))) return PAMNET_ENULL;
     if (need_grad && (!o.lT_ptr || !o.tT_ptr)) return PAMNET_ENULL;
+    if (int rc2 = check_extras(o, need_grad)) return rc2;
     const MolIn in{pos, gptr, src, dst, n, n_graphs, n_bonds, cutoff_g, with_triplets ? 1 : 0, need_grad ? 1 : 0, 0.f};
-    hipLaunchKernelGGL((mol_graph_kernel<true, false>), dim3((unsigned)n_graphs), dim3(64), 0, as_stream(stream), in,
-                       const_cast<int32_t*>(mol_tot), (int32_t*)nullptr, o, eg_cap, tp_cap);
+    hipLaunchKernelGGL(mol_fill_kernel<false>, dim3((unsigned)n_graphs), dim3(FILL_THREADS), 0, as_stream(stream), in, mol_tot, o,
+                       eg_cap, tp_cap, o.sbf ? 1.0f / o.sbf_cutoff : 0.f);
     PAMNET_LAUNCH_CHECK();
     return PAMNET_OK;
 }
@@ -418,9 +551,7 @@
     if (rc) return rc;
     if (!mol_tot || !totals) return PAMNET_ENULL;
     const MolIn in{pos, gptr, nullptr, nullptr, n, n_graphs, 0, cutoff_g, with_triplets ? 1 : 0, 0, cutoff_l};
-    const pamnet_mol_graph_out none{};
-    hipLaunchKernelGGL((mol_graph_kernel<false, true>), dim3((unsigned)n_graphs), dim3(64), 0, as_stream(stream), in, mol_tot,
-                       totals, none, (int64_t)0, (int64_t)0);
+    hipLaunchKernelGGL(mol_count_kernel<true>, dim3((unsigned)n_graphs), dim3(64), 0, as_stream(stream), in, mol_tot, totals);
     PAMNET_LAUNCH_CHECK();
     return PAMNET_OK;
 }
@@ -439,10 +570,11 @@
     if (n_local > 0 && (!o.l_row || !o.l_col || !o.l_dist || (need_grad && !o.lT_perm))) return PAMNET_ENULL;
     if (tp_cap > 0 && (!o.t_row || !o.t_col || !o.t_angle || !o.t_kind || (need_grad && !o.tT_perm))) return PAMNET_ENULL;
     if (need_grad && (!o.lT_ptr || !o.tT_ptr)) return PAMNET_ENULL;
+    if (int rc2 = check_extras(o, need_grad)) return rc2;
     const MolIn in{pos, gptr, nullptr, nullptr, n, n_graphs, n_local, cutoff_g, with_triplets ? 1 : 0, need_grad ? 1 : 0,
                    cutoff_l};
-    hipLaunchKernelGGL((mol_graph_kernel<true, true>), dim3((unsigned)n_graphs), dim3(64), 0, as_stream(stream), in,
-                       const_cast<int32_t*>(mol_tot), (int32_t*)nullptr, o, eg_cap, tp_cap);
+    hipLaunchKernelGGL(mol_fill_kernel<true>, dim3((unsigned)n_graphs), dim3(FILL_THREADS), 0, as_stream(stream), in, mol_tot, o,
+                       eg_cap, tp_cap, o.sbf ? 1.0f / o.sbf_cutoff : 0.f);
     PAMNET_LAUNCH_CHECK();
     return PAMNET_OK;
 }
diff --git a/physics-aware-multiplex-gnn_amd/csrc/sbf_core.h b/physics-aware-multiplex-gnn_amd/csrc/sbf_core.h
--- /dev/null
+++ b/physics-aware-multiplex-gnn_amd/csrc/sbf_core.h
@@ -0,0 +1,76 @@
+#pragma once
+#include "common.h"
+#include "basis_constants.h"
+
+namespace {
+
+__device__ __forceinline__ double envelope_d(double x) {
+    if (!(x < 1.0)) return 0.0;
+    const double x2 = x * x, x5 = x2 * x2 * x;
+    return 1.0 / x + x5 * (-21.0 + x * (35.0 - 15.0 * x));
+}
+
+constexpr int SERIES_TERMS = 28;
+struct SeriesTab {
+    double c[7][SERIES_TERMS + 1];
+    double inv_dfact[7];
+};
+constexpr SeriesTab make_series() {
+    SeriesTab t{};
+    for (int l = 0; l < 7; ++l) {
+        t.c[l][0] = 1.0;
+        for (int k = 1; k <= SERIES_TERMS; ++k) t.c[l][k] = t.c[l][k - 1] * -0.5 / ((double)k * (double)(2 * l + 2 * k + 1));
+        double d = 1.0;
+        for (int m = 1; m <= l; ++m) d *= (double)(2 * m + 1);
+        t.inv_dfact[l] = 1.0 / d;
+    }
+    return t;
+}
+__device__ __constant__ SeriesTab SBF_SERIES = make_series();
+
+__device__ __forceinline__ double sph_jl(int l, double z) {
+    if (z < (double)l + 1.0) {
+        const double h = z * z;
+        double sum = SBF_SERIES.c[l][SERIES_TERMS];
+#pragma unroll
+        for (int k = SERIES_TERMS - 1; k >= 0; --k) sum = fma(sum, h, SBF_SERIES.c[l][k]);
+        double pref = SBF_SERIES.inv_dfact[l];
+        for (int m = 0; m < l; ++m) pref *= z;
+        return pref * sum;
+    }
+    double s, c;
+    sincos(z, &s, &c);
+    const double iz = 1.0 / z;
+    double jm = s * iz;
+    if (l == 0) return jm;
+    double j = (jm - c) * iz;
+    for (int m = 1; m < l; ++m) {
+        const double jn = (double)(2 * m + 1) * iz * j - jm;
+        jm = j;
+        j = jn;
+    }
+    return j;
+}
+
+__device__ __forceinline__ float sbf_radial_value(float dist, float inv_cutoff, int c) {
+    const double x = (double)(dist * inv_cutoff);
+    return (float)(envelope_d(x) * PAMNET_SBF_NORM[c] * sph_jl(c / 6, (double)PAMNET_SBF_ZEROS_F32[c] * x));
+}
+
+__device__ __forceinline__ void sbf_yl0(float angle, double* y) {
+    const double ct = cos((double)angle);
+    double p0 = 1.0, p1 = ct;
+    y[0] = PAMNET_YL0_PREF[0] * p0;
+    y[1] = PAMNET_YL0_PREF[1] * p1;
+#pragma unroll
+    for (int k = 2; k <= 6; ++k) {
+        const double pl = ((double)(2 * k - 1) * ct * p1 - (double)(k - 1) * p0) / (double)k;
+        p0 = p1;
+        p1 = pl;
+        y[k] = PAMNET_YL0_PREF[k] * pl;
+    }
+}
+
+__device__ __forceinline__ float sbf_product(float rad, double y) { return (float)((double)rad * y); }
+
+}
diff --git a/physics-aware-multiplex-gnn_amd/pamnet_amd/graph.py b/physics-aware-multiplex-gnn_amd/pamnet_amd/graph.py
--- a/physics-aware-multiplex-gnn_amd/pamnet_amd/graph.py
+++ b/physics-aware-multiplex-gnn_amd/pamnet_amd/graph.py
@@ -79,6 +79,22 @@
     lib.call('pamnet_gather_scalars_i64', n, (ctypes.c_void_p * n)(*[t.data_ptr() for t in ts]),
              (ctypes.c_int32 * n)(*kinds), lib.ptr(out), lib.stream_of(out))
     return [int(v) for v in out.tolist()]
+
+
+_PINNED = __import__('threading').local()
+
+
+def host_words(words):
+    if not words.is_cuda:
+        return [int(v) for v in words.tolist()]
+    n = int(words.numel())
+    bufs = _PINNED.__dict__.setdefault('bufs', {})
+    host = bufs.get(n)
+    if host is None:
+        host = bufs[n] = torch.empty(n, dtype=I32, pin_memory=True)
+    host.copy_(words, non_blocking=True)
+    torch.cuda.current_stream(words.device).synchronize()
+    return [int(v) for v in host.tolist()]
 
 
 def _filter_count(ptr_in, nbr, dist, cut):
@@ -354,7 +370,7 @@
              types.data_ptr() if n else None, src.data_ptr() if ne else None, dst.data_ptr() if ne else None,
              lib.stream_of(batch))
     return node_graph, gf[:n_graphs + 1], (types if xk else None), src, dst, gf[n_graphs + 1:n_graphs + 2], \
-        gf[n_graphs + 2:n_graphs + 3], gf[n_graphs + 3:n_graphs + 7]
+        gf[n_graphs + 2:n_graphs + 3], gf[n_graphs + 3:n_graphs + 7], gf[n_graphs + 1:n_graphs + 7]
 
 
 def _check_sizes(flag, checks, all_kept=None, loops=None):
@@ -558,9 +574,9 @@
     return g
 
 
-def _mol_local_graph(g, pos, ing, cutoff_g, with_triplets, need_grad, cutoff_l=None):
+def _mol_local_graph(g, pos, ing, cutoff_g, with_triplets, need_grad, cutoff_l=None, aux_tables=False, basis_cutoff=None):
     import ctypes
-    node_graph, gptr, _, src0, dst0, flag, loops, totals = ing
+    node_graph, gptr, _, src0, dst0, flag, loops, totals, words = ing
     dev = pos.device
     free = cutoff_l is not None
     n, ng, m = g.n, g.n_graphs, int(src0.numel())
@@ -573,7 +589,7 @@
     else:
         lib.call('pamnet_mol_graph_count_i32', lib.ptr(pos), lib.ptr(gptr), n, ng, lib.ptr(src0), lib.ptr(dst0), m,
                  float(cutoff_g), wt, lib.ptr(mol_tot), lib.ptr(totals), st)
-    eg, tp, viol, counted, bad, lp_ = host_ints(totals[0], totals[1], totals[2], totals[3], flag, loops)
+    bad, lp_, eg, tp, viol, counted = host_words(words)
     if bad:
         _raise_bad_inputs()
     if free:
@@ -599,6 +615,16 @@
     if need_grad:
         o.gT_perm, o.lT_ptr, o.lT_perm = gT_perm.data_ptr(), lT_ptr.data_ptr(), lT_perm.data_ptr()
         o.tT_ptr, o.tT_perm = tT_ptr.data_ptr(), tT_perm.data_ptr()
+    seg_cuts = tT_edge = tT_node = sbf = None
+    if aux_tables:
+        seg_cuts = _i32(260, dev)
+        o.cuts = seg_cuts.data_ptr()
+        if need_grad:
+            tT_edge, tT_node = carve([tp] * 2)
+            o.tT_edge, o.tT_node = tT_edge.data_ptr(), tT_node.data_ptr()
+    if basis_cutoff is not None:
+        sbf = torch.empty((tp, 42), dtype=torch.float32, device=dev)
+        o.sbf, o.sbf_cutoff = sbf.data_ptr(), float(basis_cutoff)
     if free:
         lib.call('pamnet_mol_graph_free_fill_i32', lib.ptr(pos), lib.ptr(gptr), n, ng, m, float(cutoff_l), float(cutoff_g), wt,
                  1 if need_grad else 0, lib.ptr(mol_tot), eg, tp, ctypes.addressof(o), st)
@@ -616,6 +642,12 @@
         g.glob_T = _Given(g_ptr, gT_perm, n)
         g.loc_T = _Given(lT_ptr, lT_perm, n)
         g.tp_T = _Given(tT_ptr, tT_perm, max(m, 1))
+    if seg_cuts is not None:
+        g.seg_cuts = seg_cuts
+    if tT_edge is not None:
+        g.tT_edge, g.tT_node = tT_edge, tT_node
+    if sbf is not None:
+        g.sbf, g._sbf_cutoff = sbf, float(basis_cutoff)
     return True
 
 
@@ -674,8 +706,9 @@
         if (sizes is None and ing is not None and MOL_LOCAL and mol_local is not False
                 and not 0 < max_nb <= MOL_ATOMS
                 and (mol_local is True or n <= MOL_ATOMS * g.n_graphs // 2)):
-            if _mol_local_graph(g, pos, ing, cutoff_g, with_triplets, need_grad, cutoff_l=cutoff_l):
-                return _with_seg_cuts(g, dataset) if aux_tables else g
+            if _mol_local_graph(g, pos, ing, cutoff_g, with_triplets, need_grad, cutoff_l=cutoff_l, aux_tables=aux_tables,
+                                basis_cutoff=cutoff_l if default_basis else None):
+                return g
         gptr_g = radius_count(pos, node_graph, g.gptr, cutoff_g, max_nb, flag)
         lp = radius_count(pos, node_graph, g.gptr, cutoff_l)
         if sizes is not None:
@@ -716,9 +749,10 @@
         if (sizes is None and ing is not None and MOL_LOCAL and mol_local is not False and ei.size(1) > 0
                 and not 0 < max_nb <= MOL_ATOMS
                 and (mol_local is True or n <= MOL_ATOMS * g.n_graphs // 2)):
-            done = _mol_local_graph(g, pos, ing, cutoff_g, with_triplets, need_grad)
+            done = _mol_local_graph(g, pos, ing, cutoff_g, with_triplets, need_grad, aux_tables=aux_tables,
+                                    basis_cutoff=cutoff_l if default_basis else None)
             if done:
-                return _with_seg_cuts(g, dataset) if aux_tables else g
+                return g
         lp, l_src, l_dst, tp_ptr = bonds(ei, None if ing is None else (ing[3], ing[4]))
         if ing is not None:
             flag, kept = ing[5], ing[6]
diff --git a/physics-aware-multiplex-gnn_amd/pamnet_amd/lib.py b/physics-aware-multiplex-gnn_amd/pamnet_amd/lib.py
--- a/physics-aware-multiplex-gnn_amd/pamnet_amd/lib.py
+++ b/physics-aware-multiplex-gnn_amd/pamnet_amd/lib.py
@@ -5,6 +5,7 @@
 HERE = os.path.dirname(os.path.abspath(__file__))
 LIB_PATH = os.environ.get('PAMNET_HIP_LIB') or os.path.join(HERE, 'libpamnet_hip.so')
 HEADER = os.path.join(os.path.dirname(os.path.dirname(HERE)), 'include', 'pamnet_hip.h')
+ABI_VERSION = 18
 
 _lib = None
 _CT = {'float*': ctypes.c_void_p, 'int32_t*': ctypes.c_void_p, 'void*': ctypes.c_void_p,
@@ -45,6 +46,9 @@
         want = int(re.search(r'#define\s+PAMNET_ABI_VERSION\s+(\d+)', open(HEADER).read()).group(1))
         lib.pamnet_abi_version.argtypes = []
         got = int(lib.pamnet_abi_version())
+        if want != ABI_VERSION:
+            raise RuntimeError('pamnet_amd/lib.py mirrors the structures of ABI version %d, include/pamnet_hip.h declares %d'
+                               % (ABI_VERSION, want))
         if got != want:
             raise RuntimeError('libpamnet_hip.so was built for ABI version %d, include/pamnet_hip.h declares %d: rebuild '
                                '(python __graft_entry__.py)' % (got, want))
@@ -135,7 +139,8 @@
 
 class MolGraphOut(ctypes.Structure):
     _fields_ = [(k, _P) for k in ('g_ptr', 'g_row', 'g_col', 'g_dist', 'gT_perm', 'l_ptr', 'l_row', 'l_col', 'l_dist',
-                                  'lT_ptr', 'lT_perm', 't_ptr', 't_row', 't_col', 't_angle', 't_kind', 'tT_ptr', 'tT_perm')]
+                                  'lT_ptr', 'lT_perm', 't_ptr', 't_row', 't_col', 't_angle', 't_kind', 'tT_ptr', 'tT_perm',
+                                  'cuts', 'tT_edge', 'tT_node', 'sbf')] + [('sbf_cutoff', ctypes.c_float)]
 
 
 GF = {name: i for i, name in enumerate(
```

Result: no change. 69870 molecules/s (-0.2%).
